# set-soft/ComfyUI-FLOAT_Optimized

Measured on AMD Instinct MI355X. Metric: 512x512 frames/sec end-to-end audio->video @50 ODE steps, higher is better.
Workload: dtype fp16; 1 GPU; configs[1]: 10 s audio + 512x512 portrait in HBM -> 250 frames in pinned host memory; appearance encoder + wav2vec2 audio encoder + FMT sampling (50 Euler evaluations/window, CFG a=2.0 e=1.0) + decode + D2H, through InferenceAgent.infer_device (the product call); nfe=51, frames_per_clip=250, fmt_dtype=fp16, dec_dtype=fp16, decode_batch=32, hip_graph=True, parallelism=replicas x1 (one clip per GPU), stage_overlap=off

## Files before the change

comfyui-float_optimized_amd/csrc/fmt_api.hip:

```cpp
#include <math.h>
#include <stdlib.h>

#include "fmt_gemm.hpp"
#include "fmt_kernels.hpp"
#include "fmt_rb_kernels.hpp"
#include "fmt_big_kernels.hpp"

namespace {

typedef FmtLin Lin;

struct Blk {
  Lin qkv, proj, fc1, fc2;
};

constexpr int kMaxTok = 80;
constexpr int kMaxSteps = 1024;

}

struct float_fmt {
  float_fmt_cfg_t cfg;
  DevicePool pool;
  int D, ntok, Mpad, Kc, Ntot, Kx;
// ... 388 lines not shown
  }
}

struct Tiling {
  int mtw, nt, nw;
};
int pick_nw(int K, int forced) {
  const int KB = K / 32;
  if (forced && KB % forced == 0) return forced;
  if (KB >= 128 && KB % 16 == 0) return 16;
  if (KB >= 32 && KB % 8 == 0) return 8;
  return 4;
}
Tiling pick_tiling(const FmtTune& tn, int M, int N, int K, bool need_full_rows) {
  const int mt = (M + 15) / 16;
  if (need_full_rows) {
    if (mt <= 4) return {4, 1, pick_nw(K, 0)};
    return {mt <= 12 ? 12 : 15, 1, (tn.full_nw == 8 && (K / 32) % 8 == 0) ? 8 : 4};
  }
  int split = mt <= 4 ? 4 : (mt <= 12 ? 3 : 5);
  if (mt <= 2) split = mt;
  const int blocks = (mt + split - 1) / split;
  const bool wide = N >= 16384;
  if (mt >= 12) {
    const int* o = tn.plan + (wide ? 3 : 0);
    if (o[0]) {
      int nw = o[0] >= 12 ? 4 : pick_nw(K, o[2]);
      while (nw > 4 && nw * o[0] * 16 * o[1] * 16 * 4 > 160 * 1024) nw >>= 1;
      return {o[0], o[1], nw};
    }
  }
  if (wide) return {mt <= 4 ? 4 : 6, 2, std::min(8, pick_nw(K, 0))};
  if (mt > 15 && N % 64 == 0) return {3, 4, 4};
  int nt = 1;
  if (mt >= 5) {
    if ((N / 64) * blocks >= 192 && N % 64 == 0) nt = 4;
    else if ((N / 32) * blocks >= 192 && N % 32 == 0) nt = 2;
  } else if ((N / 16) * blocks > 512) {
    nt = 2;
  }
  return {split, nt, pick_nw(K, 0)};
}

GemmArgs base_args(const u16* A, const Lin& L, int M) {
  GemmArgs g;
  memset(&g, 0, sizeof(g));
  g.A = A;
  g.W = L.W;
  g.bias = L.b;
  g.K = L.K;
  g.N = L.N;
  g.M = M;
  return g;
}

Tiling pick_tiling32(int M) {
  const int mt = (M + 15) / 16;
  return {mt <= 5 ? mt : (mt <= 12 ? 3 : 5), 1, 4};
}

template <class T, int EPI>
int run_gemm(const FmtTune& tn, const GemmArgs& g, hipStream_t s, bool need_full_rows = false, const LayerPlan* plan = nullptr) {
  if constexpr (T::is32) {
    FH_REQUIRE(!need_full_rows, "the fp32 mode has no all-rows CFG epilogue tiling (token-blocked head only)");
    const Tiling t = pick_tiling32(g.M);
    GemmArgs g2 = g;
    g2.touch.W = nullptr;
    return launch_gemm<T, EPI>(g2, t.mtw, t.nt, t.nw, false, s);
  }
  if (plan && plan->on() && (g.M + 15) / 16 <= 15) {
    GemmArgs g2 = g;
    g2.touch.W = nullptr;
    return launch_gemm<T, EPI>(g2, plan->v[0], plan->v[1], plan->v[2], false, s);
  }
  const Tiling t = pick_tiling(tn, g.M, g.N, g.K, need_full_rows);
  return launch_gemm<T, EPI>(g, t.mtw, t.nt, t.nw, false, s);
}

struct PendingRed {
  int ks = 0;
  LnRed red{};
};

template <class T>
int run_gemm_partial(float_fmt* h, GemmArgs g, int ksplit, hipStream_t s, const LayerPlan* plan = nullptr) {
  g.ksplit = ksplit;
  g.out_f32 = h->slab;
  g.ldo = g.N;
  g.slab_stride = (size_t)h->Mpad * g.N;
  if (plan && plan->on() && !T::is32 && (g.M + 15) / 16 <= 15) {
    g.touch.W = nullptr;
    return launch_gemm<T, EPI_PARTIAL>(g, plan->v[0], plan->v[1], plan->v[2], false, s);
  }
  Tiling t = T::is32 ? pick_tiling32(g.M) : pick_tiling(h->tune, g.M, g.N * ksplit, g.K / ksplit, false);
  while (t.nt > 1 && g.N % (t.nt * 16)) t.nt >>= 1;
  if (T::is32) g.touch.W = nullptr;
  return launch_gemm<T, EPI_PARTIAL>(g, t.mtw, t.nt, t.nw, false, s);
}

TouchSpec make_touch(const FmtTune& tn, const Lin& L, int M, int ksplit, unsigned lanes, unsigned per_lane, int force_nt = 0) {
  TouchSpec t{};
  Tiling tl = ksplit ? pick_tiling(tn, M, L.N * ksplit, L.K / ksplit, false) : pick_tiling(tn, M, L.N, L.K, false);
  if (force_nt) tl.nt = force_nt;
  if (ksplit)
    while (tl.nt > 1 && L.N % (tl.nt * 16)) tl.nt >>= 1;
  const int ks = ksplit ? ksplit : 1;
  if (L.N % (tl.nt * 16) || L.K % (32 * ks) || 8 % ks) return t;
  const int nbn = L.N / (tl.nt * 16);
  if ((nbn * ks) % 8) return t;
  auto lg = [](unsigned v) {
    int n = 0;
    while ((1u << n) < v) ++n;
    return (1u << n) == v ? n : -1;
  };
  const unsigned P = 8 / ks, run_lines = (unsigned)(L.K / 32 / ks) * 8u;
  if (lg(run_lines) < 0 || lg((unsigned)tl.nt) < 0) return t;
  t.run_shift = (unsigned)lg(run_lines);
  t.nt_shift = (unsigned)lg((unsigned)tl.nt);
  t.p_shift = (unsigned)lg(P);
  t.tile_bytes = (unsigned)(L.K / 32) * 1024u;
  t.total = ((unsigned)nbn / P) * (unsigned)tl.nt * run_lines;
  if ((size_t)t.total > (size_t)lanes * per_lane) return t;
  t.W = reinterpret_cast<const char*>(L.W);
  return t;
}

TouchSpec make_touch_rb(const Lin& L, int shape, int kb, unsigned lanes, unsigned per_lane) {
  TouchSpec t{};
  const int ct = shape == 0 ? 4 : 8;
  if (kb <= 0 || (kb & (kb - 1)) || L.N % (ct * 16) || (L.N / (ct * 16)) % 8 || L.K / 32 < kb) return t;
  const unsigned run_lines = (unsigned)kb * 8u;
  auto lg = [](unsigned v) {
    int n = 0;
    while ((1u << n) < v) ++n;
    return n;
  };
  t.run_shift = (unsigned)lg(run_lines);
  t.nt_shift = (unsigned)lg((unsigned)ct);
  t.p_shift = 3;
  t.tile_bytes = (unsigned)(L.K / 32) * 1024u;
  t.total = (unsigned)(L.N / (ct * 16) / 8) * (unsigned)ct * run_lines;
  if ((size_t)t.total > (size_t)lanes * per_lane) return t;
  t.W = reinterpret_cast<const char*>(L.W);
  return t;
}

unsigned gemm_lanes_per_xcd(const FmtTune& tn, int M, int N, int K) {
  const Tiling t = pick_tiling(tn, M, N, K, false);
  const int mblk = ((M + 15) / 16 + t.mtw - 1) / t.mtw;
  return (unsigned)((N / (t.nt * 16)) * mblk / 8) * (unsigned)(t.nw * 64);
}

template <class T>
int launch_lnmod(float_fmt* h, int M, const float* shift, const float* scale, hipStream_t s, PendingRed* pend = nullptr,
                 const Lin* next = nullptr, u16* out = nullptr, int perm = 0, int touch_bit = 1, int rb_shape = -1) {
  const int nv = h->D / 256;
  const int rpw = h->tune.ln_rows;
  dim3 grid(rpw == 1 ? ((M + 63) / 64) * 64 : (M + rpw - 1) / rpw), block(64 * rpw);
  const int ks = pend ? pend->ks : 0;
  const bool wt = M <= kWtRows;
  LnRed red{};
  if (ks) red = pend->red;
  TouchSpec pf{};
  if (next && (h->tune.touch & (1 | touch_bit)) && rpw == 1 && !T::is32)
    pf = rb_shape >= 0 ? make_touch_rb(*next, rb_shape, h->tune.rb_touch, (grid.x / 8) * 64, 6)
                       : make_touch(h->tune, *next, M, 0, (grid.x / 8) * 64, 6);
#define LN_LAUNCH(NV, KS)                                                                                                          \
  do {                                                                                                                             \
    if (pf.W && wt) hipLaunchKernelGGL((fmt_lnmod_kernel<T, NV, KS, true, true>), grid, block, 0, s, h->xres, M, shift, scale, h->Ntot, out ? out : h->h16, red, pf, h->ntok, perm, h->sat); \
    else if (pf.W) hipLaunchKernelGGL((fmt_lnmod_kernel<T, NV, KS, true, false>), grid, block, 0, s, h->xres, M, shift, scale, h->Ntot, out ? out : h->h16, red, pf, h->ntok, perm, h->sat); \
    else if (wt) hipLaunchKernelGGL((fmt_lnmod_kernel<T, NV, KS, false, true>), grid, block, 0, s, h->xres, M, shift, scale, h->Ntot, out ? out : h->h16, red, pf, h->ntok, perm, h->sat); \
    else hipLaunchKernelGGL((fmt_lnmod_kernel<T, NV, KS, false, false>), grid, block, 0, s, h->xres, M, shift, scale, h->Ntot, out ? out : h->h16, red, pf, h->ntok, perm, h->sat);   \
  } while (0)
#define LN_CASE(NV)                     \
  case NV:                              \
    if (ks == 0) LN_LAUNCH(NV, 0);      \
    else if (ks == 1) LN_LAUNCH(NV, 1); \
    else if (ks == 2) LN_LAUNCH(NV, 2); \
    else if (ks == 4) LN_LAUNCH(NV, 4); \
    else LN_LAUNCH(NV, 8);              \
    break;
  switch (nv) {
    LN_CASE(1) LN_CASE(2) LN_CASE(4) LN_CASE(8)
    default:
      fh_set_error("dim_h %d unsupported (must be 256*{1,2,4,8})", h->D);
      return FLOAT_E_INVALID;
  }
#undef LN_CASE
#undef LN_LAUNCH
  if (pend) pend->ks = 0;
  FH_CHECK_HIP(hipGetLastError());
  return FLOAT_OK;
}

template <class T>
void launch_attn(float_fmt* h, int M, const Lin* pull, hipStream_t s) {
  const float_fmt_cfg_t& c = h->cfg;
  const int D = h->D, ntok = h->ntok;
  const int qpw = h->tune.attn_qpw, lpq = h->tune.attn_lpq;
  dim3 grid(c.heads, (M + qpw - 1) / qpw), block(qpw * lpq);
  TouchSpec pf{};
  if (pull && !T::is32) pf = make_touch(h->tune, *pull, M, 0, (grid.x * grid.y / 8) * block.x, 2);
#define ATTN_LAUNCH(LPQ, TCH)                                                                                                  \
  do {                                                                                                                         \
    if (M <= kWtRows) hipLaunchKernelGGL((fmt_attn_kernel<T, LPQ, TCH, true>), grid, block, 0, s, h->qkv16, 3 * D, h->att16, ntok, M, D, c.attn_window, pf, h->sat); \
    else hipLaunchKernelGGL((fmt_attn_kernel<T, LPQ, TCH, false>), grid, block, 0, s, h->qkv16, 3 * D, h->att16, ntok, M, D, c.attn_window, pf, h->sat);             \
  } while (0)
  if (lpq == 16) {
    if (pf.W) ATTN_LAUNCH(16, true);
    else ATTN_LAUNCH(16, false);
  } else {
    if (pf.W) ATTN_LAUNCH(8, true);
    else ATTN_LAUNCH(8, false);
  }
#undef ATTN_LAUNCH
}

int attnproj_hpw(const float_fmt* h) {
  const int hd = h->cfg.heads, hpw = h->tune.attnproj;
  if (hpw <= 0 || h->D != hd * 128 || hd % hpw) return 0;
  const int ks = hd / hpw;
  return (ks == 1 || ks == 2 || ks == 4 || ks == 8) && (hpw == 1 || hpw == 2) ? hpw : 0;
}
template <class T>
int launch_attnproj(float_fmt* h, int M, const Lin& proj, hipStream_t s) {
  const float_fmt_cfg_t& c = h->cfg;
  const int hpw = attnproj_hpw(h);
  GemmArgs g = base_args(nullptr, proj, M);
  g.sat = h->sat;
  g.out_f32 = h->slab;
  g.ldo = g.N;
  g.slab_stride = (size_t)h->Mpad * g.N;
  g.ksplit = c.heads / hpw;
  g.mblk = ((M + 15) / 16 + 2) / 3;
  const dim3 grid((unsigned)(g.ksplit * (g.N / (128 / hpw)) * g.mblk));
  fh_launch_prof(0, hpw == 2 ? fmt_attnproj_kernel<T, 3, 2> : fmt_attnproj_kernel<T, 3, 1>, grid, dim3(512), 0, s, h->qkv16, 3 * h->D, g,
                 h->ntok, h->D, c.attn_window);
  FH_CHECK_HIP(hipGetLastError());
  return FLOAT_OK;
}

constexpr int kScSteps = 64;

static int stream_priority(hipStream_t s) {
  int prio = 0;
  if (hipStreamGetPriority(s, &prio) != hipSuccess) {
    (void)hipGetLastError();
    prio = 0;
  }
  return prio;
}

template <class T>
int run_mod_all(float_fmt* h, int M, int e0, int n, hipStream_t s) {
  const int D = h->D;
  const FmtTune& tn = h->tune;
  FH_REQUIRE(n >= 1 && n <= kScSteps, "modulation batch of %d evaluations (max %d)", n, kScSteps);
  const int prio = (s == h->cap_stream && s) ? h->cap_prio : stream_priority(s);
  const bool big = !T::is32 && tn.wide && prio == 0 && big_shape_ok(tn, n * M, h->adaln_all.N, h->adaln_all.K, h->n_cu);
  hipLaunchKernelGGL((fmt_silu_c_kernel<T>), dim3((M * D / 8 + 255) / 256, n), dim3(256), 0, s, h->sc16, h->temb + (size_t)e0 * D,
                     h->ccond, M, D, (size_t)h->Mpad * D, big ? M : 0, h->sat);
  h->mod_zs = big ? (size_t)M * h->Ntot : (size_t)h->Mmod * h->Ntot;
  if constexpr (!T::is32) {
    if (big) return launch_big4<T>(h->sc16, h->adaln_all, h->modall, n * M, h->Ntot, h->n_cu, false, s);
  }
  GemmArgs g = base_args(h->sc16, h->adaln_all, M);
  g.sat = h->sat;
  g.out_f32 = h->modall;
  g.ldo = h->Ntot;
  g.zcount = n;
  const bool dma = (tn.wide_variant == 6 || tn.wide_variant == 7) && (M + 15) / 16 > 4 && dma_shape_ok(g, 320);
  g.zgroup = tn.zgroup > 0 ? tn.zgroup : (dma ? 2 : 4);
  g.a_zstride = (size_t)h->Mpad * D;
  g.o_zstride = (size_t)h->Mmod * h->Ntot;
  if constexpr (!T::is32) {
    if (tn.wide && g.N % 128 == 0 && g.K % 128 == 0) return launch_wide<T>(g, tn.wide_variant, false, s);
  }
  for (int z = 0; z < n; ++z) {
    GemmArgs gz = g;
    gz.A = g.A + (size_t)z * g.a_zstride * (sizeof(typename T::elem) / sizeof(u16));
    gz.out_f32 = g.out_f32 + (size_t)z * g.o_zstride;
    gz.zcount = 0;
    int rc = run_gemm<T, EPI_F32>(tn, gz, s);
    if (rc) return rc;
  }
  return FLOAT_OK;
}

constexpr int kMegaWgs = 256, kMegaSmem = 8 * 48 * 64 * 4;
MegaSync mega_sync_of(const float_fmt* h) {
  unsigned* m = h->mega_sync;
  return MegaSync{m, m + 8 * 32, m + 9 * 32, m + 17 * 32, m + 18 * 32, h->mega_err_host, reinterpret_cast<unsigned long long*>(m + 20 * 32), (unsigned)h->tune.mega_stamp_wg};
}
int mega_poll(float_fmt* h) {
  if (!h->mega_err_host || *reinterpret_cast<volatile unsigned*>(h->mega_err_host) == 0u) return FLOAT_OK;
  FH_CHECK_HIP(hipDeviceSynchronize());
  for (auto& gr : h->graphs) (void)hipGraphExecDestroy(gr.exec);
  h->graphs.clear();
  if (h->mega_sync) FH_CHECK_HIP(hipMemset(h->mega_sync, 0, (size_t)(32 * 20) * sizeof(unsigned)));
  *reinterpret_cast<volatile unsigned*>(h->mega_err_host) = 0u;
  h->tune.mega = 0;
  h->job.active = false;
  fh_set_error("fmt_mega_kernel: a grid barrier timed out in an earlier call (not all %d workgroups were resident) - the results of "
               "that call are invalid; the handle falls back to the launch chain (FLOAT_FMT_MEGA=0 selects it from the start)", 256);
  return FLOAT_E_HIP;
}
template <class T>
bool mega_shape_ok(const float_fmt* h, int nclip, int bc) {
  const FmtTune& tn = h->tune;
  if (T::is32 || !tn.mega || nclip != 1 || bc != 3 || h->D != 1024 || h->cfg.heads != 8 || h->n_cu < kMegaWgs) return false;
  if (attnproj_hpw(h) || tn.fc2_split != 4 || tn.proj_split != 0) return false;
  const int M = bc * h->ntok;
  auto is = [](Tiling t, int a, int b, int c) { return t.mtw == a && t.nt == b && t.nw == c; };
  const Blk& B = h->blk[0];
  return (M + 15) / 16 == 12 && (h->ntok + 15) / 16 == 4 && h->x_embed.K % 256 == 0 && h->final_lin.K % 256 == 0 &&
         is(pick_tiling(tn, M, B.qkv.N, B.qkv.K, false), 3, 4, 8) && is(pick_tiling(tn, M, B.proj.N, B.proj.K, false), 3, 1, 8) &&
         is(pick_tiling(tn, M, B.fc1.N, B.fc1.K, false), 3, 4, 8) && is(pick_tiling(tn, M, B.fc2.N * 4, B.fc2.K / 4, false), 3, 4, 8) &&
         B.fc2.K % 512 == 0;
}

template <class T>
int build_mega(float_fmt* h, int bc) {
  float_fmt::MegaPlan& P = h->mega[bc];
  P.tried = 1;
  {
    int per_cu = 0;
    if (hipOccupancyMaxActiveBlocksPerMultiprocessor(&per_cu, reinterpret_cast<const void*>(fmt_mega_kernel<T>), 512, kMegaSmem) != hipSuccess) {
      (void)hipGetLastError();
      per_cu = 0;
    }
    if (per_cu * h->n_cu < kMegaWgs) {
      h->tune.mega = 0;
      return FLOAT_OK;
    }
  }
  const float_fmt_cfg_t& c = h->cfg;
  const FmtTune& tn = h->tune;
  const int D = h->D, ntok = h->ntok, M = bc * ntok;
  std::vector<MegaStage> st;
  const size_t esz = sizeof(typename T::elem) / sizeof(u16);
  const size_t n_h = (size_t)h->Mpad * D * esz, n_hid = (size_t)h->Mpad * c.mlp_hidden * esz;
  if (!h->mega_ws) {
    int rc0 = h->pool.alloc(&h->mega_ws, (size_t)c.depth * (3 * n_h + n_hid), true);
    if (rc0) return rc0;
  }
  auto ws_h1 = [&](int b) { return h->mega_ws + (size_t)b * (3 * n_h + n_hid); };
  auto ws_h2 = [&](int b) { return ws_h1(b) + n_h; };
  auto ws_att = [&](int b) { return ws_h1(b) + 2 * n_h; };
  auto ws_hid = [&](int b) { return ws_h1(b) + 3 * n_h; };
  auto gemm_stage = [&](int kind, GemmArgs g, int mtw, int nt) {
    MegaStage m;
    memset(&m, 0, sizeof(m));
    m.kind = kind;
    g.sat = h->sat;
    g.mblk = ((g.M + 15) / 16 + mtw - 1) / mtw;
    if (g.ksplit < 1) g.ksplit = 1;
    m.g = g;
    m.nblk = (unsigned)((g.N / (nt * 16)) * g.mblk * g.ksplit);
    return m;
  };
  auto ln_stage = [&](int b_mod, int which, int ks, const float* bias, int gate_col, const Lin* next, int touch_bit, u16* out, int perm) {
    MegaStage m;
    memset(&m, 0, sizeof(m));
    m.kind = MS_LN;
    m.nblk = (unsigned)(((M + 63) / 64) * 64);
    m.shift_off = (long long)b_mod * 6 * D + (long long)which * D;
    m.scale_off = m.shift_off + D;
    m.ks = ks;
    m.red_bias = bias;
    m.red_gate_off = (long long)b_mod * 6 * D + (long long)gate_col * D;
    m.ln_out = out ? out : h->h16;
    m.perm = perm;
    if (next && (tn.touch & (1 | touch_bit))) m.pf = make_touch(tn, *next, M, 0, (m.nblk / 8) * 64, 6);
    return m;
  };
  {
    GemmArgs g = base_args(h->xin16, h->x_embed, ntok);
    g.out_f32 = h->xres;
    g.ldo = D;
    g.pos = h->pos;
    g.bc = bc;
    g.ntok = ntok;
    st.push_back(gemm_stage(MS_XEMBED, g, 4, 1));
  }
  for (int b = 0; b < c.depth; ++b) {
    const Blk& B = h->blk[b];
    if (b == 0) st.push_back(ln_stage(b, 0, 0, nullptr, 0, &B.qkv, 128, ws_h1(b), 0));
    else {
      MegaStage m = ln_stage(b, 0, 4, h->blk[b - 1].fc2.b, 0, &B.qkv, 128, ws_h1(b), 0);
      m.red_gate_off = (long long)(b - 1) * 6 * D + 5LL * D;
      st.push_back(m);
    }
    {
      GemmArgs g = base_args(ws_h1(b), B.qkv, M);
      g.out16 = h->qkv16;
      g.ldo16 = 3 * D;
      if (tn.touch & 8) g.touch = make_touch(tn, B.proj, M, 0, gemm_lanes_per_xcd(tn, M, g.N, g.K), 2);
      st.push_back(gemm_stage(MS_QKV, g, 3, 4));
    }
    {
      MegaStage m;
      memset(&m, 0, sizeof(m));
      m.kind = MS_ATTN;
      m.nblk = (unsigned)(c.heads * ((M + 7) / 8));
      if (tn.touch & 2) m.pf = make_touch(tn, B.proj, M, 0, (m.nblk / 8) * 128, 2);
      m.att_out = ws_att(b);
      st.push_back(m);
    }
    {
      GemmArgs g = base_args(ws_att(b), B.proj, M);
      g.out_f32 = h->xres;
      g.ldo = D;
      g.ldg = h->Ntot;
      if (tn.touch & 16) g.touch = make_touch(tn, B.fc1, M, 0, gemm_lanes_per_xcd(tn, M, g.N, g.K), 2);
      MegaStage m = gemm_stage(MS_PROJ, g, 3, 1);
      m.gate_off = (long long)b * 6 * D + 2LL * D;
      st.push_back(m);
    }
    st.push_back(ln_stage(b, 3, 0, nullptr, 0, &B.fc1, 64, ws_h2(b), 0));
    {
      GemmArgs g = base_args(ws_h2(b), B.fc1, M);
      g.out16 = ws_hid(b);
      g.ldo16 = B.fc2.K / 32;
      if (tn.touch & 4) g.touch = make_touch(tn, B.fc2, M, 4, gemm_lanes_per_xcd(tn, M, g.N, g.K), 2);
      st.push_back(gemm_stage(MS_FC1, g, 3, 4));
    }
    {
      GemmArgs g = base_args(ws_hid(b), B.fc2, M);
      g.ksplit = 4;
      g.out_f32 = h->slab;
      g.ldo = g.N;
      g.slab_stride = (size_t)h->Mpad * g.N;
      if (tn.touch & 32) {
        const unsigned lanes = gemm_lanes_per_xcd(tn, M, g.N * 4, g.K / 4);
        if (b + 1 < c.depth) g.touch = make_touch(tn, h->blk[b + 1].qkv, M, 0, lanes, 2);
        else g.touch = make_touch(tn, h->final_lin, M, 0, lanes, 2, 1);
      }
      st.push_back(gemm_stage(MS_FC2, g, 3, 4));
    }
  }
  {
    const int nblk = (ntok + 15) / 16, seqs = bc;
    MegaStage m = ln_stage(c.depth, 0, 4, h->blk[c.depth - 1].fc2.b, 0, nullptr, 0, h->hfin16, seqs * 16);
    m.red_gate_off = (long long)(c.depth - 1) * 6 * D + 5LL * D;
    st.push_back(m);
    GemmArgs g = base_args(h->hfin16, h->final_lin, nblk * seqs * 16);
    g.tokblk = 1;
    g.nclip = 1;
    g.bc = bc;
    g.ntok = ntok;
    g.n_prev = c.n_prev;
    g.xcur = h->xcur;
    g.xin16 = h->xin16;
    g.ldx = h->Kx / 32;
    st.push_back(gemm_stage(MS_HEAD, g, bc, 1));
  }
  for (const MegaStage& m : st) FH_REQUIRE(m.nblk <= (unsigned)kMegaWgs, "persistent kernel: a stage needs %u workgroups", m.nblk);
  int rc;
  if (!h->mega_sync && (rc = h->pool.alloc(&h->mega_sync, 32 * 20 + 2 * 3 * 64, true))) return rc;
  if (!h->mega_err_host) {
    FH_CHECK_HIP(hipHostMalloc(reinterpret_cast<void**>(&h->mega_err_host), 64, hipHostMallocMapped));
    memset(h->mega_err_host, 0, 64);
  }
  if ((rc = h->pool.alloc(&P.dev, st.size(), false))) return rc;
  FH_CHECK_HIP(hipMemcpy(P.dev, st.data(), st.size() * sizeof(MegaStage), hipMemcpyHostToDevice));
  P.nstage = (int)st.size();
  P.bc = bc;
  P.ctx = MegaCtx{h->xres, h->qkv16, h->slab, (size_t)h->Mpad * D, M, D, ntok, h->Ntot, c.attn_window, c.heads, h->sat};
  return FLOAT_OK;
}

template <class T>
int run_mega(float_fmt* h, int bc, const float* modbuf, bool euler, float dt, float a, float r, float e, hipStream_t s, float* vout_to) {
  float_fmt::MegaPlan& P = h->mega[bc];
  MegaDyn d{modbuf, dt, a, r, e, euler ? 1 : 0, vout_to ? vout_to : h->vout};
  fh_launch_prof(0, (fmt_mega_kernel<T>), dim3(kMegaWgs), dim3(512), kMegaSmem, s, P.dev, P.nstage, d, P.ctx, mega_sync_of(h));
  FH_CHECK_HIP(hipGetLastError());
  return FLOAT_OK;
}

template <class T>
int run_blocks(float_fmt* h, int nclip, int bc, const float* modbuf, bool euler, float dt, float a, float r, float e, hipStream_t s,
               float* vout_to = nullptr) {
  const float_fmt_cfg_t& c = h->cfg;
  const FmtTune& tn = h->tune;
  const int D = h->D, ntok = h->ntok, M = nclip * bc * ntok;
  int rc;
  if constexpr (!T::is32) {
    if (bc <= 4 && mega_shape_ok<T>(h, nclip, bc)) {
      if (h->mega[bc].dev) return run_mega<T>(h, bc, modbuf, euler, dt, a, r, e, s, vout_to);
    }
  }
  {
    GemmArgs g = base_args(h->xin16, h->x_embed, nclip * ntok);
    g.sat = h->sat;
    g.out_f32 = h->xres;
    g.ldo = D;
    g.pos = h->pos;
    g.bc = bc;
    g.ntok = ntok;
    if ((rc = run_gemm<T, EPI_XEMBED>(tn, g, s))) return rc;
  }
  PendingRed pend;
  RbPlan rb_qkv, rb_proj, rb_fc1, rb_fc2;
  if constexpr (!T::is32) {
    rb_qkv = pick_rb(tn, RB_QKV, M), rb_proj = pick_rb(tn, RB_PROJ, M), rb_fc1 = pick_rb(tn, RB_FC1, M), rb_fc2 = pick_rb(tn, RB_FC2, M);
  }
  auto split_ok = [&](int ks, const Lin& L) { return (ks == 1 || ks == 2 || ks == 4) && L.K % (128 * ks) == 0; };
  for (int b = 0; b < c.depth; ++b) {
    const float* mod = modbuf + (size_t)b * 6 * D;
    const Blk& B = h->blk[b];
    if ((rc = launch_lnmod<T>(h, M, mod, mod + D, s, &pend, &B.qkv, nullptr, 0, 128, rb_qkv.shape))) return rc;
    {
      GemmArgs g = base_args(h->h16, B.qkv, M);
      g.sat = h->sat;
      g.out16 = h->qkv16;
      g.ldo16 = 3 * D;
      if ((tn.touch & 8) && attnproj_hpw(h)) g.touch = make_touch(tn, B.proj, M, c.heads / attnproj_hpw(h), gemm_lanes_per_xcd(tn, M, g.N, g.K), 2, 8 / attnproj_hpw(h));
      else if ((tn.touch & 8) && !split_ok(tn.proj_split, B.proj)) g.touch = make_touch(tn, B.proj, M, 0, gemm_lanes_per_xcd(tn, M, g.N, g.K), 2);
      if (rb_qkv.shape >= 0) rc = launch_rbs<T, EPI_T16>(g, rb_qkv.shape, false, s);
      else rc = run_gemm<T, EPI_T16>(tn, g, s, false, &tn.plan_layer[RB_QKV]);
      if (rc) return rc;
    }
    if (rb_proj.shape >= 0) {
      launch_attn<T>(h, M, nullptr, s);
      GemmArgs gp = base_args(h->att16, B.proj, M);
      gp.ksplit = rb_proj.ksplit;
      gp.out_f32 = h->slab;
      gp.ldo = gp.N;
      gp.slab_stride = (size_t)h->Mpad * gp.N;
      if ((rc = launch_rbs<T, EPI_PARTIAL>(gp, rb_proj.shape, false, s))) return rc;
      pend.ks = rb_proj.ksplit;
      pend.red = LnRed{h->slab, (size_t)h->Mpad * D, B.proj.b, mod + 2 * D};
    } else if (attnproj_hpw(h)) {
      if ((rc = launch_attnproj<T>(h, M, B.proj, s))) return rc;
      pend.ks = c.heads / attnproj_hpw(h);
      pend.red = LnRed{h->slab, (size_t)h->Mpad * D, B.proj.b, mod + 2 * D};
    } else if (split_ok(tn.proj_split, B.proj)) {
      launch_attn<T>(h, M, nullptr, s);
      GemmArgs gp = base_args(h->att16, B.proj, M);
      if ((rc = run_gemm_partial<T>(h, gp, tn.proj_split, s))) return rc;
      pend.ks = tn.proj_split;
      pend.red = LnRed{h->slab, (size_t)h->Mpad * D, B.proj.b, mod + 2 * D};
    } else {
      launch_attn<T>(h, M, (tn.touch & 2) ? &B.proj : nullptr, s);
      GemmArgs g = base_args(h->att16, B.proj, M);
      g.sat = h->sat;
      g.out_f32 = h->xres;
      g.ldo = D;
      g.gate = mod + 2 * D;
      g.ldg = h->Ntot;
      if (tn.touch & 16) g.touch = make_touch(tn, B.fc1, M, 0, gemm_lanes_per_xcd(tn, M, g.N, g.K), 2);
      if ((rc = run_gemm<T, EPI_GATE_RES>(tn, g, s, false, &tn.plan_layer[RB_PROJ]))) return rc;
    }
    if ((rc = launch_lnmod<T>(h, M, mod + 3 * D, mod + 4 * D, s, &pend, &B.fc1, nullptr, 0, 64, rb_fc1.shape))) return rc;
    {
      GemmArgs g = base_args(h->h16, B.fc1, M);
      g.sat = h->sat;
      g.out16 = h->hid16;
      g.ldo16 = B.fc2.K / 32;
      if ((tn.touch & 4) && rb_fc2.shape < 0)
        g.touch = make_touch(tn, B.fc2, M, split_ok(tn.fc2_split, B.fc2) ? tn.fc2_split : 0, gemm_lanes_per_xcd(tn, M, g.N, g.K), 2);
      if (rb_fc1.shape >= 0) rc = launch_rbs<T, EPI_GELU_P16>(g, rb_fc1.shape, false, s);
      else rc = run_gemm<T, EPI_GELU_P16>(tn, g, s, false, &tn.plan_layer[RB_FC1]);
      if (rc) return rc;
    }
    if (rb_fc2.shape >= 0) {
      GemmArgs g = base_args(h->hid16, B.fc2, M);
      g.ksplit = rb_fc2.ksplit;
      g.out_f32 = h->slab;
      g.ldo = g.N;
      g.slab_stride = (size_t)h->Mpad * g.N;
      if ((rc = launch_rbs<T, EPI_PARTIAL>(g, rb_fc2.shape, false, s))) return rc;
      pend.ks = rb_fc2.ksplit;
      pend.red = LnRed{h->slab, (size_t)h->Mpad * D, B.fc2.b, mod + 5 * D};
    } else if (split_ok(tn.fc2_split, B.fc2)) {
      GemmArgs g = base_args(h->hid16, B.fc2, M);
      g.sat = h->sat;
      if (tn.touch & 32) {
        const unsigned lanes = gemm_lanes_per_xcd(tn, M, g.N * tn.fc2_split, g.K / tn.fc2_split);
        if (b + 1 < c.depth) g.touch = make_touch(tn, h->blk[b + 1].qkv, M, 0, lanes, 2);
        else g.touch = make_touch(tn, h->final_lin, M, 0, lanes, 2, 1);
      }
      if ((rc = run_gemm_partial<T>(h, g, tn.fc2_split, s, &tn.plan_layer[RB_FC2]))) return rc;
      pend.ks = tn.fc2_split;
      pend.red = LnRed{h->slab, (size_t)h->Mpad * D, B.fc2.b, mod + 5 * D};
    } else {
      GemmArgs g = base_args(h->hid16, B.fc2, M);
      g.sat = h->sat;
      g.out_f32 = h->xres;
      g.ldo = D;
      g.gate = mod + 5 * D;
      g.ldg = h->Ntot;
      if ((rc = run_gemm<T, EPI_GATE_RES>(tn, g, s))) return rc;
    }
  }
  {
    const float* mod = modbuf + (size_t)c.depth * 6 * D;
    const bool tokblk = (!tn.no_tokblk || nclip > 1) && (bc == 1 || bc == 3 || bc == 4) && h->final_lin.K % 256 == 0;
    FH_REQUIRE(tokblk || nclip == 1, "batched sampling needs the token-blocked head GEMM");
    const int nblk = (ntok + 15) / 16, seqs = nclip * bc;
    if ((rc = launch_lnmod<T>(h, M, mod, mod + D, s, &pend, nullptr, tokblk ? h->hfin16 : nullptr, tokblk ? seqs * 16 : 0))) return rc;
    GemmArgs g = base_args(tokblk ? h->hfin16 : h->h16, h->final_lin, tokblk ? nblk * seqs * 16 : M);
    g.sat = h->sat;
    g.tokblk = tokblk ? 1 : 0;
    g.nclip = nclip;
    g.bc = bc;
    g.ntok = ntok;
    g.n_prev = c.n_prev;
    g.a_cfg = a;
    g.r_cfg = r;
    g.e_cfg = e;
    g.dt = dt;
    if (euler) {
      g.xcur = h->xcur;
      g.xin16 = h->xin16;
      g.ldx = h->Kx / 32;
    } else {
      g.vout = vout_to ? vout_to : h->vout;
    }
    if (tokblk) rc = launch_gemm<T, EPI_CFG>(g, bc, 1, 8, false, s);
    else rc = run_gemm<T, EPI_CFG>(tn, g, s, true);
    if (rc) return rc;
  }
  FH_CHECK_HIP(hipGetLastError());
  return FLOAT_OK;
}

void linspace01(int n, std::vector<float>* ts) {
  ts->resize(n);
  if (n == 1) {
    (*ts)[0] = 0.f;
    return;
  }
  const float step = 1.0f / (float)(n - 1);
  const int half = n / 2;
  for (int i = 0; i < n; ++i) (*ts)[i] = (i < half) ? (0.f + step * (float)i) : (1.0f - step * (float)(n - 1 - i));
}

struct TimeSpec {
  float t;
  int nfe, stages;
  float c[4];
};
template <class T>
int prepare_time(float_fmt* h, const TimeSpec& ts, int n, hipStream_t s) {
  int rc;
  hipLaunchKernelGGL((fmt_tsin_kernel<T>), dim3(n), dim3(256), 0, s, h->tsin16, h->freqs, n, ts.t, ts.nfe, ts.stages, ts.c[0],
                     ts.c[1], ts.c[2], ts.c[3]);
  GemmArgs g = base_args(h->tsin16, h->t0, n);
  g.sat = h->sat;
  g.out16 = h->th16;
  g.ldo16 = h->t2.K / 32;
  if ((rc = launch_gemm<T, EPI_SILU_P16>(g, 4, 1, T::is32 ? 4 : pick_nw(g.K, 0), false, s))) return rc;
  GemmArgs g2 = base_args(h->th16, h->t2, n);
  g2.sat = h->sat;
  g2.out_f32 = h->temb;
  g2.ldo = h->D;
  if ((rc = launch_gemm<T, EPI_F32>(g2, 4, 1, T::is32 ? 4 : pick_nw(g2.K, 0), false, s))) return rc;
  return FLOAT_OK;
}

struct CfgMode {
  int bc;
  unsigned wr_mask, wa_mask, we_mask;
  int nclip = 1;
};

CfgMode cfg_mode(float a, float r, float e, int include_r) {
  if (a == 1.0f && r == 1.0f && e == 1.0f) return {1, 1u, 1u, 1u, 1};
  if (!include_r) return {3, 0b111u, 0b110u, 0b010u, 1};
  return {4, 0b1110u, 0b1100u, 0b0100u, 1};
}

template <class T>
int stage_window(float_fmt* h, const CfgMode& m, const float* x0, const float* wa, const float* wr, const float* we,
                 int we_len, const float* prev_x, const float* prev_wa, const float* prev_we, hipStream_t s) {
  const float_fmt_cfg_t& c = h->cfg;
  const int M = m.nclip * m.bc * h->ntok;
  hipLaunchKernelGGL((fmt_build_cond_kernel<T>), dim3(M), dim3(256), 0, s, h->cond16, h->Kc, m.bc, h->ntok, c.n_prev,
                     c.dim_w, c.dim_a, c.dim_e, wr, wa, prev_wa, we, we_len, prev_we, m.wr_mask, m.wa_mask, m.we_mask, h->sat);
  GemmArgs g = base_args(h->cond16, h->c_embed, M);
  g.sat = h->sat;
  g.out_f32 = h->ccond;
  g.ldo = h->D;
  int rc;
  if ((rc = run_gemm<T, EPI_F32>(h->tune, g, s))) return rc;
  const int n = m.nclip * h->ntok * c.dim_w;
  hipLaunchKernelGGL((fmt_init_x_kernel<T>), dim3((n + 255) / 256), dim3(256), 0, s, h->xcur, h->xin16, h->Kx / 32, x0, prev_x,
                     c.n_prev, c.n_cur, c.dim_w, m.nclip, h->sat);
  FH_CHECK_HIP(hipGetLastError());
  return FLOAT_OK;
}

int check_common(float_fmt* h, const void* we, int we_len, const void* prev_we) {
  FH_REQUIRE(h != nullptr, "null FMT handle");
  FH_REQUIRE(we_len == 1 || we_len == h->cfg.n_cur,
             "Dynamic emotion latent `we` time dimension (%d) does not match audio latent `wa` time dimension (%d).",
             we_len, h->cfg.n_cur);
  FH_REQUIRE(!(we_len > 1 && prev_we == nullptr),
             "`we` is dynamic (T>1), but prev_we was not provided with prev_x/prev_wa.");
  (void)we;
  return FLOAT_OK;
}

struct Tableau {
  int s;
  float c[4], a[4][3], b[4];
};
const Tableau& tableau(int method) {
  static const Tableau T[5] = {
      {1, {0.f}, {{0.f}}, {1.f}},
      {2, {0.f, 0.5f}, {{0.f}, {0.5f}}, {0.f, 1.f}},
      {4, {0.f, 1.f / 3, 2.f / 3, 1.f}, {{0.f}, {1.f / 3}, {-1.f / 3, 1.f}, {1.f, -1.f, 1.f}}, {0.125f, 0.375f, 0.375f, 0.125f}},
      {2, {0.f, 1.f}, {{0.f}, {1.f}}, {0.5f, 0.5f}},
      {3, {0.f, 1.f / 3, 2.f / 3}, {{0.f}, {1.f / 3}, {0.f, 2.f / 3}}, {0.25f, 0.f, 0.75f}},
  };
  return T[method];
}

TimeSpec time_spec(int method, int nfe) {
  const Tableau& tb = tableau(method);
  TimeSpec ts{};
  ts.nfe = nfe;
  ts.stages = tb.s;
  for (int j = 0; j < 4; ++j) ts.c[j] = tb.c[j];
  return ts;
}
int n_evals(int method, int nfe) { return (nfe - 1) * tableau(method).s; }

template <class T>
int run_window_steps(float_fmt* h, const CfgMode& m, int nfe, const std::vector<float>& ts, float a, float r, float e,
                     hipStream_t s) {
  const Tableau& tb = tableau(h->method);
  const float_fmt_cfg_t& c = h->cfg;
  const size_t kstride = (size_t)h->Bmax * kMaxTok * c.dim_w;
  const int n = m.nclip * c.n_cur * c.dim_w, rows = m.nclip * m.bc * h->ntok;
  const int nev = n_evals(h->method, nfe), batch = h->tune.hoist ? kScSteps : 1;
  const bool euler = h->method == FLOAT_ODE_EULER;
  int rc;
  for (int ev = 0; ev < nev; ++ev) {
    const int i = ev / tb.s, j = ev - i * tb.s, z = ev % batch;
    const float dt = ts[i + 1] - ts[i];
    if (z == 0 && (rc = run_mod_all<T>(h, rows, ev, std::min(batch, nev - ev), s))) return rc;
    const float* mod = h->modall + (size_t)z * h->mod_zs;
    if (euler) {
      if ((rc = run_blocks<T>(h, m.nclip, m.bc, mod, true, dt, a, r, e, s))) return rc;
      continue;
    }
    if (j > 0) {
      hipLaunchKernelGGL((fmt_rk_combine_kernel<T>), dim3((n + 255) / 256), dim3(256), 0, s, h->xcur, h->kbuf, kstride, j,
                         dt * tb.a[j][0], dt * tb.a[j][1], dt * tb.a[j][2], 0.f, 0, h->xin16, h->Kx / 32, c.n_prev, c.n_cur,
                         c.dim_w, m.nclip, h->sat);
    }
    if ((rc = run_blocks<T>(h, m.nclip, m.bc, mod, false, 0.f, a, r, e, s, h->kbuf + (size_t)j * kstride))) return rc;
    if (j == tb.s - 1) {
      hipLaunchKernelGGL((fmt_rk_combine_kernel<T>), dim3((n + 255) / 256), dim3(256), 0, s, h->xcur, h->kbuf, kstride, tb.s,
                         dt * tb.b[0], dt * tb.b[1], dt * tb.b[2], dt * tb.b[3], 1, h->xin16, h->Kx / 32, c.n_prev, c.n_cur,
                         c.dim_w, m.nclip, h->sat);
    }
  }
  FH_CHECK_HIP(hipGetLastError());
  return FLOAT_OK;
}

constexpr size_t kMaxGraphs = 8;
template <class T>
int run_window_steps_graph(float_fmt* h, const CfgMode& m, int we_len, int nfe, const std::vector<float>& ts, float a,
                           float r, float e, hipStream_t s) {
  float_fmt::GraphKey key;
  memset(&key, 0, sizeof(key));
  key.nfe = nfe;
  key.method = h->method;
  key.bc = m.bc;
  key.nclip = m.nclip;
  key.we_len = we_len;
  key.a = a;
  key.r = r;
  key.e = e;
  key.prio = stream_priority(s);
  float_fmt::GraphEntry* hit = nullptr;
  for (auto& g : h->graphs)
    if (g.key == key) hit = &g;
  if (!hit) {
    if (!h->cap_stream) FH_CHECK_HIP(hipStreamCreateWithFlags(&h->cap_stream, hipStreamNonBlocking));
    hipGraph_t graph = nullptr;
    h->cap_prio = key.prio;
    FH_CHECK_HIP(hipStreamBeginCapture(h->cap_stream, hipStreamCaptureModeThreadLocal));
    int rc = run_window_steps<T>(h, m, nfe, ts, a, r, e, h->cap_stream);
    hipError_t ce = hipStreamEndCapture(h->cap_stream, &graph);
    if (rc) {
      if (graph) (void)hipGraphDestroy(graph);
      return rc;
    }
    FH_CHECK_HIP(ce);
    hipGraphExec_t exec = nullptr;
    FH_CHECK_HIP(hipGraphInstantiate(&exec, graph, nullptr, nullptr, 0));
    (void)hipGraphDestroy(graph);
    if (h->graphs.size() >= kMaxGraphs) {
      size_t lru = 0;
      for (size_t i = 1; i < h->graphs.size(); ++i)
        if (h->graphs[i].used < h->graphs[lru].used) lru = i;
      FH_CHECK_HIP(hipDeviceSynchronize());
      (void)hipGraphExecDestroy(h->graphs[lru].exec);
      h->graphs.erase(h->graphs.begin() + lru);
    }
    h->graphs.push_back({key, exec, 0});
    hit = &h->graphs.back();
  }
  hit->used = ++h->graph_clock;
  FH_CHECK_HIP(hipGraphLaunch(hit->exec, s));
  return FLOAT_OK;
}

template <class T>
int window_impl(float_fmt* h, const float* x0, const float* wa, const float* wr, const float* we, int we_len,
                const float* prev_x, const float* prev_wa, const float* prev_we, int nfe, const std::vector<float>& ts,
                float a, float r, float e, int include_r, hipStream_t s, int nclip = 1) {
  CfgMode m = cfg_mode(a, r, e, include_r);
  m.nclip = nclip;
  FH_REQUIRE(!h->tune.no_tokblk || m.bc * h->ntok <= 240,
             "%d-way CFG of %d tokens is %d rows; the all-rows CFG epilogue GEMM holds at most 240 (15 row tiles)", m.bc, h->ntok,
             m.bc * h->ntok);
  int rc = stage_window<T>(h, m, x0, wa, wr, we, we_len, prev_x, prev_wa, prev_we, s);
  if (rc) return rc;
  if (nfe <= 1) return FLOAT_OK;
  hipStreamCaptureStatus cs = hipStreamCaptureStatusNone;
  if (hipStreamIsCapturing(s, &cs) != hipSuccess) {
    (void)hipGetLastError();
    cs = hipStreamCaptureStatusNone;
  }
  if (h->cfg.use_graph && !g_fh_profiling && cs == hipStreamCaptureStatusNone)
    return run_window_steps_graph<T>(h, m, we_len, nfe, ts, a, r, e, s);
  return run_window_steps<T>(h, m, nfe, ts, a, r, e, s);
}

template <class T>
int eval_impl(float_fmt* h, float t, const float* x, const float* wa, const float* wr, const float* we, int we_len,
              const float* prev_x, const float* prev_wa, const float* prev_we, float a, float r, float e, int include_r,
              float* out, hipStream_t s) {
  TimeSpec tsp{};
  tsp.t = t;
  int rc = prepare_time<T>(h, tsp, 1, s);
  if (rc) return rc;
  const CfgMode m = cfg_mode(a, r, e, include_r);
  FH_REQUIRE(!h->tune.no_tokblk || m.bc * h->ntok <= 240,
             "%d-way CFG of %d tokens is %d rows; the all-rows CFG epilogue GEMM holds at most 240 (15 row tiles)", m.bc, h->ntok,
             m.bc * h->ntok);
  if ((rc = stage_window<T>(h, m, x, wa, wr, we, we_len, prev_x, prev_wa, prev_we, s))) return rc;
  if ((rc = run_mod_all<T>(h, m.bc * h->ntok, 0, 1, s))) return rc;
  if ((rc = run_blocks<T>(h, 1, m.bc, h->modall, false, 0.f, a, r, e, s))) return rc;
  return dev_copy(out, h->vout, (size_t)h->ntok * h->cfg.dim_w, s);
}

template <class T>
int sample_window(float_fmt* h, int k, hipStream_t s) {
  const float_fmt_cfg_t& c = h->cfg;
  auto& J = h->job;
  const int L = c.n_cur, P = c.n_prev, Tn = J.T, B = J.B;
  const bool dynamic = J.we_len > 1;
  int rc;
  auto blocks = [](int n) { return dim3((n + 255) / 256); };
  if (k == J.first) {
    if ((rc = prepare_time<T>(h, time_spec(h->method, J.nfe), std::max(1, n_evals(h->method, J.nfe)), s))) return rc;
    if (J.hist_x) rc = dev_copy(h->prev_x, J.hist_x, (size_t)B * P * c.dim_w, s);
    else rc = dev_zero(h->prev_x, (size_t)B * P * c.dim_w, s);
    if (rc) return rc;
    if (J.hist_wa) rc = dev_copy(h->prev_wa, J.hist_wa, (size_t)B * P * c.dim_a, s);
    else rc = dev_zero(h->prev_wa, (size_t)B * P * c.dim_a, s);
    if (rc) return rc;
    if (J.hist_we) rc = dev_copy(h->prev_we, J.hist_we, (size_t)B * P * c.dim_e, s);
    else rc = dev_zero(h->prev_we, (size_t)B * P * c.dim_e, s);
    if (rc) return rc;
  } else if (P > 0) {
    hipLaunchKernelGGL(fmt_tail_kernel, blocks(B * P * c.dim_w), dim3(256), 0, s, h->prev_x, h->xcur, P, L, c.dim_w, B);
    hipLaunchKernelGGL(fmt_tail_kernel, blocks(B * P * c.dim_a), dim3(256), 0, s, h->prev_wa, h->wa_c, P, L, c.dim_a, B);
    if (dynamic) hipLaunchKernelGGL(fmt_tail_kernel, blocks(B * P * c.dim_e), dim3(256), 0, s, h->prev_we, h->we_c, P, L, c.dim_e, B);
  }
  hipLaunchKernelGGL(fmt_slice_pad_kernel, blocks(B * L * c.dim_a), dim3(256), 0, s, h->wa_c, J.wa, k * L, Tn, L, c.dim_a, B);
  if (dynamic) hipLaunchKernelGGL(fmt_slice_pad_kernel, blocks(B * L * c.dim_e), dim3(256), 0, s, h->we_c, J.we, k * L, Tn, L, c.dim_e, B);
  if ((rc = dev_copy(h->x0_c, J.noise + (size_t)k * B * L * c.dim_w, (size_t)B * L * c.dim_w, s))) return rc;
  rc = window_impl<T>(h, h->x0_c, h->wa_c, J.wr, dynamic ? h->we_c : J.we, dynamic ? L : 1, h->prev_x, h->prev_wa,
                      dynamic ? h->prev_we : nullptr, J.nfe, J.ts, J.a, J.r, J.e, J.include_r, s, B);
  if (rc) return rc;
  const int rows = (k == J.total - 1) ? (Tn - k * L) : L;
  return dev_copy2d(J.r_d + (size_t)k * L * c.dim_w, (size_t)Tn * c.dim_w, h->xcur, (size_t)L * c.dim_w, rows * c.dim_w, B, s);
}

template <class T>
int create_impl(float_fmt* h, const TensorTable& tt) {
  const float_fmt_cfg_t& c = h->cfg;
  const int D = c.dim_h;
  int rc;
  prime_kernels<T>();
  if ((rc = pack_linear<T>(h, tt, {"x_embedder.proj"}, D, c.dim_w, &h->x_embed))) return rc;
  if ((rc = pack_linear<T>(h, tt, {"t_embedder.mlp.0"}, D, 256, &h->t0))) return rc;
  if ((rc = pack_linear<T>(h, tt, {"t_embedder.mlp.2"}, D, D, &h->t2))) return rc;
  if ((rc = pack_linear<T>(h, tt, {"c_embedder"}, D, c.dim_w + c.dim_a + c.dim_e, &h->c_embed))) return rc;
  h->blk.resize(c.depth);
  std::vector<std::string> ada;
  for (int b = 0; b < c.depth; ++b) {
    const std::string p = "blocks." + std::to_string(b) + ".";
    if ((rc = pack_linear<T>(h, tt, {p + "attn.qkv"}, 3 * D, D, &h->blk[b].qkv))) return rc;
    if ((rc = pack_linear<T>(h, tt, {p + "attn.proj"}, D, D, &h->blk[b].proj))) return rc;
    if ((rc = pack_linear<T>(h, tt, {p + "mlp.fc1"}, c.mlp_hidden, D, &h->blk[b].fc1))) return rc;
    if ((rc = pack_linear<T>(h, tt, {p + "mlp.fc2"}, D, c.mlp_hidden, &h->blk[b].fc2))) return rc;
    ada.push_back(p + "adaLN_modulation.1");
  }
  if ((rc = pack_linear<T>(h, tt, ada, 6 * D, D, &h->adaln_all))) return rc;
  {
    Lin tail;
    if ((rc = pack_linear<T>(h, tt, {"decoder.adaLN_modulation.1"}, 2 * D, D, &tail))) return rc;
    Lin fused;
    fused.N = h->adaln_all.N + tail.N;
    fused.K = h->adaln_all.K;
    constexpr size_t esz = sizeof(typename T::elem) / sizeof(u16);
    if ((rc = h->pool.alloc(&fused.W, (size_t)fused.N * fused.K * esz, false))) return rc;
    if ((rc = h->pool.alloc(&fused.b, (size_t)fused.N, false))) return rc;
    FH_CHECK_HIP(hipMemcpy(fused.W, h->adaln_all.W, (size_t)h->adaln_all.N * fused.K * esz * sizeof(u16), hipMemcpyDeviceToDevice));
    FH_CHECK_HIP(hipMemcpy(fused.W + (size_t)h->adaln_all.N * fused.K * esz, tail.W, (size_t)tail.N * fused.K * esz * sizeof(u16),
                           hipMemcpyDeviceToDevice));
    FH_CHECK_HIP(hipMemcpy(fused.b, h->adaln_all.b, (size_t)h->adaln_all.N * sizeof(float), hipMemcpyDeviceToDevice));
    FH_CHECK_HIP(hipMemcpy(fused.b + h->adaln_all.N, tail.b, (size_t)tail.N * sizeof(float), hipMemcpyDeviceToDevice));
    h->adaln_all = fused;
  }
  if ((rc = pack_linear<T>(h, tt, {"decoder.linear"}, c.dim_w, D, &h->final_lin))) return rc;
  return FLOAT_OK;
}

}


int fmt_pack_linear(const FmtTune& tn, DevicePool* pool, int dtype, const TensorTable& tt, const std::vector<std::string>& names,
                    int N_each, int K, FmtLin* out) {
  FH_REQUIRE(dtype == FLOAT_DT_BF16 || dtype == FLOAT_DT_FP16 || dtype == FLOAT_DT_FP32, "the GEMM service: unknown dtype %d", dtype);
  if (dtype == FLOAT_DT_FP32) return pack_linear_pool<FP32>(tn, pool, tt, names, N_each, K, out);
  return dtype == FLOAT_DT_BF16 ? pack_linear_pool<BF16>(tn, pool, tt, names, N_each, K, out)
                                : pack_linear_pool<FP16>(tn, pool, tt, names, N_each, K, out);
}

int fmt_pack_linear_raw(const FmtTune& tn, DevicePool* pool, int dtype, const float* w, const float* b, int N, int K, FmtLin* out) {
  std::vector<float> zeros;
  if (!b) {
    zeros.assign(N, 0.f);
    b = zeros.data();
  }
  float_tensor_t t[2];
  memset(t, 0, sizeof(t));
  t[0].name = "raw.weight";
  t[0].data = w;
  t[0].ndim = 2;
  t[0].shape[0] = N;
  t[0].shape[1] = K;
  t[1].name = "raw.bias";
  t[1].data = b;
  t[1].ndim = 1;
  t[1].shape[0] = N;
  TensorTable tt(t, 2);
  return fmt_pack_linear(tn, pool, dtype, tt, {"raw"}, N, K, out);
}

GemmArgs fmt_gemm_args(const u16* A, const FmtLin& L, int M) { return base_args(A, L, M); }

void fmt_gemm_prime(int dtype) {
  if (dtype == FLOAT_DT_BF16) prime_kernels<BF16>();
  else if (dtype == FLOAT_DT_FP32) prime_kernels<FP32>();
  else prime_kernels<FP16>();
}

template <class T>
static int gemm_run_t(const FmtTune& tn, int epi, const GemmArgs& g, hipStream_t s) {
  switch (epi) {
    case EPI_F32: return run_gemm<T, EPI_F32>(tn, g, s);
    case EPI_T16: return run_gemm<T, EPI_T16>(tn, g, s);
    case EPI_SILU_P16: return run_gemm<T, EPI_SILU_P16>(tn, g, s);
    case EPI_GELU_P16: return run_gemm<T, EPI_GELU_P16>(tn, g, s);
    case EPI_GELUERF_P16: return run_gemm<T, EPI_GELUERF_P16>(tn, g, s);
    default: fh_set_error("fmt_gemm_run: epilogue %d is not exported", epi); return FLOAT_E_INVALID;
  }
}

int fmt_gemm_run(const FmtTune& tn, int dtype, int epi, GemmArgs g, hipStream_t s) {
  if (dtype == FLOAT_DT_FP32) return gemm_run_t<FP32>(tn, epi, g, s);
  return dtype == FLOAT_DT_BF16 ? gemm_run_t<BF16>(tn, epi, g, s) : gemm_run_t<FP16>(tn, epi, g, s);
}

template <class T>
static int debug_impl(float_fmt* h, int what, const float* in, float* out, hipStream_t s) {
  const int D = h->D, ntok = h->ntok;
  if (what == 0) {
    return dev_copy(out, h->pos, (size_t)ntok * D, s);
  }
  if (what == 2) {
    FH_REQUIRE(h->mega_sync && h->mega[3].nstage > 0 && h->mega[3].nstage <= 64, "no persistent-kernel plan");
    FH_CHECK_HIP(hipStreamSynchronize(s));
    const int n = h->mega[3].nstage * 3;
    std::vector<unsigned long long> st(n);
    FH_CHECK_HIP(hipMemcpy(st.data(), h->mega_sync + 20 * 32, n * 8, hipMemcpyDeviceToHost));
    std::vector<float> us(n);
    for (int i = 0; i < n; ++i) us[i] = st[i] ? (float)((double)(st[i] - st[0]) * 0.01) : -1.f;
    FH_CHECK_HIP(hipMemcpy(out, us.data(), n * 4, hipMemcpyHostToDevice));
    return FLOAT_OK;
  }
  FH_REQUIRE(what == 1 && in != nullptr, "float_fmt_debug: unknown request %d (or null input)", what);
// ... 19 lines not shown
  FH_REQUIRE(cfg->max_batch >= 0 && cfg->max_batch <= 16, "max_batch must be in [0, 16] (got %d)", cfg->max_batch);
  float_fmt* h = new float_fmt();
  h->tune = FmtTune::from_env();
  h->cfg = *cfg;
  h->D = cfg->dim_h;
  h->ntok = cfg->n_prev + cfg->n_cur;
  h->Bmax = cfg->max_batch > 0 ? cfg->max_batch : 1;
  h->Mpad = 16 * ((h->Bmax * 4 * h->ntok + 15) / 16 + 12);
  h->Kc = round_up(cfg->dim_w + cfg->dim_a + cfg->dim_e, 128);
  h->Kx = round_up(cfg->dim_w, 128);
  {
    int dev = 0, ncu = 0;
    if (hipGetDevice(&dev) == hipSuccess && hipDeviceGetAttribute(&ncu, hipDeviceAttributeMultiprocessorCount, dev) == hipSuccess) h->n_cu = ncu;
    else (void)hipGetLastError();
  }
  h->Ntot = cfg->depth * 6 * h->D + 2 * h->D;
  TensorTable tt(tensors, n_tensors);
  int rc = (cfg->dtype == FLOAT_DT_BF16) ? create_impl<BF16>(h, tt)
           : (cfg->dtype == FLOAT_DT_FP16) ? create_impl<FP16>(h, tt) : create_impl<FP32>(h, tt);
  const int D = h->D, Mp = h->Mpad;
  const size_t esz = cfg->dtype == FLOAT_DT_FP32 ? 2 : 1;
  auto A = [&](auto** p, size_t n) {
    if (!rc) rc = h->pool.alloc(p, std::is_same<std::remove_reference_t<decltype(**p)>, u16>::value ? n * esz : n, true);
  };
  A(&h->pos, (size_t)kMaxTok * D);
  A(&h->freqs, 128);
  A(&h->cond16, (size_t)Mp * h->Kc);
  A(&h->sc16, (size_t)kScSteps * Mp * D + (size_t)12 * 16 * D);
  A(&h->h16, (size_t)Mp * D);
  A(&h->hfin16, (size_t)h->Bmax * 64 * ((kMaxTok + 15) / 16) * D);
  A(&h->qkv16, (size_t)Mp * 3 * D);
  A(&h->att16, (size_t)Mp * D);
  A(&h->hid16, (size_t)Mp * cfg->mlp_hidden);
  A(&h->xin16, (size_t)(h->Bmax * kMaxTok + 6 * 16) * h->Kx);
  A(&h->tsin16, (size_t)kMaxSteps * 256);
  A(&h->th16, (size_t)kMaxSteps * D);
  A(&h->ccond, (size_t)Mp * D);
  h->Mmod = 16 * ((h->Bmax * 4 * h->ntok + 15) / 16);
  if (!rc) rc = h->pool.alloc(&h->modall, (size_t)kScSteps * h->Mmod * h->Ntot, false);
  A(&h->kbuf, (size_t)4 * h->Bmax * kMaxTok * cfg->dim_w);
  A(&h->xres, (size_t)Mp * D);
  A(&h->slab, (size_t)8 * Mp * D);
  A(&h->sat, 1);
  A(&h->xcur, (size_t)h->Bmax * cfg->n_cur * cfg->dim_w);
  A(&h->temb, (size_t)kMaxSteps * D);
  A(&h->vout, (size_t)h->Bmax * kMaxTok * cfg->dim_w);
  A(&h->wa_c, (size_t)h->Bmax * cfg->n_cur * cfg->dim_a);
  A(&h->we_c, (size_t)h->Bmax * cfg->n_cur * cfg->dim_e);
  A(&h->x0_c, (size_t)h->Bmax * cfg->n_cur * cfg->dim_w);
  A(&h->prev_x, (size_t)h->Bmax * cfg->n_cur * cfg->dim_w);
  A(&h->prev_wa, (size_t)h->Bmax * cfg->n_cur * cfg->dim_a);
  A(&h->prev_we, (size_t)h->Bmax * cfg->n_cur * cfg->dim_e);
  if (!rc) {
    std::vector<float> pos((size_t)h->ntok * D);
    const float_tensor_t* pe = tt.find("pos_embed");
    if (pe && TensorTable::numel(pe) == (int64_t)h->ntok * D) {
      memcpy(pos.data(), pe->data, pos.size() * sizeof(float));
    } else {
      for (int p = 0; p < h->ntok; ++p)
        for (int j = 0; j < D; ++j) {
          const float ang = (float)((double)p / pow(10000.0, 2.0 * (double)(j / 2) / (double)D));
          pos[(size_t)p * D + j] = (j & 1) ? cosf(ang) : sinf(ang);
        }
    }
    std::vector<float> fr(128);
    for (int k = 0; k < 128; ++k) fr[k] = expf(-logf(10000.0f) * (float)k / 128.0f);
    if (hipMemcpy(h->pos, pos.data(), pos.size() * sizeof(float), hipMemcpyHostToDevice) != hipSuccess ||
        hipMemcpy(h->freqs, fr.data(), fr.size() * sizeof(float), hipMemcpyHostToDevice) != hipSuccess) {
      fh_set_error("hipMemcpy of FMT tables failed");
      rc = FLOAT_E_HIP;
    }
  }
  if (!rc && cfg->dtype != FLOAT_DT_FP32) {
    const bool ok = cfg->dtype == FLOAT_DT_BF16 ? mega_shape_ok<BF16>(h, 1, 3) : mega_shape_ok<FP16>(h, 1, 3);
    if (ok) rc = cfg->dtype == FLOAT_DT_BF16 ? build_mega<BF16>(h, 3) : build_mega<FP16>(h, 3);
  }
  if (rc) {
    float_fmt_destroy(h);
    return rc;
  }
  *out = h;
  return FLOAT_OK;
}

void float_fmt_destroy(float_fmt_t* h) {
  if (!h) return;
  for (auto& g : h->graphs) (void)hipGraphExecDestroy(g.exec);
  if (h->cap_stream) (void)hipStreamDestroy(h->cap_stream);
  if (h->mega_err_host) (void)hipHostFree(h->mega_err_host);
  h->pool.release();
  delete h;
}

int float_fmt_eval(float_fmt_t* h, float t, const float* x, const float* wa, const float* wr, const float* we,
                   int32_t we_len, const float* prev_x, const float* prev_wa, const float* prev_we, float a_cfg,
                   float r_cfg, float e_cfg, int32_t include_r_cfg, float* out, void* stream) {
  int rc = check_common(h, we, we_len, prev_we);
  if (rc) return rc;
  if ((rc = mega_poll(h))) return rc;
  FH_REQUIRE(x && wa && wr && we && prev_x && prev_wa && out, "null tensor argument to float_fmt_eval");
  hipStream_t s = (hipStream_t)stream;
  return h->cfg.dtype == FLOAT_DT_BF16
             ? eval_impl<BF16>(h, t, x, wa, wr, we, we_len, prev_x, prev_wa, prev_we, a_cfg, r_cfg, e_cfg, include_r_cfg, out, s)
         : h->cfg.dtype == FLOAT_DT_FP16
             ? eval_impl<FP16>(h, t, x, wa, wr, we, we_len, prev_x, prev_wa, prev_we, a_cfg, r_cfg, e_cfg, include_r_cfg, out, s)
             : eval_impl<FP32>(h, t, x, wa, wr, we, we_len, prev_x, prev_wa, prev_we, a_cfg, r_cfg, e_cfg, include_r_cfg, out, s);
}

int float_fmt_sample_chunk(float_fmt_t* h, const float* x0, const float* wa, const float* wr, const float* we,
                           int32_t we_len, const float* prev_x, const float* prev_wa, const float* prev_we, int32_t nfe,
                           float a_cfg, float r_cfg, float e_cfg, int32_t include_r_cfg, float* out, void* stream) {
  int rc = check_common(h, we, we_len, prev_we);
  if (rc) return rc;
  if ((rc = mega_poll(h))) return rc;
  FH_REQUIRE(x0 && wa && wr && we && prev_x && prev_wa && out, "null tensor argument to float_fmt_sample_chunk");
  FH_REQUIRE(nfe >= 1 && n_evals(h->method, nfe) < kMaxSteps, "nfe=%d: too many evaluations (max %d)", nfe, kMaxSteps);
  hipStream_t s = (hipStream_t)stream;
  std::vector<float> ts;
  linspace01(nfe, &ts);
  const float_fmt_cfg_t& c = h->cfg;
  if ((rc = dev_copy(h->x0_c, x0, (size_t)c.n_cur * c.dim_w, s))) return rc;
  if ((rc = dev_copy(h->wa_c, wa, (size_t)c.n_cur * c.dim_a, s))) return rc;
  if ((rc = dev_copy(h->prev_x, prev_x, (size_t)c.n_prev * c.dim_w, s))) return rc;
  if ((rc = dev_copy(h->prev_wa, prev_wa, (size_t)c.n_prev * c.dim_a, s))) return rc;
  if (we_len > 1) {
    if ((rc = dev_copy(h->we_c, we, (size_t)c.n_cur * c.dim_e, s))) return rc;
    if ((rc = dev_copy(h->prev_we, prev_we, (size_t)c.n_prev * c.dim_e, s))) return rc;
  }
  const float* we_p = we_len > 1 ? h->we_c : we;
  const float* pwe_p = we_len > 1 ? h->prev_we : nullptr;
  const TimeSpec tsp = time_spec(h->method, nfe);
  const int nev = std::max(1, n_evals(h->method, nfe));
#define FMT_CHUNK(TT)                                                                                                          \
  do {                                                                                                                           \
    if ((rc = prepare_time<TT>(h, tsp, nev, s))) return rc;                                                                      \
    rc = window_impl<TT>(h, h->x0_c, h->wa_c, wr, we_p, we_len, h->prev_x, h->prev_wa, pwe_p, nfe, ts, a_cfg, r_cfg, e_cfg,      \
                         include_r_cfg, s);                                                                                      \
  } while (0)
  if (c.dtype == FLOAT_DT_BF16) FMT_CHUNK(BF16);
  else if (c.dtype == FLOAT_DT_FP16) FMT_CHUNK(FP16);
  else FMT_CHUNK(FP32);
#undef FMT_CHUNK
  if (rc) return rc;
  return dev_copy(out, h->xcur, (size_t)c.n_cur * c.dim_w, s);
}

int float_fmt_debug(float_fmt_t* h, int32_t what, const float* in, float* out, void* stream) {
  FH_REQUIRE(h != nullptr && out != nullptr, "null argument to float_fmt_debug");
  return h->cfg.dtype == FLOAT_DT_BF16   ? debug_impl<BF16>(h, what, in, out, (hipStream_t)stream)
         : h->cfg.dtype == FLOAT_DT_FP16 ? debug_impl<FP16>(h, what, in, out, (hipStream_t)stream)
                                         : debug_impl<FP32>(h, what, in, out, (hipStream_t)stream);
}

int float_fmt_saturation(float_fmt_t* h, uint64_t* total, int32_t reset, void* stream) {
  FH_REQUIRE(h && total, "null argument to float_fmt_saturation");
  FH_CHECK_HIP(hipStreamSynchronize((hipStream_t)stream));
  unsigned long long v = 0;
  FH_CHECK_HIP(hipMemcpy(&v, h->sat, sizeof(v), hipMemcpyDeviceToHost));
  *total = v;
  if (reset) {
    FH_CHECK_HIP(hipMemsetAsync(h->sat, 0, sizeof(v), (hipStream_t)stream));
    FH_CHECK_HIP(hipStreamSynchronize((hipStream_t)stream));
  }
  if (int rc = mega_poll(h)) return rc;
  return FLOAT_OK;
}

int float_fmt_set_method(float_fmt_t* h, int32_t method) {
  FH_REQUIRE(h != nullptr, "null FMT handle");
  FH_REQUIRE(method >= FLOAT_ODE_EULER && method <= FLOAT_ODE_HEUN3, "unknown ODE method %d", method);
  h->method = method;
  return FLOAT_OK;
}

int float_fmt_sample_begin(float_fmt_t* h, const float* wr, const float* wa, int32_t T, const float* we, int32_t we_len,
                           const float* noise, int32_t nfe, float a_cfg, float r_cfg, float e_cfg, int32_t include_r_cfg,
                           float* r_d) {
  FH_REQUIRE(h != nullptr, "null FMT handle");
  FH_REQUIRE(wr && wa && we && noise && r_d, "null tensor argument to float_fmt_sample");
  FH_REQUIRE(T >= 1, "T must be >= 1 (got %d)", T);
  FH_REQUIRE(we_len == 1 || we_len == T,
             "Dynamic emotion latent `we` time dimension (%d) does not match audio latent `wa` time dimension (%d).",
             we_len, T);
  FH_REQUIRE(nfe >= 1 && n_evals(h->method, nfe) < kMaxSteps, "nfe=%d: too many evaluations (max %d)", nfe, kMaxSteps);
  auto& J = h->job;
  J.wr = wr;
  J.wa = wa;
  J.we = we;
  J.noise = noise;
  J.r_d = r_d;
  J.T = T;
  J.we_len = we_len;
  J.nfe = nfe;
  J.include_r = include_r_cfg;
  J.a = a_cfg;
  J.r = r_cfg;
  J.e = e_cfg;
  J.B = 1;
  J.next = 0;
  J.n_chunks = (T + h->cfg.n_cur - 1) / h->cfg.n_cur;
  J.first = 0;
  J.total = J.n_chunks;
  J.hist_x = J.hist_wa = J.hist_we = nullptr;
  linspace01(nfe, &J.ts);
  J.active = true;
  return FLOAT_OK;
}

int float_fmt_sample_begin_range(float_fmt_t* h, const float* wr, const float* wa, int32_t T, const float* we, int32_t we_len,
                                 const float* noise, int32_t nfe, float a_cfg, float r_cfg, float e_cfg, int32_t include_r_cfg,
                                 float* r_d, int32_t first_window, int32_t end_window, const float* hist_x, const float* hist_wa,
                                 const float* hist_we) {
  int rc = float_fmt_sample_begin(h, wr, wa, T, we, we_len, noise, nfe, a_cfg, r_cfg, e_cfg, include_r_cfg, r_d);
  if (rc) return rc;
  auto& J = h->job;
  J.active = false;
  FH_REQUIRE(first_window >= 0 && first_window < end_window && end_window <= J.total,
             "window range [%d, %d) outside the clip's %d windows", first_window, end_window, J.total);
  FH_REQUIRE(we_len == 1 || hist_we != nullptr || hist_x == nullptr,
             "a dynamic-emotion job that starts from a history needs hist_we too");
  J.first = J.next = first_window;
  J.n_chunks = end_window;
  J.hist_x = hist_x;
  J.hist_wa = hist_wa;
  J.hist_we = we_len > 1 ? hist_we : nullptr;
  J.active = true;
  return FLOAT_OK;
}

int float_fmt_sample_next(float_fmt_t* h, void* stream, int32_t* window_done, int32_t* windows_left) {
  FH_REQUIRE(h != nullptr && h->job.active, "float_fmt_sample_next without float_fmt_sample_begin");
  if (int prc = mega_poll(h)) return prc;
  auto& J = h->job;
  hipStream_t s = (hipStream_t)stream;
  const int k = J.next;
  int rc = h->cfg.dtype == FLOAT_DT_BF16   ? sample_window<BF16>(h, k, s)
           : h->cfg.dtype == FLOAT_DT_FP16 ? sample_window<FP16>(h, k, s)
                                           : sample_window<FP32>(h, k, s);
  if (rc) {
    J.active = false;
    return rc;
  }
  J.next = k + 1;
  if (window_done) *window_done = k;
  if (windows_left) *windows_left = J.n_chunks - J.next;
  if (J.next >= J.n_chunks) J.active = false;
  return FLOAT_OK;
}

int float_fmt_sample_batch(float_fmt_t* h, int32_t n_clips, const float* wr, const float* wa, int32_t T, const float* we,
                           int32_t we_len, const float* noise, int32_t nfe, float a_cfg, float r_cfg, float e_cfg,
                           int32_t include_r_cfg, float* r_d, void* stream) {
  FH_REQUIRE(h != nullptr, "null FMT handle");
  FH_REQUIRE(n_clips >= 1 && n_clips <= h->Bmax, "batch of %d clips, the handle was created with max_batch = %d", n_clips, h->Bmax);
  int rc = float_fmt_sample_begin(h, wr, wa, T, we, we_len, noise, nfe, a_cfg, r_cfg, e_cfg, include_r_cfg, r_d);
  if (rc) return rc;
  h->job.B = n_clips;
  int32_t left = 1;
  while (left > 0)
    if ((rc = float_fmt_sample_next(h, stream, nullptr, &left))) return rc;
  return FLOAT_OK;
}

int float_fmt_sample(float_fmt_t* h, const float* wr, const float* wa, int32_t T, const float* we, int32_t we_len,
                     const float* noise, int32_t nfe, float a_cfg, float r_cfg, float e_cfg, int32_t include_r_cfg,
                     float* r_d, void* stream) {
  int rc = float_fmt_sample_begin(h, wr, wa, T, we, we_len, noise, nfe, a_cfg, r_cfg, e_cfg, include_r_cfg, r_d);
  if (rc) return rc;
  int32_t left = 1;
  while (left > 0)
    if ((rc = float_fmt_sample_next(h, stream, nullptr, &left))) return rc;
  return FLOAT_OK;
}

}
```

comfyui-float_optimized_amd/csrc/fmt_kernels.hpp:

```cpp
#pragma once
#include "common.hpp"
#include "fmt_pack.hpp"

template <class T, int MTW, int NT, int NW, int EPI, bool COH>
__device__ __forceinline__ void fmt_gemm_body(const GemmArgs& g, const unsigned bid, const unsigned nblk) {
  constexpr int BN = NT * 16;
  constexpr int ROWS = MTW * 16;
  constexpr bool WT = NW >= 8 || COH;
  auto ldA = [](const typename T::elem* p) -> typename T::pack8 { return T::load8(p); };
  constexpr int NTHR = NW * 64;
  constexpr int PF = T::is32 ? 1 : ((MTW + NT <= 7) ? 4 : ((MTW + NT <= 8) ? 3 : 2));
  typedef typename T::elem E;
  typedef typename T::pack8 P8;
  extern __shared__ __attribute__((aligned(16))) float red[];
  const int lane = threadIdx.x & 63;
  const int w = threadIdx.x >> 6;
  const int r16 = lane & 15, q = lane >> 4;
  int bx, by, ks = 0;
  {
    const int nbn = g.N / BN, id = (int)bid;
    const int nbx = (EPI == EPI_PARTIAL) ? nbn * g.ksplit : nbn;
    if ((nbx & 7) == 0) {
      const int slot = id >> 3;
      by = slot % g.mblk;
      bx = (slot / g.mblk) * 8 + (id & 7);
    } else {
      bx = id % nbx;
      by = id / nbx;
    }
    if constexpr (EPI == EPI_PARTIAL) {
      if ((nbx & 7) == 0 && (8 % g.ksplit) == 0) {
        const int P = 8 / g.ksplit, x = bx & 7;
        ks = x / P;
        bx = (bx >> 3) * P + (x % P);
      } else {
        ks = bx / nbn;
        bx = bx % nbn;
      }
    }
  }
  const int nb0 = bx * NT;
  const int mt0 = by * MTW;
  const int n0 = nb0 * 16, m0 = mt0 * 16;

  f32x4 acc[MTW][NT];
#pragma unroll
  for (int i = 0; i < MTW; ++i)
#pragma unroll
    for (int j = 0; j < NT; ++j) acc[i][j] = f32x4{0.f, 0.f, 0.f, 0.f};

  const int KB = g.K >> 5;
  const int KBs = (EPI == EPI_PARTIAL) ? KB / g.ksplit : KB;
  const int KBw = KBs / NW;
  const E* Ap = reinterpret_cast<const E*>(g.A) + ((size_t)mt0 * KB + ks * KBs + w * KBw) * 512 + lane * 8;
  const E* Wp = reinterpret_cast<const E*>(g.W) + ((size_t)nb0 * KB + ks * KBs + w * KBw) * 512 + lane * 8;
  const size_t tstride = (size_t)KB * 512;
  constexpr bool kEarlyRes = (EPI == EPI_GATE_RES) && (MTW * 16 * (NT * 2) <= NW * 64);
  float4 res_pf[2], gate_pf[2];
  if constexpr (kEarlyRes) {
    const int r = threadIdx.x / (NT * 2), cg = threadIdx.x % (NT * 2);
    const int row = m0 + r, nb = n0 + cg * 8;
    if (r < ROWS && row < g.M) {
      const float* o = g.out_f32 + (size_t)row * g.ldo + nb;
      const float* gt = g.gate + (size_t)row * g.ldg + nb;
      res_pf[0] = fh_load_f4<COH>(o);
      res_pf[1] = fh_load_f4<COH>(o + 4);
      gate_pf[0] = fh_load_f4_stream(gt);
      gate_pf[1] = fh_load_f4_stream(gt + 4);
    }
  }

  P8 a[PF][MTW], b[PF][NT];
#pragma unroll
  for (int p = 0; p < PF; ++p) {
    if (p < KBw) {
#pragma unroll
      for (int j = 0; j < NT; ++j) b[p][j] = T::load8_nt(Wp + j * tstride + (size_t)p * 512);
#pragma unroll
      for (int i = 0; i < MTW; ++i) a[p][i] = ldA(Ap + i * tstride + (size_t)p * 512);
    }
  }
  constexpr bool kTouch = (EPI == EPI_GELU_P16 || EPI == EPI_T16 || EPI == EPI_GATE_RES || EPI == EPI_PARTIAL);
  unsigned touched[2] = {0u, 0u};
  if constexpr (kTouch) {
    if (g.touch.W) fmt_touch(g.touch, bid & 7, (bid >> 3) * NTHR + threadIdx.x, (nblk >> 3) * NTHR, touched);
  }
  for (int kb0 = 0; kb0 < KBw; kb0 += PF) {
#pragma unroll
    for (int p = 0; p < PF; ++p) {
      const int kb = kb0 + p;
      if (kb < KBw) {
#pragma unroll
        for (int i = 0; i < MTW; ++i)
#pragma unroll
          for (int j = 0; j < NT; ++j) acc[i][j] = T::mfma(a[p][i], b[p][j], acc[i][j]);
        if (kb + PF < KBw) {
#pragma unroll
          for (int j = 0; j < NT; ++j)
            b[p][j] = T::load8_nt(Wp + j * tstride + (size_t)(kb + PF) * 512);
#pragma unroll
          for (int i = 0; i < MTW; ++i) a[p][i] = ldA(Ap + i * tstride + (size_t)(kb + PF) * 512);
        }
      }
    }
  }

  if constexpr (kTouch) {
    if (g.touch.W) fmt_touch_retire(touched);
  }
  float* my = red + w * (ROWS * BN);
#pragma unroll
  for (int i = 0; i < MTW; ++i)
#pragma unroll
    for (int j = 0; j < NT; ++j)
#pragma unroll
      for (int r = 0; r < 4; ++r) my[(i * 16 + q * 4 + r) * BN + j * 16 + r16] = acc[i][j][r];
  __syncthreads();

  constexpr int S = ROWS * BN;
  constexpr int CG = BN / 8;
  unsigned rm = 0u;
  auto slab_sum = [&](int o) {
    float a = red[o];
#pragma unroll
    for (int ww = 1; ww < NW; ++ww) a += red[ww * S + o];
    return a;
  };
  if constexpr (EPI == EPI_CFG) {
    const int nclip = g.nclip > 1 ? g.nclip : 1;
    const int tb = g.tokblk ? by / nclip : 0, q = g.tokblk ? by - tb * nclip : 0;
    const int ni = g.tokblk ? 16 : g.ntok, i0 = tb * 16, rstride = g.tokblk ? 16 : g.ntok;
    float* const vout_q = g.vout ? g.vout + (size_t)q * g.ntok * g.N : nullptr;
    float* const xcur_q = g.xcur ? g.xcur + (size_t)q * (g.ntok - g.n_prev) * g.N : nullptr;
    for (int idx = threadIdx.x; idx < ni * BN; idx += NTHR) {
      const int il = idx / BN, i = i0 + il, c = idx % BN, n = n0 + c;
      if (i >= g.ntok) break;
      const float bias = g.bias[n];
      float v[4];
#pragma unroll
      for (int b2 = 0; b2 < 4; ++b2) {
        if (b2 < g.bc) {
          const int o = (b2 * rstride + il) * BN + c;
          v[b2] = slab_sum(o) + bias;
        } else {
          v[b2] = 0.f;
        }
      }
      float out;
      if (g.bc == 1) {
        out = v[0];
      } else if (g.bc == 3) {
        out = v[0] + g.a_cfg * (v[2] - v[0]) + g.e_cfg * (v[1] - v[2]);
      } else {
        out = v[0] + g.r_cfg * (v[1] - v[0]) + g.a_cfg * (v[3] - v[1]) + g.e_cfg * (v[2] - v[3]);
      }
      if (vout_q) vout_q[(size_t)i * g.N + n] = out;
      if (xcur_q && i >= g.n_prev) {
        const size_t xo = (size_t)(i - g.n_prev) * g.N + n;
        const float xn = xcur_q[xo] + g.dt * out;
        xcur_q[xo] = xn;
        reinterpret_cast<E*>(g.xin16)[fmt_pack_off(q * g.ntok + i, n, g.ldx)] = fh_cvt<T>(xn, rm);
      }
    }
  } else {
    for (int idx = threadIdx.x; idx < ROWS * CG; idx += NTHR) {
      const int r = idx / CG, cg = idx % CG;
      const int row = m0 + r, nb = n0 + cg * 8;
      if (row >= g.M) continue;
      float v[8];
      {
        const float* p0 = red + r * BN + cg * 8;
#pragma unroll
        for (int e = 0; e < 8; e += 4) {
          float4 a4 = *reinterpret_cast<const float4*>(p0 + e);
#pragma unroll
          for (int ww = 1; ww < NW; ++ww) {
            const float4 t4 = *reinterpret_cast<const float4*>(p0 + ww * S + e);
            a4.x += t4.x;
            a4.y += t4.y;
            a4.z += t4.z;
            a4.w += t4.w;
          }
          float4 bb = float4{0.f, 0.f, 0.f, 0.f};
          if constexpr (EPI != EPI_PARTIAL) bb = *reinterpret_cast<const float4*>(g.bias + nb + e);
          v[e + 0] = a4.x + bb.x;
          v[e + 1] = a4.y + bb.y;
          v[e + 2] = a4.z + bb.z;
          v[e + 3] = a4.w + bb.w;
        }
      }
      if constexpr (EPI == EPI_F32 || EPI == EPI_PARTIAL) {
        float* o = g.out_f32 + (size_t)ks * g.slab_stride + (size_t)row * g.ldo + nb;
        fh_store_f4_wt<fh_site<COH>(4), WT>(o, float4{v[0], v[1], v[2], v[3]});
        fh_store_f4_wt<fh_site<COH>(4), WT>(o + 4, float4{v[4], v[5], v[6], v[7]});
      } else if constexpr (EPI == EPI_T16 || EPI == EPI_SILU_P16 || EPI == EPI_GELU_P16 || EPI == EPI_GELUERF_P16) {
        P8 u;
#pragma unroll
        for (int i = 0; i < 8; ++i) {
          float x = v[i];
          if constexpr (EPI == EPI_SILU_P16) x = fh_silu(x);
          if constexpr (EPI == EPI_GELU_P16) x = fh_gelu_tanh(x);
          if constexpr (EPI == EPI_GELUERF_P16) x = fh_gelu_erf(x);
          T::set(u, i, x);
        }
        fh_track_pack<T>(rm, u);
        E* const o16 = reinterpret_cast<E*>(g.out16);
        if constexpr (EPI == EPI_T16) T::template store8_wt<fh_site<COH>(8), WT>(o16 + (size_t)row * g.ldo16 + nb, u);
        else T::template store8_wt<fh_site<COH>(8), WT>(o16 + fmt_pack_off(row, nb, g.ldo16), u);
      } else if constexpr (EPI == EPI_GATE_RES) {
        float* o = g.out_f32 + (size_t)row * g.ldo + nb;
        const float* gt = g.gate + (size_t)row * g.ldg + nb;
#pragma unroll
        for (int e = 0; e < 8; e += 4) {
          float4 x, gg;
          if constexpr (kEarlyRes) {
            x = res_pf[e / 4];
            gg = gate_pf[e / 4];
          } else {
            x = fh_load_f4<COH>(o + e);
            gg = fh_load_f4_stream(gt + e);
          }
          x.x += gg.x * v[e + 0];
          x.y += gg.y * v[e + 1];
          x.z += gg.z * v[e + 2];
          x.w += gg.w * v[e + 3];
          fh_store_f4_wt<fh_site<COH>(16), WT>(o + e, x);
        }
      } else if constexpr (EPI == EPI_XEMBED) {
        const int q = row / g.ntok, tok = row - q * g.ntok;
        const float* ps = g.pos + (size_t)tok * g.N + nb;
#pragma unroll
        for (int i = 0; i < 8; ++i) v[i] += ps[i];
        for (int b2 = 0; b2 < g.bc; ++b2) {
          float* o = g.out_f32 + (size_t)((q * g.bc + b2) * g.ntok + tok) * g.ldo + nb;
          fh_store_f4_wt<fh_site<COH>(32), WT>(o, float4{v[0], v[1], v[2], v[3]});
          fh_store_f4_wt<fh_site<COH>(32), WT>(o + 4, float4{v[4], v[5], v[6], v[7]});
        }
      }
    }
  }
  if constexpr (EPI == EPI_CFG || EPI == EPI_T16 || EPI == EPI_SILU_P16 || EPI == EPI_GELU_P16 || EPI == EPI_GELUERF_P16) fh_range_flush<T>(g.sat, rm);
}

template <class T, int MTW, int NT, int NW, int EPI>
__global__ __launch_bounds__(NW * 64) void fmt_gemm_kernel(GemmArgs g) {
  fmt_gemm_body<T, MTW, NT, NW, EPI, false>(g, blockIdx.x, gridDim.x);
}

template <class T, int MTW, int KCH , int NWV = 4>
__global__ __launch_bounds__(NWV * 64) void fmt_gemm_wide_kernel(GemmArgs g) {
  constexpr int EPI = EPI_F32;
  constexpr int NF = MTW * KCH;
  constexpr int NFW = (NF + NWV - 1) / NWV;
  constexpr int WR = NWV / 4, MTR = MTW / WR;
  static_assert(MTW % WR == 0, "row tiles must split evenly over the wave rows");
  extern __shared__ __attribute__((aligned(16))) unsigned char sA[];
  const int lane = threadIdx.x & 63, w = threadIdx.x >> 6, wc = w & 3, wr = w >> 2;
  const int r16 = lane & 15, q = lane >> 4;
  const int nbn = g.N >> 7;
  const int nbx = (EPI == EPI_PARTIAL) ? nbn * g.ksplit : nbn;
  int bx, by, bz = 0, ks = 0;
  {
    const int id = blockIdx.x;
    const int nz = g.zcount > 1 ? g.zcount : 1;
    if (nz > 1 && (nbx & 7) == 0 && g.zgroup > 1) {
      const int slot = id >> 3, G = g.zgroup, ncx = nbx >> 3, rows = g.mblk * nz;
      const int full = ncx / G, per_grp = G * rows;
      int grp = slot / per_grp, rem = slot - grp * per_grp, gw = G;
      if (grp >= full) {
        grp = full;
        rem = slot - full * per_grp;
        gw = ncx - full * G;
      }
      const int zy = rem / gw;
      bz = zy / g.mblk;
      by = zy - bz * g.mblk;
      bx = (grp * G + (rem - zy * gw)) * 8 + (id & 7);
    } else if ((nbx & 7) == 0) {
      const int slot = id >> 3, zy = slot % (g.mblk * nz);
      bz = zy / g.mblk;
      by = zy - bz * g.mblk;
      bx = (slot / (g.mblk * nz)) * 8 + (id & 7);
    } else {
      bx = id % nbx;
      const int zy = id / nbx;
      bz = zy / g.mblk;
      by = zy - bz * g.mblk;
    }
    if constexpr (EPI == EPI_PARTIAL) {
      if ((nbx & 7) == 0 && (8 % g.ksplit) == 0) {
        const int P = 8 / g.ksplit, x = bx & 7;
        ks = x / P;
        bx = (bx >> 3) * P + (x % P);
      } else {
        ks = bx / nbn;
        bx = bx % nbn;
      }
    }
  }
  const int mt0 = by * MTW;
  const int nb0 = bx * 8 + wc * 2;
  const int KB = g.K >> 5;
  const int KBs = (EPI == EPI_PARTIAL) ? KB / g.ksplit : KB;
  const int nchunk = KBs / KCH;
  const size_t tstride = (size_t)KB * 512;
  const u16* Wp = g.W + (size_t)nb0 * tstride + (size_t)ks * KBs * 512 + lane * 8;
  const u16* Ag = g.A + (size_t)bz * g.a_zstride + (size_t)mt0 * tstride + (size_t)ks * KBs * 512 + lane * 8;
  float* const outz = g.out_f32 + (size_t)bz * g.o_zstride + (size_t)ks * g.slab_stride;

  f32x4 acc[MTR][2];
#pragma unroll
  for (int i = 0; i < MTR; ++i) acc[i][0] = acc[i][1] = f32x4{0.f, 0.f, 0.f, 0.f};

  u32x4 an[NFW], bn[KCH][2], bc[KCH][2];
  auto issue = [&](int c) {
    const int kc = c * KCH;
#pragma unroll
    for (int f = 0; f < NFW; ++f) {
      const int fi = f * NWV + w;
      if (fi < NF) {
        const int i = fi / KCH, kk = fi % KCH;
        an[f] = *reinterpret_cast<const u32x4*>(Ag + i * tstride + (size_t)(kc + kk) * 512);
      }
    }
#pragma unroll
    for (int kk = 0; kk < KCH; ++kk) {
      bn[kk][0] = __builtin_nontemporal_load(reinterpret_cast<const u32x4*>(Wp + (size_t)(kc + kk) * 512));
      bn[kk][1] = __builtin_nontemporal_load(reinterpret_cast<const u32x4*>(Wp + tstride + (size_t)(kc + kk) * 512));
    }
  };
  auto commit = [&](int buf) {
#pragma unroll
    for (int f = 0; f < NFW; ++f) {
      const int fi = f * NWV + w;
      if (fi < NF) *reinterpret_cast<u32x4*>(sA + (buf * NF + fi) * 1024 + lane * 16) = an[f];
    }
#pragma unroll
    for (int kk = 0; kk < KCH; ++kk) {
      bc[kk][0] = bn[kk][0];
      bc[kk][1] = bn[kk][1];
    }
  };
  issue(0);
  commit(0);
  __syncthreads();
  for (int c = 0; c < nchunk; ++c) {
    const int buf = c & 1;
    if (c + 1 < nchunk) issue(c + 1);
#pragma unroll
    for (int kk = 0; kk < KCH; ++kk) {
#pragma unroll
      for (int i = 0; i < MTR; ++i) {
        const u32x4 a = *reinterpret_cast<const u32x4*>(sA + (buf * NF + (wr * MTR + i) * KCH + kk) * 1024 + lane * 16);
        acc[i][0] = T::mfma(bc[kk][0], a, acc[i][0]);
        acc[i][1] = T::mfma(bc[kk][1], a, acc[i][1]);
      }
    }
    if (c + 1 < nchunk) {
      commit(buf ^ 1);
      __syncthreads();
    }
  }
#pragma unroll
  for (int i = 0; i < MTR; ++i) {
// ... 86 lines not shown
#define DMA_WAIT(K)                                   \
  do {                                                \
    if (NHI == 0 || w < NHI) fh_wait_vmcnt<(K)*IMAX>(); \
    else fh_wait_vmcnt<(K)*ILO>();                    \
  } while (0)
  const unsigned abase = (unsigned)(lane * 16 + wr * 6 * 1024), bbase = (unsigned)(lane * 16 + (RT + wc * 5) * 1024);

  f32x4 acc[6][5];
#pragma unroll
  for (int i = 0; i < 6; ++i)
#pragma unroll
    for (int j = 0; j < 5; ++j) acc[i][j] = f32x4{0.f, 0.f, 0.f, 0.f};
  u32x4 a0[6], b0[5], a1[6], b1[5];

#define DMA_READ(S, AR, BR)                                        \
  do {                                                             \
    const unsigned so = (unsigned)(((S) % NS) * STAGE);            \
    AR[0] = fh_ds_read128<0>(abase + so);                          \
    AR[1] = fh_ds_read128<1024>(abase + so);                       \
    AR[2] = fh_ds_read128<2048>(abase + so);                       \
    AR[3] = fh_ds_read128<3072>(abase + so);                       \
    AR[4] = fh_ds_read128<4096>(abase + so);                       \
    AR[5] = fh_ds_read128<5120>(abase + so);                       \
    BR[0] = fh_ds_read128<0>(bbase + so);                          \
    BR[1] = fh_ds_read128<1024>(bbase + so);                       \
    BR[2] = fh_ds_read128<2048>(bbase + so);                       \
    BR[3] = fh_ds_read128<3072>(bbase + so);                       \
    BR[4] = fh_ds_read128<4096>(bbase + so);                       \
  } while (0)
#define DMA_STEP(S, AC, BC, AN, BN)                                                            \
  do {                                                                                         \
    const int s_ = (S);                                                                        \
    if (s_ + 1 < KB) {                                                                         \
      const int rem = KB - 2 - s_;                               \
      if (NS == 4 && rem >= 2) DMA_WAIT(2);                                                    \
      else if (rem >= 1) DMA_WAIT(1);                                                          \
      else DMA_WAIT(0);                                                                        \
    }                                                                                          \
    __builtin_amdgcn_s_barrier();                                                              \
    if (s_ + NS < KB) issue(s_ + NS);                                                          \
    if (s_ + 1 < KB) DMA_READ(s_ + 1, AN, BN);                                                 \
    __builtin_amdgcn_sched_barrier(0);                                                         \
    _Pragma("unroll") for (int i = 0; i < 6; ++i)                                              \
      _Pragma("unroll") for (int j = 0; j < 5; ++j) acc[i][j] = T::mfma(BC[j], AC[i], acc[i][j]); \
    __builtin_amdgcn_sched_barrier(0);                                                         \
    asm volatile("s_waitcnt lgkmcnt(0)" ::: "memory");                                         \
    __builtin_amdgcn_sched_barrier(0);                                                         \
  } while (0)

#define DMA_WAIT_UPTO(K)                      \
  do {                                        \
    const int k_ = (K);                       \
    if (NS == 4 && k_ >= 2) DMA_WAIT(2);      \
    else if (k_ >= 1) DMA_WAIT(1);            \
    else DMA_WAIT(0);                         \
  } while (0)
#define DMA_STEP_STG(S, AC, BC, AN, BN)                                                        \
  do {                                                                                         \
    const int s_ = (S);                                                                        \
    if (!g1 && s_ + 1 < KB) DMA_WAIT_UPTO(KB - 2 - s_);                                        \
    __builtin_amdgcn_s_barrier();                                                              \
    if (s_ + NS < KB) issue(s_ + NS);                                                          \
    if (s_ + 1 < KB) DMA_READ(s_ + 1, AN, BN);                                                 \
    asm volatile("s_waitcnt lgkmcnt(0)" ::: "memory");                                         \
    __builtin_amdgcn_sched_barrier(0);                                                         \
    if (g1 && s_ + 2 < KB) {                                                                   \
      DMA_WAIT_UPTO(KB - 3 - s_);                                                              \
    }                                                                                          \
    __builtin_amdgcn_s_barrier();                                                              \
    __builtin_amdgcn_sched_barrier(0);                                                         \
    _Pragma("unroll") for (int i = 0; i < 6; ++i)                                              \
      _Pragma("unroll") for (int j = 0; j < 5; ++j) acc[i][j] = T::mfma(BC[j], AC[i], acc[i][j]); \
    __builtin_amdgcn_sched_barrier(0);                                                         \
  } while (0)

  const bool g1 = wr == 1;
#ifdef DMA_CLK
  const unsigned long long c0 = clock64(), w0 = wall_clock64();
#endif
#pragma unroll
  for (int s = 0; s < NS; ++s) issue(s);
  if constexpr (STG) DMA_WAIT(NS - 2);
  else DMA_WAIT(NS - 1);
  __builtin_amdgcn_s_barrier();
  DMA_READ(0, a0, b0);
  asm volatile("s_waitcnt lgkmcnt(0)" ::: "memory");
  __builtin_amdgcn_sched_barrier(0);
  if constexpr (STG) {
    if (g1) __builtin_amdgcn_s_barrier();
    for (int s = 0; s < KB; s += 2) {
      DMA_STEP_STG(s, a0, b0, a1, b1);
      DMA_STEP_STG(s + 1, a1, b1, a0, b0);
    }
    if (!g1) __builtin_amdgcn_s_barrier();
  } else {
    for (int s = 0; s < KB; s += 2) {
      DMA_STEP(s, a0, b0, a1, b1);
      DMA_STEP(s + 1, a1, b1, a0, b0);
    }
  }
#ifdef DMA_CLK
  if ((blockIdx.x == 3000 || blockIdx.x == 6001) && threadIdx.x == 0) {
    const unsigned long long c1 = clock64(), w1 = wall_clock64();
    printf("tile loop: %llu core clocks, %llu wall ticks\n", c1 - c0, w1 - w0);
  }
#endif
#undef DMA_STEP_STG
#undef DMA_WAIT_UPTO
#undef DMA_STEP
#undef DMA_READ
#undef DMA_WAIT
  float* const outz = g.out_f32 + (size_t)bz * g.o_zstride;
  constexpr int OW = CT * 16, OSTR = OW + 4, C4 = OW / 4, NTHR = NW * 64;
  static_assert(96 * OSTR * 4 <= NS * STAGE, "output staging does not fit the ring");
  float* const so = reinterpret_cast<float*>(ring);
  float4 bb[5];
#pragma unroll
  for (int j = 0; j < 5; ++j) bb[j] = *reinterpret_cast<const float4*>(g.bias + (bx * CT + wc * 5 + j) * 16 + q * 4);
#pragma unroll
  for (int p = 0; p < 2; ++p) {
    if (wr == p) {
#pragma unroll
      for (int i = 0; i < 6; ++i)
#pragma unroll
        for (int j = 0; j < 5; ++j)
          *reinterpret_cast<float4*>(so + (i * 16 + r16) * OSTR + (wc * 5 + j) * 16 + q * 4) =
              float4{acc[i][j][0] + bb[j].x, acc[i][j][1] + bb[j].y, acc[i][j][2] + bb[j].z, acc[i][j][3] + bb[j].w};
    }
    __syncthreads();
    {
#pragma unroll
      for (int k = 0; k < (96 * C4) / NTHR; ++k) {
        const int idx = k * NTHR + threadIdx.x, rl = idx / C4, c4 = idx - rl * C4;
        const int row = by * (RT * 16) + p * 96 + rl;
        if (row < g.M)
          *reinterpret_cast<float4*>(outz + (size_t)row * g.ldo + bx * OW + c4 * 4) = *reinterpret_cast<const float4*>(so + rl * OSTR + c4 * 4);
      }
    }
    if (p == 0) __syncthreads();
  }
}

struct LnRed {
  const float* slab;
  size_t slab_stride;
  const float* bias;
  const float* gate;
};

constexpr int kLnTouch = 6;

template <class T, int NV, int KS, bool TOUCH, bool WT_, bool COH>
__device__ __forceinline__ void fmt_lnmod_body(float* __restrict__ x, int M, const float* __restrict__ shift,
                                               const float* __restrict__ scale, int ldm, u16* __restrict__ out, const LnRed& red,
                                               const TouchSpec& pf, int ntok, int perm, unsigned long long* sat, const unsigned bid,
                                               const unsigned nblk, const int wpb) {
  constexpr int D = NV * 256;
  constexpr bool WT = WT_ || COH;
  const int lane = threadIdx.x & 63;
  int row = bid * wpb + (threadIdx.x >> 6);
  unsigned touched[kLnTouch] = {};
  const unsigned tfirst = (bid >> 3) * 64 + lane, tstride = (nblk >> 3) * 64;
  const bool touch = TOUCH && wpb == 1;
  if (wpb == 1) {
    const int x = bid & 7, j = bid >> 3;
    row = (((j >> 3) * 8 + x) << 3) + (j & 7);
  }
  if (row >= M) {
    if (touch) {
      fmt_touch(pf, bid & 7, tfirst, tstride, touched);
      fmt_touch_retire(touched);
    }
    return;
  }
  float* xr = x + (size_t)row * D;
#ifdef FMT_DIAG_HOTMOD
  const size_t mrow = 0;
#else
  const size_t mrow = (size_t)row;
#endif
  const float* sh = shift + mrow * ldm;
  const float* sc = scale + mrow * ldm;
  float4 v[NV], a[NV], b[NV];
  float s = 0.f;
#pragma unroll
  for (int i = 0; i < NV; ++i) {
    const int c = i * 256 + lane * 4;
    v[i] = fh_load_f4<COH>(xr + c);
    a[i] = fh_load_f4_stream(sh + c);
    b[i] = fh_load_f4_stream(sc + c);
  }
  if (KS == 0 && touch) fmt_touch(pf, bid & 7, tfirst, tstride, touched);
  if constexpr (KS > 0) {
    float4 p[KS][NV], gt[NV], bi[NV];
#pragma unroll
    for (int i = 0; i < NV; ++i) {
      const int c = i * 256 + lane * 4;
#pragma unroll
      for (int k = 0; k < KS; ++k) {
        const float* ps = red.slab + k * red.slab_stride + (size_t)row * D + c;
        if constexpr (COH) p[k][i] = fh_load_f4<true>(ps);
        else p[k][i] = fh_load_f4_stream(ps);
      }
      gt[i] = fh_load_f4_stream(red.gate + mrow * ldm + c);
      bi[i] = *reinterpret_cast<const float4*>(red.bias + c);
    }
    if (touch) fmt_touch(pf, bid & 7, tfirst, tstride, touched);
#pragma unroll
    for (int i = 0; i < NV; ++i) {
      float4 t = p[0][i];
#pragma unroll
      for (int k = 1; k < KS; ++k) {
        t.x += p[k][i].x;
        t.y += p[k][i].y;
        t.z += p[k][i].z;
        t.w += p[k][i].w;
      }
      v[i].x += gt[i].x * (t.x + bi[i].x);
      v[i].y += gt[i].y * (t.y + bi[i].y);
      v[i].z += gt[i].z * (t.z + bi[i].z);
      v[i].w += gt[i].w * (t.w + bi[i].w);
      fh_store_f4_wt<fh_site<COH>(1), WT>(xr + i * 256 + lane * 4, v[i]);
    }
  }
#pragma unroll
  for (int i = 0; i < NV; ++i) s += (v[i].x + v[i].y) + (v[i].z + v[i].w);
  const float mu = wave_sum(s) * (1.f / D);
  float s2 = 0.f;
#pragma unroll
  for (int i = 0; i < NV; ++i) {
    const float d0 = v[i].x - mu, d1 = v[i].y - mu, d2 = v[i].z - mu, d3 = v[i].w - mu;
    s2 += (d0 * d0 + d1 * d1) + (d2 * d2 + d3 * d3);
  }
  const float rstd = rsqrtf(wave_sum(s2) * (1.f / D) + 1e-6f);
  unsigned rm = 0u;
  int orow = row;
  if (perm) {
    const int b = row / ntok, i = row - b * ntok;
    orow = (i >> 4) * perm + b * 16 + (i & 15);
  }
#pragma unroll
  for (int i = 0; i < NV; ++i) {
    const int c = i * 256 + lane * 4;
    fh_store4_wt<T, fh_site<COH>(1), WT>(reinterpret_cast<typename T::elem*>(out) + fmt_pack_off(orow, c, D / 32),
              (v[i].x - mu) * rstd * (1.f + b[i].x) + a[i].x, (v[i].y - mu) * rstd * (1.f + b[i].y) + a[i].y,
              (v[i].z - mu) * rstd * (1.f + b[i].z) + a[i].z, (v[i].w - mu) * rstd * (1.f + b[i].w) + a[i].w, rm);
  }
  fh_range_flush<T>(sat, rm);
  if (touch) fmt_touch_retire(touched);
}

template <class T, int NV, int KS, bool TOUCH, bool WT>
__global__ __launch_bounds__(256) void fmt_lnmod_kernel(float* __restrict__ x, int M, const float* __restrict__ shift,
                                                        const float* __restrict__ scale, int ldm, u16* __restrict__ out,
                                                        LnRed red, TouchSpec pf, int ntok, int perm, unsigned long long* sat) {
  fmt_lnmod_body<T, NV, KS, TOUCH, WT, false>(x, M, shift, scale, ldm, out, red, pf, ntok, perm, sat, blockIdx.x, gridDim.x,
                                              (int)(blockDim.x >> 6));
}

template <class T, int LPQ, bool TOUCH, bool WT_, bool COH>
__device__ __forceinline__ void fmt_attn_body(const u16* __restrict__ qkv, int ld, u16* __restrict__ out, int ntok, int M, int D,
                                              int window, const TouchSpec& pf, unsigned long long* sat, const int h, const int run,
                                              const int nthr, const unsigned lin, const unsigned nwg) {
  constexpr int HD = 128, PD = HD / LPQ, NU = PD / 8;
  constexpr bool WT = WT_ || COH;
  auto ld8 = [](const typename T::elem* p) -> typename T::pack8 {
    if constexpr (COH && !T::is32) return fh_load16<true>(p);
    else return T::load8(p);
  };
  const int row_ = run * (nthr / LPQ) + threadIdx.x / LPQ, part = threadIdx.x % LPQ;
  unsigned touched[2] = {0u, 0u};
  auto touch = [&]() {
    if constexpr (TOUCH) {
      fmt_touch(pf, lin & 7, (lin >> 3) * nthr + threadIdx.x, (nwg >> 3) * nthr, touched);
    }
  };
  if (row_ >= M) {
    touch();
    if constexpr (TOUCH) fmt_touch_retire(touched);
    return;
  }
  const int b = row_ / ntok, qi = row_ - b * ntok;
  const int d0 = h * HD + part * PD;
  const float scale = rsqrtf((float)HD);
  typedef typename T::elem E;
  typedef typename T::pack8 P8;
  const E* base = reinterpret_cast<const E*>(qkv) + (size_t)(b * ntok) * ld + d0;
  float qf[PD], o[PD];
#pragma unroll
  for (int u = 0; u < NU; ++u) {
    const P8 uu = ld8(base + (size_t)qi * ld + u * 8);
#pragma unroll
    for (int j = 0; j < 8; ++j) qf[u * 8 + j] = T::get(uu, j) * scale;
  }
#pragma unroll
  for (int i = 0; i < PD; ++i) o[i] = 0.f;
  float m = -INFINITY, l = 0.f;
  auto fold = [&](const P8* k, const P8* v, bool valid) {
    float dot = 0.f;
#pragma unroll
    for (int u = 0; u < NU; ++u) {
#pragma unroll
      for (int j = 0; j < 8; ++j) dot += qf[u * 8 + j] * T::get(k[u], j);
    }
#pragma unroll
    for (int d = 1; d < LPQ; d <<= 1) dot += __shfl_xor(dot, d, 64);
    if (!valid) return;
    const float mn = fmaxf(m, dot);
    const float alpha = __expf(m - mn), p = __expf(dot - mn);
    l = l * alpha + p;
    m = mn;
#pragma unroll
    for (int u = 0; u < NU; ++u) {
#pragma unroll
      for (int j = 0; j < 8; ++j) o[u * 8 + j] = o[u * 8 + j] * alpha + p * T::get(v[u], j);
    }
  };
  if (window <= 2) {
    P8 kk[5][NU], vv[5][NU];
#pragma unroll
    for (int t = 0; t < 5; ++t) {
      const int kj = min(max(qi + t - 2, 0), ntok - 1);
      const E* kp = base + (size_t)kj * ld + D;
#pragma unroll
      for (int u = 0; u < NU; ++u) {
        kk[t][u] = ld8(kp + u * 8);
        vv[t][u] = ld8(kp + D + u * 8);
      }
    }
    touch();
#pragma unroll
    for (int t = 0; t < 5; ++t) {
      const int kj = qi + t - 2;
      const bool valid = kj >= 0 && kj < ntok && (t - 2 >= -window) && (t - 2 <= window);
      fold(kk[t], vv[t], valid);
    }
  } else {
    touch();
    for (int kj = qi - window; kj <= qi + window; ++kj) {
      const int kc = min(max(kj, 0), ntok - 1);
      const E* kp = base + (size_t)kc * ld + D;
      P8 k[NU], v[NU];
#pragma unroll
      for (int u = 0; u < NU; ++u) {
        k[u] = ld8(kp + u * 8);
        v[u] = ld8(kp + D + u * 8);
      }
      fold(k, v, kj >= 0 && kj < ntok);
    }
  }
  const float inv = 1.f / l;
  const int row = b * ntok + qi;
  unsigned rm = 0u;
#pragma unroll
  for (int u = 0; u < NU; ++u) {
    P8 uo;
#pragma unroll
    for (int j = 0; j < 8; ++j) T::set(uo, j, o[u * 8 + j] * inv);
    fh_track_pack<T>(rm, uo);
    T::template store8_wt<fh_site<COH>(2), WT>(reinterpret_cast<E*>(out) + fmt_pack_off(row, d0 + u * 8, D / 32), uo);
  }
  fh_range_flush<T>(sat, rm);
  if constexpr (TOUCH) fmt_touch_retire(touched);
}

template <class T, int LPQ, bool TOUCH, bool WT>
__global__ __launch_bounds__(512) void fmt_attn_kernel(const u16* __restrict__ qkv, int ld, u16* __restrict__ out, int ntok,
                                                       int M, int D, int window, TouchSpec pf, unsigned long long* sat) {
  fmt_attn_body<T, LPQ, TOUCH, WT, false>(qkv, ld, out, ntok, M, D, window, pf, sat, blockIdx.x, blockIdx.y, blockDim.x,
                                          blockIdx.x + gridDim.x * blockIdx.y, gridDim.x * gridDim.y);
}

__device__ __forceinline__ float fh_sum8_dpp(float v) {
  v += __builtin_bit_cast(float, __builtin_amdgcn_mov_dpp(__builtin_bit_cast(int, v), 0xB1, 0xF, 0xF, true));
  v += __builtin_bit_cast(float, __builtin_amdgcn_mov_dpp(__builtin_bit_cast(int, v), 0x4E, 0xF, 0xF, true));
  v += __builtin_bit_cast(float, __builtin_amdgcn_mov_dpp(__builtin_bit_cast(int, v), 0x141, 0xF, 0xF, true));
  return v;
}

template <class T, int MTW, int HPW >
__global__ __launch_bounds__(512) void fmt_attnproj_kernel(const u16* __restrict__ qkv, int ld, GemmArgs g, int ntok, int D, int window) {
  constexpr int HD = 128, LPQ = 8, NU = HD / (LPQ * 8), KBH = HD / 32, NWV = 8, ROWS = MTW * 16;
  constexpr int NCT = NWV / HPW;
  constexpr int NPAIR = ROWS * HPW, NPASS = (NPAIR * LPQ + NWV * 64 - 1) / (NWV * 64);
  typedef typename T::elem E;
  typedef typename T::pack8 P8;
  __shared__ __attribute__((aligned(16))) E sO[HPW * MTW * KBH * 512];
  __shared__ __attribute__((aligned(16))) float sR[(HPW > 1 ? (HPW - 1) : 1) * NCT * MTW * 256];
  const int lane = threadIdx.x & 63, w = threadIdx.x >> 6, r16 = lane & 15, q4 = lane >> 4;
  const int ct = w % NCT, hh = w / NCT;
  int ks, bx, by;
  {
    const int id = blockIdx.x, nbn = g.N / (NCT * 16), nbx = nbn * g.ksplit;
    if ((nbx & 7) == 0 && (8 % g.ksplit) == 0) {
      const int slot = id >> 3, P = 8 / g.ksplit, x = id & 7;
      by = slot % g.mblk;
      ks = x / P;
      bx = (slot / g.mblk) * P + (x % P);
    } else {
      const int bxl = id % nbx;
      by = id / nbx;
      ks = bxl / nbn;
      bx = bxl - ks * nbn;
    }
  }
  const int KB = g.K >> 5;
  const int h0 = ks * HPW;
  const int nt = bx * NCT + ct;
  const E* Wp = reinterpret_cast<const E*>(g.W) + ((size_t)nt * KB + (h0 + hh) * KBH) * 512 + lane * 8;
// ... 15 lines not shown
      if (row_ < g.M) {
        const int bq = row_ / ntok, qi = row_ - bq * ntok;
        const E* base = reinterpret_cast<const E*>(qkv) + (size_t)(bq * ntok) * ld + (h0 + ah) * HD + part * 8;
        float qf[NU * 8], o[NU * 8];
        P8 qq[NU];
#pragma unroll
        for (int u = 0; u < NU; ++u) qq[u] = T::load8(base + (size_t)qi * ld + u * 64);
#pragma unroll
        for (int i = 0; i < NU * 8; ++i) o[i] = 0.f;
        float l = 0.f;
        auto dotk = [&](const P8* k) {
          float dot = 0.f;
#pragma unroll
          for (int u = 0; u < NU; ++u) {
#pragma unroll
            for (int j = 0; j < 8; ++j) dot += qf[u * 8 + j] * T::get(k[u], j);
          }
          return fh_sum8_dpp(dot);
        };
        if (window <= 2) {
          P8 kk[5][NU], vv[5][NU];
#pragma unroll
          for (int t = 0; t < 5; ++t) {
            const int kj = min(max(qi + t - 2, 0), ntok - 1);
            const E* kp = base + (size_t)kj * ld + D;
#pragma unroll
            for (int u = 0; u < NU; ++u) {
              kk[t][u] = T::load8(kp + u * 64);
              vv[t][u] = T::load8(kp + D + u * 64);
            }
          }
#pragma unroll
          for (int u = 0; u < NU; ++u) {
#pragma unroll
            for (int j = 0; j < 8; ++j) qf[u * 8 + j] = T::get(qq[u], j) * scale;
          }
          float dot[5], m = -INFINITY;
#pragma unroll
          for (int t = 0; t < 5; ++t) {
            const int kj = qi + t - 2;
            const bool valid = kj >= 0 && kj < ntok && (t - 2 >= -window) && (t - 2 <= window);
            dot[t] = valid ? dotk(kk[t]) : -INFINITY;
            m = fmaxf(m, dot[t]);
          }
#pragma unroll
          for (int t = 0; t < 5; ++t) {
            const float p = __expf(dot[t] - m);
            l += p;
#pragma unroll
            for (int u = 0; u < NU; ++u) {
#pragma unroll
              for (int j = 0; j < 8; ++j) o[u * 8 + j] += p * T::get(vv[t][u], j);
            }
          }
        } else {
#pragma unroll
          for (int u = 0; u < NU; ++u) {
#pragma unroll
            for (int j = 0; j < 8; ++j) qf[u * 8 + j] = T::get(qq[u], j) * scale;
          }
          float m = -INFINITY;
          for (int kj = max(qi - window, 0); kj <= min(qi + window, ntok - 1); ++kj) {
            const E* kp = base + (size_t)kj * ld + D;
            P8 k[NU], v[NU];
#pragma unroll
            for (int u = 0; u < NU; ++u) {
              k[u] = T::load8(kp + u * 64);
              v[u] = T::load8(kp + D + u * 64);
            }
            const float dot = dotk(k);
            const float mn = fmaxf(m, dot);
            const float alpha = __expf(m - mn), p = __expf(dot - mn);
            l = l * alpha + p;
            m = mn;
#pragma unroll
            for (int u = 0; u < NU; ++u) {
#pragma unroll
              for (int j = 0; j < 8; ++j) o[u * 8 + j] = o[u * 8 + j] * alpha + p * T::get(v[u], j);
            }
          }
        }
        const float inv = 1.f / l;
#pragma unroll
        for (int u = 0; u < NU; ++u) {
#pragma unroll
          for (int j = 0; j < 8; ++j) T::set(uo[u], j, o[u * 8 + j] * inv);
          fh_track_pack<T>(rm, uo[u]);
        }
      }
#pragma unroll
      for (int u = 0; u < NU; ++u) T::store8(sO + ah * (MTW * KBH * 512) + fmt_pack_off(qslot, u * 64 + part * 8, KBH), uo[u]);
    }
  }
  fh_range_flush<T>(g.sat, rm);
  __syncthreads();

  f32x4 acc[MTW];
#pragma unroll
  for (int i = 0; i < MTW; ++i) acc[i] = f32x4{0.f, 0.f, 0.f, 0.f};
  const E* const sOh = sO + hh * (MTW * KBH * 512);
#pragma unroll
  for (int kk = 0; kk < KBH; ++kk) {
#pragma unroll
    for (int i = 0; i < MTW; ++i) acc[i] = T::mfma(b[kk], T::load8(sOh + (i * KBH + kk) * 512 + lane * 8), acc[i]);
  }
  if constexpr (HPW > 1) {
    if (hh > 0) {
#pragma unroll
      for (int i = 0; i < MTW; ++i) *reinterpret_cast<f32x4*>(sR + (((hh - 1) * NCT + ct) * MTW + i) * 256 + lane * 4) = acc[i];
    }
    __syncthreads();
    if (hh > 0) return;
#pragma unroll
    for (int o = 1; o < HPW; ++o) {
#pragma unroll
      for (int i = 0; i < MTW; ++i) {
        const f32x4 t = *reinterpret_cast<const f32x4*>(sR + (((o - 1) * NCT + ct) * MTW + i) * 256 + lane * 4);
        acc[i] += t;
      }
    }
  }
  float* const outp = g.out_f32 + (size_t)ks * g.slab_stride + nt * 16 + q4 * 4;
#pragma unroll
  for (int i = 0; i < MTW; ++i) {
    const int row = (by * MTW + i) * 16 + r16;
    if (row < g.M) __builtin_nontemporal_store(acc[i], reinterpret_cast<f32x4*>(outp + (size_t)row * g.ldo));
  }
}

enum { MS_XEMBED = 0, MS_LN, MS_QKV, MS_ATTN, MS_PROJ, MS_FC1, MS_FC2, MS_HEAD };
struct MegaStage {
  int kind;
  unsigned nblk;
  GemmArgs g;
  long long gate_off;
  long long shift_off, scale_off, red_gate_off;
  int ks;
  const float* red_bias;
  u16* ln_out;
  int perm;
  TouchSpec pf;
  u16* att_out;
};
struct MegaCtx {
  float* xres;
  const u16* qkv16;
  const float* slab;
  size_t slab_stride;
  int M, D, ntok, ldm, window, heads;
  unsigned long long* sat;
};
struct MegaDyn {
  const float* mod;
  float dt, a, r, e;
  int euler;
  float* vout;
};
struct MegaSync {
  unsigned* grp;
  unsigned* top;
  unsigned* rel;
  unsigned* seq;
  unsigned* err;
  unsigned* err_host;
  unsigned long long* stamps;
  unsigned stamp_wg;
};

__device__ __forceinline__ bool fmt_grid_barrier(const MegaSync& sy, unsigned gen, unsigned nwg) {
  typedef __attribute__((address_space(1))) unsigned int gu32;
  const unsigned g = blockIdx.x & 7u, per = nwg >> 3;
  const unsigned old = __hip_atomic_fetch_add((gu32*)(sy.grp + g * 32), 1u, __ATOMIC_RELAXED, __HIP_MEMORY_SCOPE_AGENT);
  if (old + 1u == gen * per) {
    const unsigned t = __hip_atomic_fetch_add((gu32*)sy.top, 1u, __ATOMIC_RELAXED, __HIP_MEMORY_SCOPE_AGENT);
    if (t + 1u == gen * 8u) {
#pragma unroll
      for (int i = 0; i < 8; ++i) __hip_atomic_store((gu32*)(sy.rel + i * 32), gen, __ATOMIC_RELAXED, __HIP_MEMORY_SCOPE_AGENT);
    }
  }
  unsigned spins = 0;
  while ((int)(__hip_atomic_load((gu32*)(sy.rel + g * 32), __ATOMIC_RELAXED, __HIP_MEMORY_SCOPE_AGENT) - gen) < 0) {
    if (++spins > (1u << 18) || ((spins & 63u) == 0u && __hip_atomic_load((gu32*)sy.err, __ATOMIC_RELAXED, __HIP_MEMORY_SCOPE_AGENT) != 0u)) {
      __hip_atomic_store((gu32*)sy.err, 1u, __ATOMIC_RELAXED, __HIP_MEMORY_SCOPE_AGENT);
      if (sy.err_host) __hip_atomic_store((gu32*)sy.err_host, 1u, __ATOMIC_RELAXED, __HIP_MEMORY_SCOPE_SYSTEM);
      return false;
    }
    __builtin_amdgcn_s_sleep(1);
  }
  return true;
}

template <class T>
__global__ __launch_bounds__(512) void fmt_mega_kernel(const MegaStage* __restrict__ tab, int nstage, MegaDyn d, MegaCtx c,
                                                       MegaSync sy) {
  typedef __attribute__((address_space(1))) unsigned int gu32;
  __shared__ unsigned s_flag[2];
  const unsigned bid = blockIdx.x, nwg = gridDim.x;
  if (threadIdx.x == 0) {
    s_flag[0] = __hip_atomic_load((gu32*)sy.seq, __ATOMIC_RELAXED, __HIP_MEMORY_SCOPE_AGENT);
    s_flag[1] = 1u;
  }
  __syncthreads();
  const unsigned seq0 = s_flag[0];
  const unsigned gen0 = seq0 * (unsigned)(nstage - 1);
#ifdef MEGA_STAMPS
#define MEGA_STAMP(k) do { if (sy.stamps && bid == sy.stamp_wg && threadIdx.x == 0) sy.stamps[s * 3 + (k)] = __builtin_amdgcn_s_memrealtime(); } while (0)
#else
#define MEGA_STAMP(k) do { } while (0)
#endif
  for (int s = 0; s < nstage; ++s) {
    const MegaStage& st = tab[s];
    MEGA_STAMP(0);
    if (bid < st.nblk) {
      switch (st.kind) {
        case MS_XEMBED:
          fmt_gemm_body<T, 4, 1, 8, EPI_XEMBED, true>(st.g, bid, st.nblk);
          break;
        case MS_LN:
          if (threadIdx.x < 64) {
            const LnRed red{c.slab, c.slab_stride, st.red_bias, d.mod + st.red_gate_off};
            if (st.ks == 0)
              fmt_lnmod_body<T, 4, 0, true, true, true>(c.xres, c.M, d.mod + st.shift_off, d.mod + st.scale_off, c.ldm, st.ln_out, red,
                                                        st.pf, c.ntok, st.perm, c.sat, bid, st.nblk, 1);
            else
              fmt_lnmod_body<T, 4, 4, true, true, true>(c.xres, c.M, d.mod + st.shift_off, d.mod + st.scale_off, c.ldm, st.ln_out, red,
                                                        st.pf, c.ntok, st.perm, c.sat, bid, st.nblk, 1);
          }
          break;
        case MS_QKV:
          fmt_gemm_body<T, 3, 4, 8, EPI_T16, true>(st.g, bid, st.nblk);
          break;
        case MS_ATTN:
          if (threadIdx.x < 128)
            fmt_attn_body<T, 16, true, true, true>(c.qkv16, 3 * c.D, st.att_out, c.ntok, c.M, c.D, c.window, st.pf, c.sat,
                                                   (int)(bid % (unsigned)c.heads), (int)(bid / (unsigned)c.heads), 128, bid, st.nblk);
          break;
        case MS_PROJ: {
          GemmArgs g = st.g;
          g.gate = d.mod + st.gate_off;
          fmt_gemm_body<T, 3, 1, 8, EPI_GATE_RES, true>(g, bid, st.nblk);
          break;
        }
        case MS_FC1:
          fmt_gemm_body<T, 3, 4, 8, EPI_GELU_P16, true>(st.g, bid, st.nblk);
          break;
        case MS_FC2:
          fmt_gemm_body<T, 3, 4, 8, EPI_PARTIAL, true>(st.g, bid, st.nblk);
          break;
        default: {
          GemmArgs g = st.g;
          g.a_cfg = d.a;
          g.r_cfg = d.r;
          g.e_cfg = d.e;
          g.dt = d.dt;
          if (!d.euler) {
            g.xcur = nullptr;
            g.xin16 = nullptr;
            g.vout = d.vout;
          }
          fmt_gemm_body<T, 3, 1, 8, EPI_CFG, true>(g, bid, st.nblk);
          break;
        }
      }
    }
    MEGA_STAMP(1);
    if (s + 1 < nstage) {
      asm volatile("s_waitcnt vmcnt(0)" ::: "memory");
      __syncthreads();
      MEGA_STAMP(2);
      if (threadIdx.x == 0) {
        int pre = 0;
#pragma unroll
        for (int i = 0; i < (int)(sizeof(MegaStage) + 63) / 64; ++i) pre ^= reinterpret_cast<const int*>(&tab[s + 1])[i * 16];
        asm volatile("" ::"s"(pre));
        if (!fmt_grid_barrier(sy, gen0 + (unsigned)s + 1u, nwg)) s_flag[1] = 0u;
      }
      __syncthreads();
      if (s_flag[1] == 0u) return;
    }
  }
  if (bid == 0 && threadIdx.x == 0) __hip_atomic_store((gu32*)sy.seq, seq0 + 1u, __ATOMIC_RELAXED, __HIP_MEMORY_SCOPE_AGENT);
}

template <class T>
__global__ void fmt_build_cond_kernel(u16* __restrict__ out, int ld, int bc, int ntok, int n_prev, int dim_w, int dim_a,
                                      int dim_e, const float* __restrict__ wr, const float* __restrict__ wa,
                                      const float* __restrict__ prev_wa, const float* __restrict__ we, int we_len,
                                      const float* __restrict__ prev_we, unsigned wr_mask, unsigned wa_mask,
                                      unsigned we_mask, unsigned long long* sat) {
  const int row = blockIdx.x;
  const int s = row / ntok, i = row % ntok, q = s / bc, b = s - q * bc, n_cur = ntok - n_prev;
  const bool on_r = (wr_mask >> b) & 1, on_a = (wa_mask >> b) & 1, on_e = (we_mask >> b) & 1;
  wr += (size_t)q * dim_w;
  wa += (size_t)q * n_cur * dim_a;
  prev_wa += (size_t)q * n_prev * dim_a;
  we += (size_t)q * we_len * dim_e;
  if (prev_we) prev_we += (size_t)q * n_prev * dim_e;
  unsigned rm = 0u;
  for (int c = threadIdx.x; c < ld; c += blockDim.x) {
    float v = 0.f;
    if (c < dim_w) {
      v = on_r ? wr[c] : 0.f;
    } else if (c < dim_w + dim_a) {
      const int k = c - dim_w;
      if (i < n_prev) v = prev_wa[i * dim_a + k];
      else if (on_a) v = wa[(i - n_prev) * dim_a + k];
    } else if (c < dim_w + dim_a + dim_e) {
      const int k = c - dim_w - dim_a;
      if (on_e) {
        if (we_len == 1) v = we[k];
        else v = (i < n_prev) ? prev_we[i * dim_e + k] : we[(i - n_prev) * dim_e + k];
      }
    }
    reinterpret_cast<typename T::elem*>(out)[fmt_pack_off(row, c, ld / 32)] = fh_cvt<T>(v, rm);
  }
  fh_range_flush<T>(sat, rm);
}

__device__ __forceinline__ float fmt_linspace01(int i, int n) {
  if (n <= 1) return 0.f;
  const float step = __fdiv_rn(1.0f, (float)(n - 1));
  return (i < n / 2) ? __fmul_rn(step, (float)i) : __fsub_rn(1.0f, __fmul_rn(step, (float)(n - 1 - i)));
}
template <class T>
__global__ void fmt_tsin_kernel(u16* __restrict__ out, const float* __restrict__ freqs, int n_steps, float t0, int nfe,
                                int stages, float c0, float c1, float c2, float c3) {
  const int s = blockIdx.x;
  if (s >= n_steps) return;
  float t = t0;
  if (nfe > 0) {
    const int i = s / stages, j = s - i * stages;
    const float gi = fmt_linspace01(i, nfe);
    t = gi;
    if (j > 0) {
      const float cj = j == 1 ? c1 : (j == 2 ? c2 : c3);
      t = __fadd_rn(gi, __fmul_rn(__fsub_rn(fmt_linspace01(i + 1, nfe), gi), cj));
    }
  }
  (void)c0;
  const int k = threadIdx.x;
  const float arg = t * freqs[k & 127];
  reinterpret_cast<typename T::elem*>(out)[fmt_pack_off(s, k, 8)] = T::from_float(k < 128 ? cosf(arg) : sinf(arg));
}

template <class T>
__global__ void fmt_silu_c_kernel(u16* __restrict__ out, const float* __restrict__ temb, const float* __restrict__ ccond,
                                  int M, int D, size_t step_stride, int dense_rows, unsigned long long* sat) {
  const int idx = (blockIdx.x * blockDim.x + threadIdx.x) * 8;
  if (idx >= M * D) return;
  const int c = idx % D, row = idx / D + (int)blockIdx.y * dense_rows;
  typename T::elem* const o = reinterpret_cast<typename T::elem*>(out) + (dense_rows ? (size_t)0 : (size_t)blockIdx.y * step_stride);
  temb += (size_t)blockIdx.y * D;
  typename T::pack8 u;
#pragma unroll
  for (int h = 0; h < 2; ++h) {
    const float4 a = *reinterpret_cast<const float4*>(ccond + idx + 4 * h);
    const float4 t = *reinterpret_cast<const float4*>(temb + c + 4 * h);
    T::set(u, 4 * h + 0, fh_silu(a.x + t.x));
    T::set(u, 4 * h + 1, fh_silu(a.y + t.y));
    T::set(u, 4 * h + 2, fh_silu(a.z + t.z));
    T::set(u, 4 * h + 3, fh_silu(a.w + t.w));
  }
  unsigned rm = 0u;
  fh_track_pack<T>(rm, u);
  fh_range_flush<T>(sat, rm);
  T::store8(o + fmt_pack_off(row, c, D / 32), u);
}

template <class T>
__global__ void fmt_init_x_kernel(float* __restrict__ xcur, u16* __restrict__ xin16, int ldx, const float* __restrict__ x0,
                                  const float* __restrict__ prev_x, int n_prev, int n_cur, int dim_w, int nclip,
                                  unsigned long long* sat) {
  const int idx = blockIdx.x * blockDim.x + threadIdx.x;
  const int ntok = n_prev + n_cur;
  if (idx >= nclip * ntok * dim_w) return;
  const int q = idx / (ntok * dim_w), r = idx - q * ntok * dim_w;
  const int i = r / dim_w, c = r % dim_w;
  float v;
  if (i < n_prev) {
    v = prev_x[((size_t)q * n_prev + i) * dim_w + c];
  } else {
    v = x0[((size_t)q * n_cur + (i - n_prev)) * dim_w + c];
    xcur[((size_t)q * n_cur + (i - n_prev)) * dim_w + c] = v;
  }
  unsigned rm = 0u;
  reinterpret_cast<typename T::elem*>(xin16)[fmt_pack_off(q * ntok + i, c, ldx)] = fh_cvt<T>(v, rm);
  fh_range_flush<T>(sat, rm);
}

template <class T>
__global__ void fmt_rk_combine_kernel(float* __restrict__ xcur, const float* __restrict__ kbuf, size_t kstride, int nk, float c0,
                                      float c1, float c2, float c3, int final, u16* __restrict__ xin16, int ldx, int n_prev,
                                      int n_cur, int W, int nclip, unsigned long long* sat) {
  const int idx = blockIdx.x * blockDim.x + threadIdx.x;
  if (idx >= nclip * n_cur * W) return;
  const int q = idx / (n_cur * W), r = idx - q * n_cur * W;
  const int i = r / W, c = r % W, ntok = n_prev + n_cur;
  const float cf[4] = {c0, c1, c2, c3};
  float y = xcur[idx];
  for (int m = 0; m < nk; ++m) y += cf[m] * kbuf[(size_t)m * kstride + ((size_t)q * ntok + n_prev + i) * W + c];
  if (final) xcur[idx] = y;
  unsigned rm = 0u;
  reinterpret_cast<typename T::elem*>(xin16)[fmt_pack_off(q * ntok + n_prev + i, c, ldx)] = fh_cvt<T>(y, rm);
  fh_range_flush<T>(sat, rm);
}

__global__ void fmt_slice_pad_kernel(float* __restrict__ dst, const float* __restrict__ src, int t0, int T, int n, int dim,
                                     int nclip) {
  const int idx = blockIdx.x * blockDim.x + threadIdx.x;
  if (idx >= nclip * n * dim) return;
  const int q = idx / (n * dim), r = idx - q * n * dim;
  const int i = r / dim, c = r % dim;
  const int t = min(t0 + i, T - 1);
  dst[idx] = src[((size_t)q * T + t) * dim + c];
}

__global__ void fmt_tail_kernel(float* __restrict__ dst, const float* __restrict__ src, int n_prev, int n_cur, int dim, int nclip) {
  const int idx = blockIdx.x * blockDim.x + threadIdx.x;
  if (idx >= nclip * n_prev * dim) return;
  const int q = idx / (n_prev * dim), r = idx - q * n_prev * dim;
  dst[idx] = src[((size_t)q * n_cur + (n_cur - n_prev)) * dim + r];
}

template <class T>
__global__ void fmt_dbg_to16_kernel(u16* __restrict__ dst, const float* __restrict__ src, int n) {
  const int i = blockIdx.x * blockDim.x + threadIdx.x;
  if (i < n) reinterpret_cast<typename T::elem*>(dst)[i] = T::from_float(src[i]);
}
template <class T>
__global__ void fmt_dbg_unpack_kernel(float* __restrict__ dst, const u16* __restrict__ src, int rows, int D) {
  const int i = blockIdx.x * blockDim.x + threadIdx.x;
  if (i >= rows * D) return;
  const int r = i / D, c = i - r * D;
  dst[i] = T::to_float(reinterpret_cast<const typename T::elem*>(src)[fmt_pack_off(r, c, D / 32)]);
}

__global__ void fmt_copy_kernel(float* __restrict__ dst, size_t dpitch, const float* __restrict__ src, size_t spitch, int width, int rows) {
  const int idx = blockIdx.x * blockDim.x + threadIdx.x;
  if (idx >= rows * width) return;
  const int r = idx / width, c = idx - r * width;
  dst[(size_t)r * dpitch + c] = src ? src[(size_t)r * spitch + c] : 0.f;
}
```

comfyui-float_optimized_amd/csrc/fmt_pack.hpp:

```cpp
#pragma once
#include "common.hpp"

enum {
  EPI_F32 = 0,
  EPI_T16 = 1,
  EPI_SILU_P16 = 2,
  EPI_GELU_P16 = 3,
  EPI_GATE_RES = 4,
  EPI_XEMBED = 5,
  EPI_CFG = 6,
  EPI_PARTIAL = 7,
  EPI_GELUERF_P16 = 8
};

__host__ __device__ __forceinline__ size_t fmt_pack_off(int row, int k, int KB) {
  return ((size_t)((row >> 4) * KB + (k >> 5)) * 64 + (row & 15) + 16 * ((k >> 3) & 3)) * 8 + (k & 7);
}

struct TouchSpec {
  const char* W;
  unsigned run_shift;
  unsigned nt_shift;
  unsigned p_shift;
  unsigned tile_bytes;
  unsigned total;
};

__device__ __forceinline__ unsigned fmt_touch_line(const TouchSpec& t, unsigned xcd, unsigned l) {
  if (l >= t.total) return 0u;
  const unsigned r = l >> t.run_shift, off = l & ((1u << t.run_shift) - 1u);
  const unsigned cb = r >> t.nt_shift, jn = r & ((1u << t.nt_shift) - 1u);
  const unsigned ks = xcd >> t.p_shift, bx = (cb << t.p_shift) + (xcd & ((1u << t.p_shift) - 1u));
  return *reinterpret_cast<const unsigned*>(t.W + (size_t)((bx << t.nt_shift) + jn) * t.tile_bytes +
                                            ((size_t)((ks << t.run_shift) + off) << 7));
}
template <int N>
__device__ __forceinline__ void fmt_touch(const TouchSpec& t, unsigned xcd, unsigned first, unsigned stride, unsigned (&v)[N]) {
#pragma unroll
  for (int i = 0; i < N; ++i) v[i] = fmt_touch_line(t, xcd, first + (unsigned)i * stride);
}
template <int N>
__device__ __forceinline__ void fmt_touch_retire(const unsigned (&v)[N]) {
  unsigned o = 0u;
#pragma unroll
  for (int i = 0; i < N; ++i) o |= v[i];
  asm volatile("" ::"v"(o));
}

struct GemmArgs {
  const u16* A;
  const u16* W;
  const float* bias;
  int K, M, N;
  int mblk;
  float* out_f32;
  int ldo;
  u16* out16;
  int ldo16;
  const float* gate;
  int ldg;
  const float* pos;
  int bc, ntok, n_prev;
  int nclip;
  float a_cfg, r_cfg, e_cfg, dt;
  float* vout;
  float* xcur;
  u16* xin16;
  int ldx;
  int ksplit;
  size_t slab_stride;
  TouchSpec touch;
  int zcount, zgroup;
  size_t a_zstride, o_zstride;
  int tokblk;
  unsigned long long* sat;
};
```

comfyui-float_optimized_amd/csrc/tuning.hpp:

```cpp
#pragma once
#include <stdio.h>
#include <stdlib.h>
#include <string.h>

#include <algorithm>
#include <string>

inline int env_int(const char* name, int dflt, int lo, int hi) {
  const char* v = getenv(name);
  if (!v || !*v) return dflt;
  char* end = nullptr;
  const long x = strtol(v, &end, 10);
  return (end && *end == 0 && x >= lo && x <= hi) ? (int)x : dflt;
}
inline int env_atoi(const char* name, int dflt) {
  const char* v = getenv(name);
  return v ? atoi(v) : dflt;
}
inline bool env_set(const char* name) { return getenv(name) != nullptr; }
inline int env_scan(const char* s, int* v) { int n = 0; return sscanf(s, "%d%n", v, &n) == 1 ? n : 0; }
inline int env_scan(const char* s, double* v) { int n = 0; return sscanf(s, "%lf%n", v, &n) == 1 ? n : 0; }
template <class V>
int env_list(const char* name, V* v, int n, char sep = ',') {
  const char* s = getenv(name);
  int got = 0;
  while (s && got < n) {
    const int used = env_scan(s, v + got);
    if (!used) break;
    ++got;
    s += used;
    if (sep == ',' && *s++ != ',') break;
  }
  return got;
}

struct LayerPlan {
  int v[3] = {0, 0, 0};
  bool on() const { return v[0] > 0; }
};

enum { RB_QKV = 0, RB_PROJ, RB_FC1, RB_FC2 };

struct FmtTune {
  bool wide = true;
  int wide_variant = 7;
  bool big = true;
  bool rb = true;
  int rb_touch = 16;
  struct Rb {
    int n = 0, shape = -1, ksplit = 1;
  } rb_layer[4];
  int full_nw = 8;
  int plan[6] = {0, 0, 0, 0, 0, 0};
  LayerPlan plan_layer[4];
  int fc2_split = 4;
  int proj_split = 0;
  int touch = 230;
  bool hoist = true;
  int zgroup = 0;
  int ln_rows = 1;
  int attn_qpw = 8, attn_lpq = 16;
  bool no_tokblk = false;
  int attnproj = 0;
  int mega = 0;
  int mega_stamp_wg = 0;
  bool pack_host = false;

  static FmtTune from_env() {
    FmtTune t;
    t.wide = env_atoi("FLOAT_FMT_WIDE", 1) != 0;
    t.wide_variant = env_atoi("FLOAT_FMT_WIDE_VARIANT", t.wide_variant);
    t.big = env_atoi("FLOAT_FMT_BIG", 1) != 0;
    t.rb = env_atoi("FLOAT_FMT_RB", 1) != 0;
    t.rb_touch = env_atoi("FLOAT_FMT_RB_TOUCH", t.rb_touch);
    static const char* const layers[4] = {"QKV", "PROJ", "FC1", "FC2"};
    for (int l = 0; l < 4; ++l) {
      const std::string s = layers[l];
      int rb[2] = {-1, 1};
      t.rb_layer[l].n = env_list(("FLOAT_FMT_RB_" + s).c_str(), rb, 2);
      t.rb_layer[l].shape = rb[0];
      t.rb_layer[l].ksplit = rb[1];
      env_list(("FLOAT_FMT_PLAN_" + s).c_str(), t.plan_layer[l].v, 3);
    }
    t.full_nw = env_atoi("FLOAT_FMT_FULL_NW", t.full_nw);
    env_list("FLOAT_FMT_PLAN", t.plan, 6);
    t.fc2_split = env_atoi("FLOAT_FMT_FC2_SPLIT", t.fc2_split);
    t.proj_split = env_atoi("FLOAT_FMT_PROJ_SPLIT", t.proj_split);
    t.touch = env_atoi("FLOAT_FMT_TOUCH", t.touch);
    t.hoist = env_atoi("FLOAT_FMT_HOIST", 1) != 0;
    t.zgroup = std::max(0, env_atoi("FLOAT_FMT_ZGROUP", 0));
    t.ln_rows = std::max(1, std::min(4, env_atoi("FLOAT_FMT_LN_ROWS", 1)));
    int attn[2] = {t.attn_qpw, t.attn_lpq};
    env_list("FLOAT_FMT_ATTN", attn, 2);
    t.attn_lpq = attn[1] == 16 ? 16 : 8;
    t.attn_qpw = std::max(1, std::min(512 / t.attn_lpq, attn[0]));
    t.no_tokblk = env_set("FLOAT_FMT_NO_TOKBLK");
    t.attnproj = env_atoi("FLOAT_FMT_ATTNPROJ", 0);
    t.mega = env_atoi("FLOAT_FMT_MEGA", 0);
    t.mega_stamp_wg = env_atoi("FLOAT_FMT_MEGA_STAMP_WG", 0);
    t.pack_host = env_atoi("FLOAT_PACK_HOST", 0) != 0;
    return t;
  }
};

struct DecTune {
  int lds_pad = 0;
  unsigned ride_wgs = 16;
  int ride_min_res = 64;
  unsigned ride_pace = 3;
  bool ride_equal = false;
  double ride_w[4][3] = {{170, 140, 50}, {170, 155, 100}, {220, 200, 180}, {300, 250, 120}};
  int ride_tail = 0;
#ifdef DEC_STAMPS
  int ride_test = 0;
#endif
  bool cb_order = true;
  int conv_bn = 64, conv_bn_lo = 32;
  int tpw = 0;
  int conv_db = 0;
  bool no_zfuse = false;
  int zblur_min = 64;
  int flow_pix = 0;
  int flow_wgs = 2048;
  bool flow_epi = true;
  bool write_pyr = false;
  bool copy_memcpy = false;
  bool short_first = true;
  bool style_norm = true;

  static DecTune from_env() {
    DecTune t;
    t.lds_pad = env_int("FLOAT_DEC_LDS_PAD", 0, 0, 160 * 1024);
    t.ride_wgs = (unsigned)env_int("FLOAT_DEC_RIDE_WGS", 16, 0, 64) / 8 * 8;
    t.ride_min_res = env_int("FLOAT_DEC_RIDE_MIN_RES", 64, 64, 512);
    t.ride_pace = (unsigned)env_int("FLOAT_DEC_RIDE_PACE", 3, 0, 64);
    t.ride_equal = env_set("FLOAT_DEC_RIDE_EQUAL");
    double w[12];
    if (env_list("FLOAT_DEC_RIDE_W", w, 12, ' ') == 12)
      for (int i = 0; i < 12; ++i)
        if (w[i] > 0.0 && w[i] < 1e6) t.ride_w[i / 3][i % 3] = w[i];
    t.ride_tail = env_atoi("FLOAT_DEC_RIDE_TAIL", 0);
#ifdef DEC_STAMPS
    t.ride_test = env_int("FLOAT_DEC_RIDE_TEST", 0, 0, 2);
#endif
    t.cb_order = env_atoi("FLOAT_DEC_CB_ORDER", 1) != 0;
    t.conv_bn = env_int("FLOAT_DEC_CONV_BN", 64, 32, 64);
    t.conv_bn_lo = env_int("FLOAT_DEC_CONV_BN_LO", 32, 32, 64);
    t.tpw = env_int("FLOAT_DEC_TPW", 0, 0, 4096);
    t.conv_db = env_int("FLOAT_DEC_CONV_DB", 0, 0, 3);
    t.no_zfuse = env_set("FLOAT_DEC_NO_ZFUSE");
    t.zblur_min = env_int("FLOAT_DEC_ZBLUR_MIN", 64, 16, 4096);
    t.flow_pix = env_int("FLOAT_DEC_FLOW_PIX", 0, 0, 4);
    t.flow_wgs = env_int("FLOAT_DEC_FLOW_WGS", 2048, 8, 1 << 20);
    t.flow_epi = env_int("FLOAT_DEC_FLOW_EPI", 1, 0, 1) != 0;
    t.write_pyr = env_set("FLOAT_DEC_WRITE_PYR");
    const char* copy = getenv("FLOAT_DEC_COPY");
    t.copy_memcpy = copy && !strcmp(copy, "memcpy");
    t.short_first = env_int("FLOAT_DEC_SHORT_FIRST", 1, 0, 1) != 0;
    t.style_norm = env_int("FLOAT_DEC_STYLE_NORM", 1, 0, 1) != 0;
    return t;
  }
};

struct EncTune {
  bool no_tiles = false;
  static EncTune from_env() { return EncTune{env_set("FLOAT_ENC_NO_TILES")}; }
};

struct AudTune {
  bool attn_mfma = true;
  static AudTune from_env() { return AudTune{env_atoi("FLOAT_AUD_ATTN_MFMA", 1) != 0}; }
};
```

comfyui-float_optimized_amd/fmt.py:

```python
import ctypes as C
import math

import torch

from . import native
from .config import FmtConfig


@native.rebuildable
class FlowMatchingTransformerHIP:

    def __init__(self, state_dict, cfg: FmtConfig = None, device="cuda:0", dtype="fp16", use_graph=2, max_batch=1):
        self.cfg = cfg or FmtConfig()
        self.device = torch.device(device)
        self.dtype = dtype = native.canon_dtype(dtype)
        self.max_batch = max(1, int(max_batch))
        L = native.lib()
        c = self.cfg
        ncfg = native.FmtCfg(c.dim_w, c.dim_a, c.dim_e, c.dim_h, c.fmt_depth, c.num_heads,
                             int(c.dim_h * c.mlp_ratio), c.num_prev_frames, c.num_frames_for_clip,
                             c.attention_window, native.DTYPES[dtype], int(use_graph), self.max_batch)
        sd = {k[4:] if k.startswith("fmt.") else k: v for k, v in state_dict.items()
              if k not in ("alignment_mask", "fmt.alignment_mask")}
        arr, keep = native.tensor_table(sd)
        h = C.c_void_p()
        with torch.cuda.device(self.device):
            native.check(L.float_fmt_create(C.byref(ncfg), arr, len(sd), C.byref(h)))
        self._h = h
        del keep

    def set_method(self, name):
        if name not in native.ODE_METHODS:
            raise ValueError("unknown fixed-step ODE method %r (known: %s)" % (name, ", ".join(native.ODE_METHODS)))
        native.check(native.lib().float_fmt_set_method(self._h, native.ODE_METHODS[name]))
        self.method = name

    @torch.no_grad()
    def pos_embed_in_use(self):
        out = torch.empty(self.cfg.n_tokens, self.cfg.dim_h, device=self.device, dtype=torch.float32)
        with torch.cuda.device(self.device):
            native.check(native.lib().float_fmt_debug(self._h, 0, None, native.dev_ptr(out), native.stream_ptr(self.device)))
        return out

    @torch.no_grad()
    def attention_probe(self, qkv):
        qkv = self._f(qkv)
        if qkv.shape != (self.cfg.n_tokens, 3 * self.cfg.dim_h):
            raise ValueError("qkv must be (%d,%d)" % (self.cfg.n_tokens, 3 * self.cfg.dim_h))
        out = torch.empty(self.cfg.n_tokens, self.cfg.dim_h, device=self.device, dtype=torch.float32)
        with torch.cuda.device(self.device):
            native.check(native.lib().float_fmt_debug(self._h, 1, native.dev_ptr(qkv), native.dev_ptr(out),
                                                      native.stream_ptr(self.device)))
        return out

    def saturation(self, reset=False):
        with torch.cuda.device(self.device):
            return native.saturation("float_fmt_saturation", self._h, self.device, reset)

    def close(self):
        if getattr(self, "_h", None) and native is not None:
            native.lib().float_fmt_destroy(self._h)
            self._h = None

    __del__ = close

    def _f(self, t):
        return None if t is None else t.to(self.device, torch.float32).contiguous()

    def _check_shapes(self, x, wa, wr, we, prev_x, prev_wa, prev_we):
        c = self.cfg
        B = x.shape[0]
        if x.shape != (B, c.num_frames_for_clip, c.dim_w):
            raise ValueError("x must be (B,%d,%d), got %s" % (c.num_frames_for_clip, c.dim_w, tuple(x.shape)))
        if wa.shape != (B, c.num_frames_for_clip, c.dim_a):
            raise ValueError("wa must be (B,%d,%d), got %s" % (c.num_frames_for_clip, c.dim_a, tuple(wa.shape)))
        if wr.shape != (B, c.dim_w):
            raise ValueError("wr must be (B,%d), got %s" % (c.dim_w, tuple(wr.shape)))
        if prev_x is None or prev_wa is None:
            raise ValueError("prev_x was provided, but prev_wa was not." if prev_x is not None
                             else "prev_x / prev_wa are required")
        if we.dim() != 3 or we.shape[2] != c.dim_e:
            raise ValueError("we must be (B,1|%d,%d)" % (c.num_frames_for_clip, c.dim_e))
        if we.shape[1] > 1 and prev_we is None:
            raise ValueError("`we` is dynamic (T>1), but prev_we was not provided with prev_x/prev_wa.")
        if we.shape[1] not in (1, c.num_frames_for_clip):
            raise ValueError("Dynamic emotion latent `we` time dimension (%d) does not match audio latent `wa` "
                             "time dimension (%d)." % (we.shape[1] + c.num_prev_frames,
                                                       c.num_frames_for_clip + c.num_prev_frames))

    @torch.no_grad()
    def forward_with_cfv(self, t, x, wa, wr, we, prev_x, prev_wa, prev_we=None, a_cfg_scale=1.0, r_cfg_scale=1.0,
                         e_cfg_scale=1.0, include_r_cfg=False, **kwargs):
        x, wa, wr, we, prev_x, prev_wa, prev_we = map(self._f, (x, wa, wr, we, prev_x, prev_wa, prev_we))
        self._check_shapes(x, wa, wr, we, prev_x, prev_wa, prev_we)
        c, L = self.cfg, native.lib()
        tval = float(torch.as_tensor(t).reshape(-1)[0])
        B = x.shape[0]
        out = torch.empty(B, c.n_tokens, c.dim_w, device=self.device, dtype=torch.float32)
        dynamic = we.shape[1] > 1
        with torch.cuda.device(self.device):
            s = native.stream_ptr(self.device)
            for b in range(B):
                native.check(L.float_fmt_eval(
                    self._h, tval, native.dev_ptr(x[b]), native.dev_ptr(wa[b]), native.dev_ptr(wr[b]),
                    native.dev_ptr(we[b]), we.shape[1], native.dev_ptr(prev_x[b]), native.dev_ptr(prev_wa[b]),
                    native.dev_ptr(prev_we[b]) if dynamic else None, a_cfg_scale, r_cfg_scale, e_cfg_scale,
                    1 if include_r_cfg else 0, native.dev_ptr(out[b]), s))
        return out

    @torch.no_grad()
    def sample_chunk(self, x0, wa, wr, we, prev_x, prev_wa, prev_we=None, nfe=10, a_cfg_scale=1.0, r_cfg_scale=1.0,
                     e_cfg_scale=1.0, include_r_cfg=False):
        x0, wa, wr, we, prev_x, prev_wa, prev_we = map(self._f, (x0, wa, wr, we, prev_x, prev_wa, prev_we))
        self._check_shapes(x0, wa, wr, we, prev_x, prev_wa, prev_we)
        c, L = self.cfg, native.lib()
        B = x0.shape[0]
        out = torch.empty(B, c.num_frames_for_clip, c.dim_w, device=self.device, dtype=torch.float32)
        dynamic = we.shape[1] > 1
        with torch.cuda.device(self.device):
            s = native.stream_ptr(self.device)
            for b in range(B):
                native.check(L.float_fmt_sample_chunk(
                    self._h, native.dev_ptr(x0[b]), native.dev_ptr(wa[b]), native.dev_ptr(wr[b]),
                    native.dev_ptr(we[b]), we.shape[1], native.dev_ptr(prev_x[b]), native.dev_ptr(prev_wa[b]),
                    native.dev_ptr(prev_we[b]) if dynamic else None, int(nfe), a_cfg_scale, r_cfg_scale, e_cfg_scale,
                    1 if include_r_cfg else 0, native.dev_ptr(out[b]), s))
        return out

    @torch.no_grad()
    def sample(self, r_s, wa, we, noise, nfe=10, a_cfg_scale=2.0, r_cfg_scale=1.0, e_cfg_scale=1.0,
               include_r_cfg=False):
        r_s, wa, we, noise = map(self._f, (r_s, wa, we, noise))
        c, L = self.cfg, native.lib()
        B, T = wa.shape[0], wa.shape[1]
        n_chunks = int(math.ceil(T / c.num_frames_for_clip))
        if noise.shape != (n_chunks, B, c.num_frames_for_clip, c.dim_w):
            raise ValueError("noise must be (%d,%d,%d,%d), got %s" % (n_chunks, B, c.num_frames_for_clip, c.dim_w,
                                                                      tuple(noise.shape)))
        if we.shape[1] not in (1, T):
            raise ValueError("Dynamic emotion latent `we` time dimension (%d) does not match audio latent `wa` "
                             "time dimension (%d)." % (we.shape[1], T))
        r_d = torch.empty(B, T, c.dim_w, device=self.device, dtype=torch.float32)
        with torch.cuda.device(self.device):
            s = native.stream_ptr(self.device)
            for b0 in range(0, B, self.max_batch):
                nb = min(self.max_batch, B - b0)
                nz = noise[:, b0:b0 + nb].contiguous()
                native.check(L.float_fmt_sample_batch(
                    self._h, nb, native.dev_ptr(r_s[b0:b0 + nb]), native.dev_ptr(wa[b0:b0 + nb]), T,
                    native.dev_ptr(we[b0:b0 + nb]), we.shape[1], native.dev_ptr(nz), int(nfe), a_cfg_scale, r_cfg_scale,
                    e_cfg_scale, 1 if include_r_cfg else 0, native.dev_ptr(r_d[b0:b0 + nb]), s))
        return r_d


class WindowSampler:

    def __init__(self, fmt, r_s, wa, we, noise, nfe, a_cfg_scale, r_cfg_scale, e_cfg_scale, include_r_cfg=False,
                 windows=None, hist=None, r_d=None):
        self.fmt = fmt
        c = fmt.cfg
        f = fmt._f
        self.r_s, self.wa, self.we = f(r_s).reshape(-1), f(wa).reshape(-1, c.dim_a), f(we).reshape(-1, c.dim_e)
        self.T = self.wa.shape[0]
        self.n_chunks = int(math.ceil(self.T / c.num_frames_for_clip))
        self.noise = f(noise).reshape(self.n_chunks, c.num_frames_for_clip, c.dim_w)
        self.r_d = torch.empty(1, self.T, c.dim_w, device=fmt.device, dtype=torch.float32) if r_d is None else r_d
        w0, w1 = windows if windows is not None else (0, self.n_chunks)
        self.left = w1 - w0
        args = (fmt._h, native.dev_ptr(self.r_s), native.dev_ptr(self.wa), self.T, native.dev_ptr(self.we),
                self.we.shape[0], native.dev_ptr(self.noise), int(nfe), a_cfg_scale, r_cfg_scale, e_cfg_scale,
                1 if include_r_cfg else 0, native.dev_ptr(self.r_d))
        with torch.cuda.device(fmt.device):
            if windows is None and hist is None:
                native.check(native.lib().float_fmt_sample_begin(*args))
            else:
                self._hist = [None if t is None else f(t).reshape(c.num_prev_frames, -1) for t in (hist or (None, None, None))]
                native.check(native.lib().float_fmt_sample_begin_range(
                    *args, int(w0), int(w1), *[native.dev_ptr(t) if t is not None else None for t in self._hist]))

    def next(self):
        k, left = C.c_int32(0), C.c_int32(0)
        with torch.cuda.device(self.fmt.device):
            native.check(native.lib().float_fmt_sample_next(self.fmt._h, native.stream_ptr(self.fmt.device),
                                                            C.byref(k), C.byref(left)))
        self.left = left.value
        L = self.fmt.cfg.num_frames_for_clip
        return k.value, (k.value * L, min(self.T, (k.value + 1) * L))


def draw_noise(n_chunks, batch, cfg, seed, device="cpu"):
    g = torch.Generator(device)
    g.manual_seed(int(seed))
    return torch.stack([torch.randn(batch, cfg.num_frames_for_clip, cfg.dim_w, generator=g, device=device)
                        for _ in range(n_chunks)])
```

comfyui-float_optimized_amd/native.py:

```python
import ctypes as C
import os

import torch

_HERE = os.path.dirname(os.path.abspath(__file__))
LIB_PATH = os.path.join(_HERE, "csrc", "libfloat_hip.so")

FLOAT_DT_BF16, FLOAT_DT_FP16, FLOAT_DT_FP32 = 0, 1, 2
ODE_METHODS = {"euler": 0, "midpoint": 1, "rk4": 2, "heun2": 3, "heun3": 4}
DTYPES = {"bf16": FLOAT_DT_BF16, "bfloat16": FLOAT_DT_BF16, "fp16": FLOAT_DT_FP16, "float16": FLOAT_DT_FP16,
          "fp32": FLOAT_DT_FP32, "float32": FLOAT_DT_FP32}
DTYPE_NAMES = {FLOAT_DT_BF16: "bf16", FLOAT_DT_FP16: "fp16", FLOAT_DT_FP32: "fp32"}
DEC_SAT_SITES = 40
ABI_VERSION = 6


def canon_dtype(dtype):
    try:
        return DTYPE_NAMES[DTYPES[str(dtype)]]
    except KeyError:
        raise ValueError("unknown dtype %r (one of %s)" % (dtype, ", ".join(sorted(DTYPES)))) from None


class NativeLibraryError(RuntimeError):
    pass


class FloatTensor(C.Structure):
    _fields_ = [("name", C.c_char_p), ("data", C.POINTER(C.c_float)), ("ndim", C.c_int32),
                ("shape", C.c_int64 * 6)]


class FmtCfg(C.Structure):
    _fields_ = [(n, C.c_int32) for n in ("dim_w", "dim_a", "dim_e", "dim_h", "depth", "heads", "mlp_hidden",
                                         "n_prev", "n_cur", "attn_window", "dtype", "use_graph", "max_batch")]


class DecCfg(C.Structure):
    _fields_ = [(n, C.c_int32) for n in ("size", "style_dim", "dtype", "max_frames")]


class DecUnit(C.Structure):
    _fields_ = [(n, C.c_int32) for n in ("dtype", "cin", "cout", "res", "upsample", "n_frames", "style_dim", "flags")]


class EncCfg(C.Structure):
    _fields_ = [(n, C.c_int32) for n in ("size", "dim", "dim_motion", "dtype")]


class AudCfg(C.Structure):
    _fields_ = [("n_conv", C.c_int32), ("conv_dim", C.c_int32 * 8), ("conv_kernel", C.c_int32 * 8), ("conv_stride", C.c_int32 * 8)] + \
               [(n, C.c_int32) for n in ("hidden", "layers", "heads", "intermediate", "pos_k", "pos_groups", "dim_w", "only_last",
                                         "dtype")] + [("ln_eps", C.c_float)] + \
               [(n, C.c_int32) for n in ("feat_norm_layer", "stable_ln", "conv_bias", "num_labels")]


_F = C.POINTER(C.c_float)
_SIGNATURES = {
    "float_hip_abi_version": (C.c_int, []),
    "float_last_error": (C.c_char_p, []),
    "float_set_profiling": (C.c_int, [C.c_int32]),
    "float_probe_peaks": (C.c_int, [C.POINTER(C.c_float)] * 4 + [C.POINTER(C.c_int32)]),
    "float_profile_ms": (C.c_double, [C.c_int32, C.POINTER(C.c_int64)]),
    "float_stream_create_cu_range": (C.c_int, [C.c_int32, C.c_int32, C.POINTER(C.c_void_p)]),
    "float_stream_destroy": (C.c_int, [C.c_void_p]),
    "float_fmt_create": (C.c_int, [C.POINTER(FmtCfg), C.POINTER(FloatTensor), C.c_int32, C.POINTER(C.c_void_p)]),
    "float_fmt_destroy": (None, [C.c_void_p]),
    "float_fmt_set_method": (C.c_int, [C.c_void_p, C.c_int32]),
    "float_fmt_debug": (C.c_int, [C.c_void_p, C.c_int32, C.c_void_p, C.c_void_p, C.c_void_p]),
    "float_fmt_eval": (C.c_int, [C.c_void_p, C.c_float] + [C.c_void_p] * 4 + [C.c_int32] + [C.c_void_p] * 3 +
                       [C.c_float] * 3 + [C.c_int32, C.c_void_p, C.c_void_p]),
    "float_fmt_sample_chunk": (C.c_int, [C.c_void_p] + [C.c_void_p] * 4 + [C.c_int32] + [C.c_void_p] * 3 +
                               [C.c_int32] + [C.c_float] * 3 + [C.c_int32, C.c_void_p, C.c_void_p]),
    "float_fmt_sample": (C.c_int, [C.c_void_p, C.c_void_p, C.c_void_p, C.c_int32, C.c_void_p, C.c_int32, C.c_void_p,
                                   C.c_int32] + [C.c_float] * 3 + [C.c_int32, C.c_void_p, C.c_void_p]),
    "float_fmt_sample_batch": (C.c_int, [C.c_void_p, C.c_int32, C.c_void_p, C.c_void_p, C.c_int32, C.c_void_p, C.c_int32,
                                         C.c_void_p, C.c_int32] + [C.c_float] * 3 + [C.c_int32, C.c_void_p, C.c_void_p]),
    "float_fmt_sample_begin": (C.c_int, [C.c_void_p, C.c_void_p, C.c_void_p, C.c_int32, C.c_void_p, C.c_int32, C.c_void_p,
                                         C.c_int32] + [C.c_float] * 3 + [C.c_int32, C.c_void_p]),
    "float_fmt_sample_next": (C.c_int, [C.c_void_p, C.c_void_p, C.POINTER(C.c_int32), C.POINTER(C.c_int32)]),
    "float_fmt_sample_begin_range": (C.c_int, [C.c_void_p, C.c_void_p, C.c_void_p, C.c_int32, C.c_void_p, C.c_int32, C.c_void_p,
                                               C.c_int32] + [C.c_float] * 3 + [C.c_int32, C.c_void_p, C.c_int32, C.c_int32] +
                                     [C.c_void_p] * 3),
    "float_dec_create": (C.c_int, [C.POINTER(DecCfg), C.POINTER(FloatTensor), C.c_int32, C.POINTER(C.c_void_p)]),
    "float_dec_destroy": (None, [C.c_void_p]),
    "float_dec_set_feats": (C.c_int, [C.c_void_p, C.POINTER(C.c_void_p), C.c_int32, C.c_void_p]),
    "float_dec_frames": (C.c_int, [C.c_void_p, C.c_void_p, C.c_void_p, C.c_int32, C.c_void_p, C.c_void_p]),
    "float_dec_frames_host": (C.c_int, [C.c_void_p, C.c_void_p, C.c_void_p, C.c_int32, C.c_void_p, C.c_void_p, C.c_void_p,
                                        C.c_void_p]),
    "float_dec_frames_u8": (C.c_int, [C.c_void_p, C.c_void_p, C.c_void_p, C.c_int32, C.c_void_p, C.c_void_p]),
    "float_dec_frames_host_u8": (C.c_int, [C.c_void_p, C.c_void_p, C.c_void_p, C.c_int32, C.c_void_p, C.c_void_p, C.c_void_p,
                                           C.c_void_p]),
    "float_dec_feat_shape": (C.c_int, [C.c_void_p, C.c_int32, C.POINTER(C.c_int32), C.POINTER(C.c_int32)]),
    "float_dec_frames_raw": (C.c_int, [C.c_void_p, C.c_void_p, C.c_void_p, C.c_int32, C.c_void_p, C.c_void_p]),
    "float_dec_direction": (C.c_int, [C.c_void_p, C.c_void_p, C.c_void_p, C.c_void_p]),
    "float_dec_saturation": (C.c_int, [C.c_void_p, C.POINTER(C.c_uint64), C.POINTER(C.c_uint64), C.c_int32, C.c_void_p]),
    "float_dec_debug_styled_conv": (C.c_int, [C.POINTER(DecUnit), C.POINTER(FloatTensor), C.c_int32, C.c_void_p, C.c_void_p,
                                              C.c_void_p, C.POINTER(C.c_uint64), C.c_void_p]),
    "float_dec_debug_flow_level": (C.c_int, [C.POINTER(DecUnit), C.POINTER(FloatTensor), C.c_int32] + [C.c_void_p] * 9),
    "float_dec_set_feats16": (C.c_int, [C.c_void_p, C.POINTER(C.c_void_p), C.c_int32, C.c_int32, C.c_void_p]),
    "float_enc_create": (C.c_int, [C.POINTER(EncCfg), C.POINTER(FloatTensor), C.c_int32, C.POINTER(C.c_void_p)]),
    "float_enc_destroy": (None, [C.c_void_p]),
    "float_enc_forward": (C.c_int, [C.c_void_p] * 5 + [C.POINTER(C.c_void_p), C.c_int32, C.c_void_p]),
    "float_aud_create": (C.c_int, [C.POINTER(AudCfg), C.POINTER(FloatTensor), C.c_int32, C.POINTER(C.c_void_p)]),
    "float_aud_destroy": (None, [C.c_void_p]),
    "float_aud_reserve": (C.c_int, [C.c_void_p, C.c_int32, C.c_int32, C.c_void_p]),
    "float_aud_classify": (C.c_int, [C.c_void_p, C.c_void_p, C.c_int32, C.c_void_p, C.c_void_p]),
    "float_aud_inference": (C.c_int, [C.c_void_p, C.c_void_p, C.c_int32, C.c_int32, C.c_void_p, C.c_void_p]),
    "float_enc_feats16": (C.c_int, [C.c_void_p, C.POINTER(C.c_void_p), C.POINTER(C.c_int32), C.c_int32, C.POINTER(C.c_int32)]),
    "float_enc_export_feats16": (C.c_int, [C.c_void_p, C.POINTER(C.c_void_p), C.c_int32, C.c_void_p]),
    "float_fmt_saturation": (C.c_int, [C.c_void_p, C.POINTER(C.c_uint64), C.c_int32, C.c_void_p]),
    "float_enc_saturation": (C.c_int, [C.c_void_p, C.POINTER(C.c_uint64), C.c_int32, C.c_void_p]),
    "float_aud_saturation": (C.c_int, [C.c_void_p, C.POINTER(C.c_uint64), C.c_int32, C.c_void_p]),
    "float_cmp_segments": (C.c_int, [C.c_void_p, C.c_void_p, C.c_int32, C.c_int64, C.c_float, C.c_void_p, C.c_void_p, C.c_size_t,
                                     C.c_void_p]),
    "float_cmp_work_bytes": (C.c_size_t, [C.c_int32, C.c_int64]),
}
EXPORTS = tuple(_SIGNATURES)

_lib = None


def lib():
    global _lib
    if _lib is not None:
        return _lib
    if not os.path.exists(LIB_PATH):
        raise NativeLibraryError(
            "libfloat_hip.so not built: run `python -c 'import __graft_entry__ as g; g.build()'` or "
            "`make -C comfyui-float_optimized_amd/csrc` (there is no CPU fallback)")
    try:
        L = C.CDLL(LIB_PATH)
    except OSError as e:
        raise NativeLibraryError("cannot load %s: %s" % (LIB_PATH, e)) from e
    for name, (res, args) in _SIGNATURES.items():
        try:
            fn = getattr(L, name)
        except AttributeError as e:
            raise NativeLibraryError("libfloat_hip.so does not export %s" % name) from e
        fn.restype = res
        fn.argtypes = args
    if L.float_hip_abi_version() != ABI_VERSION:
        raise NativeLibraryError("libfloat_hip.so ABI version mismatch")
    _lib = L
    return L


_ERR_TYPES = {1: ValueError, 2: KeyError, 3: RuntimeError, 4: MemoryError}


def check(rc):
    if rc != 0:
        msg = lib().float_last_error().decode("utf-8", "replace")
        raise _ERR_TYPES.get(rc, RuntimeError)(msg)


def tensor_table(state):
    keep = []
    arr = (FloatTensor * len(state))()
    for i, (k, v) in enumerate(state.items()):
        t = v.detach().to("cpu", torch.float32).contiguous()
        nm = k.encode()
        keep.append((t, nm))
        arr[i].name = nm
        arr[i].data = C.cast(t.data_ptr(), _F)
        arr[i].ndim = t.dim()
        for d in range(t.dim()):
            arr[i].shape[d] = t.shape[d]
    return arr, keep


def dev_ptr(t, name="tensor"):
    if t is None:
        return None
    if not t.is_cuda:
        raise ValueError("%s must live on the GPU" % name)
    if t.dtype != torch.float32 or not t.is_contiguous():
        raise TypeError("%s must be contiguous float32" % name)
    return C.c_void_p(t.data_ptr())


def stream_ptr(device=None):
    return C.c_void_p(torch.cuda.current_stream(device).cuda_stream)


def cu_range_stream(cu_begin, cu_end, device=None):
    p = C.c_void_p()
    check(lib().float_stream_create_cu_range(int(cu_begin), int(cu_end), C.byref(p)))
    return torch.cuda.ExternalStream(p.value, device=device)


def saturation(fn_name, handle, device=None, reset=False):
    tot = C.c_uint64(0)
    check(getattr(lib(), fn_name)(handle, C.byref(tot), 1 if reset else 0, stream_ptr(device)))
    return int(tot.value)


CMP_STATS = ("sum_sq_diff", "sum_sq_ref", "max_abs", "beyond_thr", "non_finite")
_cmp_work = {}


def cmp_segments(a, b, seg_len, thr=2.0 / 255):
    if not a.is_cuda or a.device != b.device or a.numel() != b.numel():
        raise ValueError("cmp_segments: a and b must hold the same number of elements on one GPU")
    seg_len = int(seg_len)
    if seg_len <= 0 or a.numel() == 0 or a.numel() % seg_len:
        raise ValueError("cmp_segments: %d elements are not whole segments of %d" % (a.numel(), seg_len))
    n_seg = a.numel() // seg_len
    L = lib()
    need = int(L.float_cmp_work_bytes(n_seg, seg_len))
    with torch.cuda.device(a.device):
        s = stream_ptr(a.device)
        key = (a.device.index, s.value)
        work = _cmp_work.get(key)
        if work is None or work.numel() * 8 < need:
            work = _cmp_work[key] = torch.empty((need + 7) // 8, dtype=torch.float64, device=a.device)
        stats = torch.empty(n_seg, len(CMP_STATS), dtype=torch.float64, device=a.device)
        check(L.float_cmp_segments(dev_ptr(a, "a"), dev_ptr(b, "b"), n_seg, seg_len, float(thr), C.c_void_p(stats.data_ptr()),
                                   C.c_void_p(work.data_ptr()), work.numel() * 8, s))
    return stats


def set_profiling(on):
    check(lib().float_set_profiling(1 if on else 0))


def profile_ms(which):
    n = C.c_int64(0)
    ms = lib().float_profile_ms(which, C.byref(n))
    return ms, n.value


def rebuildable(cls):
    init = cls.__init__

    def __init__(self, *a, **k):
        if "_ctor" not in self.__dict__:
            self._ctor = (a, k)
        init(self, *a, **k)

    def offload(self):
        self.close()

    def to_target(self):
        if not self.__dict__.get("_h"):
            a, k = self._ctor
            type(self).__init__(self, *a, **k)
        return self

    cls.__init__ = __init__
    cls.offload = offload
    cls.to_target = to_target
    cls.resident = property(lambda self: bool(self.__dict__.get("_h")))
    return cls


def probe_peaks(device=None):
    v = [C.c_float(0) for _ in range(4)]
    n = C.c_int32(0)
    with torch.cuda.device(device if device is not None else torch.cuda.current_device()):
        torch.cuda.synchronize()
        check(lib().float_probe_peaks(C.byref(v[0]), C.byref(v[1]), C.byref(v[2]), C.byref(v[3]), C.byref(n)))
    return {"hbm_read_GBps": round(v[0].value, 1), "hbm_copy_GBps": round(v[1].value, 1), "mfma_f16_16x16x32_TFLOPs": round(v[2].value, 1),
            "mfma_f16_32x32x16_TFLOPs": round(v[3].value, 1), "compute_units": n.value}
# ... 1 lines not shown
```

include/float_hip.h:

```cpp
#ifndef FLOAT_HIP_H
#define FLOAT_HIP_H

#include <stddef.h>
#include <stdint.h>

#ifdef __cplusplus
extern "C" {
#endif

#define FLOAT_HIP_ABI_VERSION 6

enum {
  FLOAT_OK = 0,
  FLOAT_E_INVALID = 1,
  FLOAT_E_MISSING = 2,
  FLOAT_E_HIP = 3,
  FLOAT_E_NOMEM = 4
};

enum { FLOAT_DT_BF16 = 0, FLOAT_DT_FP16 = 1, FLOAT_DT_FP32 = 2 };

typedef struct {
  const char* name;
  const float* data;
  int32_t ndim;
  int64_t shape[6];
} float_tensor_t;

typedef struct {
  int32_t dim_w, dim_a, dim_e, dim_h;
  int32_t depth, heads;
  int32_t mlp_hidden;
  int32_t n_prev, n_cur;
  int32_t attn_window;
  int32_t dtype;
  int32_t use_graph;
  int32_t max_batch;
} float_fmt_cfg_t;

typedef struct float_fmt float_fmt_t;

int float_fmt_create(const float_fmt_cfg_t* cfg, const float_tensor_t* tensors, int32_t n_tensors,
                     float_fmt_t** out);
void float_fmt_destroy(float_fmt_t* h);

enum { FLOAT_ODE_EULER = 0, FLOAT_ODE_MIDPOINT = 1, FLOAT_ODE_RK4 = 2, FLOAT_ODE_HEUN2 = 3, FLOAT_ODE_HEUN3 = 4 };
int float_fmt_set_method(float_fmt_t* h, int32_t method);

int float_fmt_saturation(float_fmt_t* h, uint64_t* total, int32_t reset, void* stream);

int float_fmt_eval(float_fmt_t* h, float t, const float* x, const float* wa, const float* wr,
                   const float* we, int32_t we_len, const float* prev_x, const float* prev_wa,
                   const float* prev_we, float a_cfg, float r_cfg, float e_cfg, int32_t include_r_cfg,
                   float* out, void* stream);

int float_fmt_sample_chunk(float_fmt_t* h, const float* x0, const float* wa, const float* wr,
                           const float* we, int32_t we_len, const float* prev_x, const float* prev_wa,
                           const float* prev_we, int32_t nfe, float a_cfg, float r_cfg, float e_cfg,
                           int32_t include_r_cfg, float* out, void* stream);

int float_fmt_sample(float_fmt_t* h, const float* wr, const float* wa, int32_t T, const float* we,
                     int32_t we_len, const float* noise, int32_t nfe, float a_cfg, float r_cfg,
                     float e_cfg, int32_t include_r_cfg, float* r_d, void* stream);

int float_fmt_sample_batch(float_fmt_t* h, int32_t n_clips, const float* wr, const float* wa, int32_t T,
                           const float* we, int32_t we_len, const float* noise, int32_t nfe, float a_cfg,
                           float r_cfg, float e_cfg, int32_t include_r_cfg, float* r_d, void* stream);

int float_fmt_sample_begin(float_fmt_t* h, const float* wr, const float* wa, int32_t T, const float* we,
                           int32_t we_len, const float* noise, int32_t nfe, float a_cfg, float r_cfg,
                           float e_cfg, int32_t include_r_cfg, float* r_d);
int float_fmt_sample_next(float_fmt_t* h, void* stream, int32_t* window_done, int32_t* windows_left);

int float_fmt_sample_begin_range(float_fmt_t* h, const float* wr, const float* wa, int32_t T, const float* we,
                                 int32_t we_len, const float* noise, int32_t nfe, float a_cfg, float r_cfg,
                                 float e_cfg, int32_t include_r_cfg, float* r_d, int32_t first_window,
                                 int32_t end_window, const float* hist_x, const float* hist_wa, const float* hist_we);

int float_fmt_debug(float_fmt_t* h, int32_t what, const float* in, float* out, void* stream);

typedef struct {
  int32_t size;
  int32_t style_dim;
  int32_t dtype;
  int32_t max_frames;
} float_dec_cfg_t;

typedef struct float_dec float_dec_t;

int float_dec_create(const float_dec_cfg_t* cfg, const float_tensor_t* tensors, int32_t n_tensors,
                     float_dec_t** out);
void float_dec_destroy(float_dec_t* h);

int float_dec_set_feats(float_dec_t* h, const float* const* feats, int32_t n_feats, void* stream);

int float_dec_frames(float_dec_t* h, const float* s_r, const float* r_d, int32_t n_frames,
                     float* out_hwc, void* stream);

int float_dec_frames_host(float_dec_t* h, const float* s_r, const float* r_d, int32_t n_frames,
                          float* out_hwc, float* host_hwc, void* stream, void* copy_stream);

int float_dec_frames_u8(float_dec_t* h, const float* s_r, const float* r_d, int32_t n_frames,
                        uint8_t* out_hwc, void* stream);
int float_dec_frames_host_u8(float_dec_t* h, const float* s_r, const float* r_d, int32_t n_frames,
                             uint8_t* out_hwc, uint8_t* host_hwc, void* stream, void* copy_stream);

int float_dec_feat_shape(float_dec_t* h, int32_t i, int32_t* channels, int32_t* resolution);

int float_dec_frames_raw(float_dec_t* h, const float* s_r, const float* r_d, int32_t n_frames,
                         float* out_chw, void* stream);

#define FLOAT_DEC_SAT_SITES 40
int float_dec_saturation(float_dec_t* h, uint64_t* total, uint64_t* per_site, int32_t reset, void* stream);

typedef struct {
  int32_t dtype;
  int32_t cin, cout;
  int32_t res;
  int32_t upsample;
  int32_t n_frames;
  int32_t style_dim;
  int32_t flags;
} float_dec_unit_t;
int float_dec_debug_styled_conv(const float_dec_unit_t* u, const float_tensor_t* tensors, int32_t n_tensors, const float* x,
                                const float* style, float* out, uint64_t* saturated, void* stream);
int float_dec_debug_flow_level(const float_dec_unit_t* u, const float_tensor_t* tensors, int32_t n_tensors, const float* x,
                               const float* feat, const float* style, const float* prev_flow, const float* prev_rgb,
                               float* out_flow, float* out_blend, float* out_rgb, void* stream);

int float_dec_direction(float_dec_t* h, const float* lam, float* r_s, void* stream);

int float_dec_set_feats16(float_dec_t* h, const void* const* feats16, int32_t n_feats, int32_t dtype,
                          void* stream);

typedef struct {
  int32_t size;
  int32_t dim;
  int32_t dim_motion;
  int32_t dtype;
} float_enc_cfg_t;

typedef struct float_enc float_enc_t;

int float_enc_create(const float_enc_cfg_t* cfg, const float_tensor_t* tensors, int32_t n_tensors,
                     float_enc_t** out);
void float_enc_destroy(float_enc_t* h);

int float_enc_forward(float_enc_t* h, const float* img, float* s_r, float* lam, float* r_s,
                      float* const* feats, int32_t n_feats, void* stream);

int float_enc_saturation(float_enc_t* h, uint64_t* total, int32_t reset, void* stream);
int float_enc_feats16(float_enc_t* h, const void** feats16, int32_t* channels, int32_t max_feats,
                      int32_t* n_out);
int float_enc_export_feats16(float_enc_t* h, void* const* dst, int32_t n_feats, void* stream);

typedef struct {
  int32_t n_conv;
  int32_t conv_dim[8], conv_kernel[8], conv_stride[8];
  int32_t hidden, layers, heads, intermediate;
  int32_t pos_k, pos_groups;
  int32_t dim_w;
  int32_t only_last;
  int32_t dtype;
  float ln_eps;
  int32_t feat_norm_layer;
  int32_t stable_ln;
  int32_t conv_bias;
  int32_t num_labels;
} float_aud_cfg_t;

typedef struct float_aud float_aud_t;

int float_aud_create(const float_aud_cfg_t* cfg, const float_tensor_t* tensors, int32_t n_tensors,
                     float_aud_t** out);
void float_aud_destroy(float_aud_t* h);

int float_aud_reserve(float_aud_t* h, int32_t n_samples, int32_t seq_len, void* stream);
int float_aud_saturation(float_aud_t* h, uint64_t* total, int32_t reset, void* stream);

int float_aud_inference(float_aud_t* h, const float* a, int32_t n_samples, int32_t seq_len, float* wa,
                        void* stream);

int float_aud_classify(float_aud_t* h, const float* a, int32_t n_samples, float* scores, void* stream);

int float_hip_abi_version(void);
const char* float_last_error(void);
int float_stream_create_cu_range(int32_t cu_begin, int32_t cu_end, void** stream_out);
int float_stream_destroy(void* stream);
int float_set_profiling(int32_t on);
double float_profile_ms(int32_t which, int64_t* n_launches);
int float_probe_peaks(float* hbm_read_gbps, float* hbm_copy_gbps, float* mfma16_tflops, float* mfma32_tflops, int32_t* n_cu);

int float_cmp_segments(const float* a, const float* b, int32_t n_seg, int64_t seg_len, float thr, double* stats, void* work,
                       size_t work_bytes, void* stream);
size_t float_cmp_work_bytes(int32_t n_seg, int64_t seg_len);

#ifdef __cplusplus
}
#endif
#endif
```

Measured before the change: 2361 frames/s.

## Deduplicate adaLN modulation rows across CFG branches and tokens

Builds a compact row map so CFG branches that share the same conditioning, and tokens whose conditioning does not vary, share one modulation row. The condition build, c_embed GEMM and the per-step modulation computation then run only over the unique rows. LayerNorm-mod and gated-residual epilogues index the modulation buffer through this map instead of using the raw row index. This cuts the per-step modulation GEMM work and memory traffic, at the cost of an integer division/remap in hot epilogues and a more complex indexing contract.

After: 2303 frames/s. 2.5% lower.

```diff
diff --git a/comfyui-float_optimized_amd/csrc/fmt_api.hip b/comfyui-float_optimized_amd/csrc/fmt_api.hip
--- a/comfyui-float_optimized_amd/csrc/fmt_api.hip
+++ b/comfyui-float_optimized_amd/csrc/fmt_api.hip
@@ -564,7 +564,7 @@
 }
 
 template <class T>
-int launch_lnmod(float_fmt* h, int M, const float* shift, const float* scale, hipStream_t s, PendingRed* pend = nullptr,
+int launch_lnmod(float_fmt* h, int M, const float* shift, const float* scale, const ModRows& mr, hipStream_t s, PendingRed* pend = nullptr,
                  const Lin* next = nullptr, u16* out = nullptr, int perm = 0, int touch_bit = 1, int rb_shape = -1) {
   const int nv = h->D / 256;
   const int rpw = h->tune.ln_rows;
@@ -579,10 +579,10 @@
                        : make_touch(h->tune, *next, M, 0, (grid.x / 8) * 64, 6);
 #define LN_LAUNCH(NV, KS)                                                                                                          \
   do {                                                                                                                             \
-    if (pf.W && wt) hipLaunchKernelGGL((fmt_lnmod_kernel<T, NV, KS, true, true>), grid, block, 0, s, h->xres, M, shift, scale, h->Ntot, out ? out : h->h16, red, pf, h->ntok, perm, h->sat); \
-    else if (pf.W) hipLaunchKernelGGL((fmt_lnmod_kernel<T, NV, KS, true, false>), grid, block, 0, s, h->xres, M, shift, scale, h->Ntot, out ? out : h->h16, red, pf, h->ntok, perm, h->sat); \
-    else if (wt) hipLaunchKernelGGL((fmt_lnmod_kernel<T, NV, KS, false, true>), grid, block, 0, s, h->xres, M, shift, scale, h->Ntot, out ? out : h->h16, red, pf, h->ntok, perm, h->sat); \
-    else hipLaunchKernelGGL((fmt_lnmod_kernel<T, NV, KS, false, false>), grid, block, 0, s, h->xres, M, shift, scale, h->Ntot, out ? out : h->h16, red, pf, h->ntok, perm, h->sat);   \
+    if (pf.W && wt) hipLaunchKernelGGL((fmt_lnmod_kernel<T, NV, KS, true, true>), grid, block, 0, s, h->xres, M, shift, scale, h->Ntot, out ? out : h->h16, red, pf, h->ntok, perm, h->sat, mr); \
+    else if (pf.W) hipLaunchKernelGGL((fmt_lnmod_kernel<T, NV, KS, true, false>), grid, block, 0, s, h->xres, M, shift, scale, h->Ntot, out ? out : h->h16, red, pf, h->ntok, perm, h->sat, mr); \
+    else if (wt) hipLaunchKernelGGL((fmt_lnmod_kernel<T, NV, KS, false, true>), grid, block, 0, s, h->xres, M, shift, scale, h->Ntot, out ? out : h->h16, red, pf, h->ntok, perm, h->sat, mr); \
+    else hipLaunchKernelGGL((fmt_lnmod_kernel<T, NV, KS, false, false>), grid, block, 0, s, h->xres, M, shift, scale, h->Ntot, out ? out : h->h16, red, pf, h->ntok, perm, h->sat, mr);   \
   } while (0)
 #define LN_CASE(NV)                     \
   case NV:                              \
@@ -883,16 +883,16 @@
 }
 
 template <class T>
-int run_mega(float_fmt* h, int bc, const float* modbuf, bool euler, float dt, float a, float r, float e, hipStream_t s, float* vout_to) {
+int run_mega(float_fmt* h, int bc, const float* modbuf, const ModRows& mr, bool euler, float dt, float a, float r, float e, hipStream_t s, float* vout_to) {
   float_fmt::MegaPlan& P = h->mega[bc];
-  MegaDyn d{modbuf, dt, a, r, e, euler ? 1 : 0, vout_to ? vout_to : h->vout};
+  MegaDyn d{modbuf, mr, dt, a, r, e, euler ? 1 : 0, vout_to ? vout_to : h->vout};
   fh_launch_prof(0, (fmt_mega_kernel<T>), dim3(kMegaWgs), dim3(512), kMegaSmem, s, P.dev, P.nstage, d, P.ctx, mega_sync_of(h));
   FH_CHECK_HIP(hipGetLastError());
   return FLOAT_OK;
 }
 
 template <class T>
-int run_blocks(float_fmt* h, int nclip, int bc, const float* modbuf, bool euler, float dt, float a, float r, float e, hipStream_t s,
+int run_blocks(float_fmt* h, int nclip, int bc, const float* modbuf, const ModRows& mr, bool euler, float dt, float a, float r, float e, hipStream_t s,
                float* vout_to = nullptr) {
   const float_fmt_cfg_t& c = h->cfg;
   const FmtTune& tn = h->tune;
@@ -900,7 +900,7 @@
   int rc;
   if constexpr (!T::is32) {
     if (bc <= 4 && mega_shape_ok<T>(h, nclip, bc)) {
-      if (h->mega[bc].dev) return run_mega<T>(h, bc, modbuf, euler, dt, a, r, e, s, vout_to);
+      if (h->mega[bc].dev) return run_mega<T>(h, bc, modbuf, mr, euler, dt, a, r, e, s, vout_to);
     }
   }
   {
@@ -922,7 +922,7 @@
   for (int b = 0; b < c.depth; ++b) {
     const float* mod = modbuf + (size_t)b * 6 * D;
     const Blk& B = h->blk[b];
-    if ((rc = launch_lnmod<T>(h, M, mod, mod + D, s, &pend, &B.qkv, nullptr, 0, 128, rb_qkv.shape))) return rc;
+    if ((rc = launch_lnmod<T>(h, M, mod, mod + D, mr, s, &pend, &B.qkv, nullptr, 0, 128, rb_qkv.shape))) return rc;
     {
       GemmArgs g = base_args(h->h16, B.qkv, M);
       g.sat = h->sat;
@@ -962,10 +962,11 @@
       g.ldo = D;
       g.gate = mod + 2 * D;
       g.ldg = h->Ntot;
+      g.mrows = mr;
       if (tn.touch & 16) g.touch = make_touch(tn, B.fc1, M, 0, gemm_lanes_per_xcd(tn, M, g.N, g.K), 2);
       if ((rc = run_gemm<T, EPI_GATE_RES>(tn, g, s, false, &tn.plan_layer[RB_PROJ]))) return rc;
     }
-    if ((rc = launch_lnmod<T>(h, M, mod + 3 * D, mod + 4 * D, s, &pend, &B.fc1, nullptr, 0, 64, rb_fc1.shape))) return rc;
+    if ((rc = launch_lnmod<T>(h, M, mod + 3 * D, mod + 4 * D, mr, s, &pend, &B.fc1, nullptr, 0, 64, rb_fc1.shape))) return rc;
     {
       GemmArgs g = base_args(h->h16, B.fc1, M);
       g.sat = h->sat;
@@ -1004,6 +1005,7 @@
       g.ldo = D;
       g.gate = mod + 5 * D;
       g.ldg = h->Ntot;
+      g.mrows = mr;
       if ((rc = run_gemm<T, EPI_GATE_RES>(tn, g, s))) return rc;
     }
   }
@@ -1012,7 +1014,7 @@
     const bool tokblk = (!tn.no_tokblk || nclip > 1) && (bc == 1 || bc == 3 || bc == 4) && h->final_lin.K % 256 == 0;
     FH_REQUIRE(tokblk || nclip == 1, "batched sampling needs the token-blocked head GEMM");
     const int nblk = (ntok + 15) / 16, seqs = nclip * bc;
-    if ((rc = launch_lnmod<T>(h, M, mod, mod + D, s, &pend, nullptr, tokblk ? h->hfin16 : nullptr, tokblk ? seqs * 16 : 0))) return rc;
+    if ((rc = launch_lnmod<T>(h, M, mod, mod + D, mr, s, &pend, nullptr, tokblk ? h->hfin16 : nullptr, tokblk ? seqs * 16 : 0))) return rc;
     GemmArgs g = base_args(tokblk ? h->hfin16 : h->h16, h->final_lin, tokblk ? nblk * seqs * 16 : M);
     g.sat = h->sat;
     g.tokblk = tokblk ? 1 : 0;
@@ -1085,19 +1087,73 @@
   return {4, 0b1110u, 0b1100u, 0b0100u, 1};
 }
 
-template <class T>
-int stage_window(float_fmt* h, const CfgMode& m, const float* x0, const float* wa, const float* wr, const float* we,
+int mod_rows(const CfgMode& m, int we_len, int n_prev, int n_cur, bool compact, ModRows* out) {
+  ModRows r;
+  memset(&r, 0, sizeof(r));
+  FH_REQUIRE(m.bc >= 1 && m.bc <= 4 && n_prev >= 0 && n_cur >= 1, "modulation row layout: %d CFG branches of %d + %d tokens", m.bc, n_prev, n_cur);
+  const int ntok = n_prev + n_cur;
+  auto inv = [](int d) { return d > 1 ? (unsigned)((0xffffffffull + (unsigned)d) / (unsigned)d) : 0u; };
+  r.ntok = ntok;
+  r.n_prev = n_prev;
+  r.bc = m.bc;
+  r.inv_ntok = inv(ntok);
+  r.inv_bc = inv(m.bc);
+  r.one_ntok = ntok == 1;
+  r.one_bc = m.bc == 1;
+  int next = 0, prev_of[4], cur_of[4];
+  unsigned prev_key[4], cur_key[4];
+  for (int b = 0; b < m.bc; ++b) {
+    const unsigned on_r = (m.wr_mask >> b) & 1u, on_a = (m.wa_mask >> b) & 1u, on_e = (m.we_mask >> b) & 1u;
+    prev_key[b] = on_r | on_e << 2;
+    cur_key[b] = on_r | on_a << 1 | on_e << 2;
+    prev_of[b] = cur_of[b] = b;
+    if (compact)
+      for (int o = b - 1; o >= 0; --o) {
+        if (prev_key[o] == prev_key[b]) prev_of[b] = o;
+        if (cur_key[o] == cur_key[b]) cur_of[b] = o;
+      }
+    const bool per_tok = !compact || on_a || (on_e && we_len > 1);
+    unsigned pb, cb;
+    if (prev_of[b] == b) {
+      pb = (unsigned)next;
+      next += n_prev;
+      r.own |= 1u << b;
+    } else {
+      pb = (unsigned)(r.prev_base >> (16 * prev_of[b])) & 0xffffu;
+    }
+    if (cur_of[b] == b) {
+      cb = (unsigned)next;
+      next += per_tok ? n_cur : 1;
+      r.own |= 1u << (4 + b);
+    } else {
+      cb = (unsigned)(r.cur_base >> (16 * cur_of[b])) & 0xffffu;
+    }
+    r.prev_base |= (unsigned long long)pb << (16 * b);
+    r.cur_base |= (unsigned long long)cb << (16 * b);
+    if (per_tok) r.cur_stride |= 1u << b;
+  }
+  r.per_clip = next;
+  *out = r;
+  return FLOAT_OK;
+}
+int mod_rows_total(const ModRows& r, int nclip) { return nclip * r.per_clip; }
+
+template <class T>
+int stage_window(float_fmt* h, const CfgMode& m, const ModRows& mr, const float* x0, const float* wa, const float* wr, const float* we,
                  int we_len, const float* prev_x, const float* prev_wa, const float* prev_we, hipStream_t s) {
   const float_fmt_cfg_t& c = h->cfg;
   const int M = m.nclip * m.bc * h->ntok;
   hipLaunchKernelGGL((fmt_build_cond_kernel<T>), dim3(M), dim3(256), 0, s, h->cond16, h->Kc, m.bc, h->ntok, c.n_prev,
-                     c.dim_w, c.dim_a, c.dim_e, wr, wa, prev_wa, we, we_len, prev_we, m.wr_mask, m.wa_mask, m.we_mask, h->sat);
-  GemmArgs g = base_args(h->cond16, h->c_embed, M);
+                     c.dim_w, c.dim_a, c.dim_e, wr, wa, prev_wa, we, we_len, prev_we, m.wr_mask, m.wa_mask, m.we_mask, mr, h->sat);
+  GemmArgs g = base_args(h->cond16, h->c_embed, mod_rows_total(mr, m.nclip));
   g.sat = h->sat;
   g.out_f32 = h->ccond;
   g.ldo = h->D;
   int rc;
-  if ((rc = run_gemm<T, EPI_F32>(h->tune, g, s))) return rc;
+  {
+    const Tiling t = T::is32 ? pick_tiling32(M) : pick_tiling(h->tune, M, g.N, g.K, false);
+    if ((rc = launch_gemm<T, EPI_F32>(g, t.mtw, t.nt, t.nw, false, s))) return rc;
+  }
   const int n = m.nclip * h->ntok * c.dim_w;
   hipLaunchKernelGGL((fmt_init_x_kernel<T>), dim3((n + 255) / 256), dim3(256), 0, s, h->xcur, h->xin16, h->Kx / 32, x0, prev_x,
                      c.n_prev, c.n_cur, c.dim_w, m.nclip, h->sat);
@@ -1142,12 +1198,12 @@
 int n_evals(int method, int nfe) { return (nfe - 1) * tableau(method).s; }
 
 template <class T>
-int run_window_steps(float_fmt* h, const CfgMode& m, int nfe, const std::vector<float>& ts, float a, float r, float e,
-                     hipStream_t s) {
+int run_window_steps(float_fmt* h, const CfgMode& m, const ModRows& mr, int nfe, const std::vector<float>& ts, float a, float r,
+                     float e, hipStream_t s) {
   const Tableau& tb = tableau(h->method);
   const float_fmt_cfg_t& c = h->cfg;
   const size_t kstride = (size_t)h->Bmax * kMaxTok * c.dim_w;
-  const int n = m.nclip * c.n_cur * c.dim_w, rows = m.nclip * m.bc * h->ntok;
+  const int n = m.nclip * c.n_cur * c.dim_w, rows = mod_rows_total(mr, m.nclip);
   const int nev = n_evals(h->method, nfe), batch = h->tune.hoist ? kScSteps : 1;
   const bool euler = h->method == FLOAT_ODE_EULER;
   int rc;
@@ -1157,7 +1213,7 @@
     if (z == 0 && (rc = run_mod_all<T>(h, rows, ev, std::min(batch, nev - ev), s))) return rc;
     const float* mod = h->modall + (size_t)z * h->mod_zs;
     if (euler) {
-      if ((rc = run_blocks<T>(h, m.nclip, m.bc, mod, true, dt, a, r, e, s))) return rc;
+      if ((rc = run_blocks<T>(h, m.nclip, m.bc, mod, mr, true, dt, a, r, e, s))) return rc;
       continue;
     }
     if (j > 0) {
@@ -1165,7 +1221,7 @@
                          dt * tb.a[j][0], dt * tb.a[j][1], dt * tb.a[j][2], 0.f, 0, h->xin16, h->Kx / 32, c.n_prev, c.n_cur,
                          c.dim_w, m.nclip, h->sat);
     }
-    if ((rc = run_blocks<T>(h, m.nclip, m.bc, mod, false, 0.f, a, r, e, s, h->kbuf + (size_t)j * kstride))) return rc;
+    if ((rc = run_blocks<T>(h, m.nclip, m.bc, mod, mr, false, 0.f, a, r, e, s, h->kbuf + (size_t)j * kstride))) return rc;
     if (j == tb.s - 1) {
       hipLaunchKernelGGL((fmt_rk_combine_kernel<T>), dim3((n + 255) / 256), dim3(256), 0, s, h->xcur, h->kbuf, kstride, tb.s,
                          dt * tb.b[0], dt * tb.b[1], dt * tb.b[2], dt * tb.b[3], 1, h->xin16, h->Kx / 32, c.n_prev, c.n_cur,
@@ -1178,7 +1234,7 @@
 
 constexpr size_t kMaxGraphs = 8;
 template <class T>
-int run_window_steps_graph(float_fmt* h, const CfgMode& m, int we_len, int nfe, const std::vector<float>& ts, float a,
+int run_window_steps_graph(float_fmt* h, const CfgMode& m, const ModRows& mr, int we_len, int nfe, const std::vector<float>& ts, float a,
                            float r, float e, hipStream_t s) {
   float_fmt::GraphKey key;
   memset(&key, 0, sizeof(key));
@@ -1199,7 +1255,7 @@
     hipGraph_t graph = nullptr;
     h->cap_prio = key.prio;
     FH_CHECK_HIP(hipStreamBeginCapture(h->cap_stream, hipStreamCaptureModeThreadLocal));
-    int rc = run_window_steps<T>(h, m, nfe, ts, a, r, e, h->cap_stream);
+    int rc = run_window_steps<T>(h, m, mr, nfe, ts, a, r, e, h->cap_stream);
     hipError_t ce = hipStreamEndCapture(h->cap_stream, &graph);
     if (rc) {
       if (graph) (void)hipGraphDestroy(graph);
@@ -1234,8 +1290,10 @@
   FH_REQUIRE(!h->tune.no_tokblk || m.bc * h->ntok <= 240,
              "%d-way CFG of %d tokens is %d rows; the all-rows CFG epilogue GEMM holds at most 240 (15 row tiles)", m.bc, h->ntok,
              m.bc * h->ntok);
-  int rc = stage_window<T>(h, m, x0, wa, wr, we, we_len, prev_x, prev_wa, prev_we, s);
+  ModRows mr;
+  int rc = mod_rows(m, we_len, h->cfg.n_prev, h->cfg.n_cur, h->tune.modrows, &mr);
   if (rc) return rc;
+  if ((rc = stage_window<T>(h, m, mr, x0, wa, wr, we, we_len, prev_x, prev_wa, prev_we, s))) return rc;
   if (nfe <= 1) return FLOAT_OK;
   hipStreamCaptureStatus cs = hipStreamCaptureStatusNone;
   if (hipStreamIsCapturing(s, &cs) != hipSuccess) {
@@ -1243,8 +1301,8 @@
     cs = hipStreamCaptureStatusNone;
   }
   if (h->cfg.use_graph && !g_fh_profiling && cs == hipStreamCaptureStatusNone)
-    return run_window_steps_graph<T>(h, m, we_len, nfe, ts, a, r, e, s);
-  return run_window_steps<T>(h, m, nfe, ts, a, r, e, s);
+    return run_window_steps_graph<T>(h, m, mr, we_len, nfe, ts, a, r, e, s);
+  return run_window_steps<T>(h, m, mr, nfe, ts, a, r, e, s);
 }
 
 template <class T>
@@ -1259,9 +1317,11 @@
   FH_REQUIRE(!h->tune.no_tokblk || m.bc * h->ntok <= 240,
              "%d-way CFG of %d tokens is %d rows; the all-rows CFG epilogue GEMM holds at most 240 (15 row tiles)", m.bc, h->ntok,
              m.bc * h->ntok);
-  if ((rc = stage_window<T>(h, m, x, wa, wr, we, we_len, prev_x, prev_wa, prev_we, s))) return rc;
-  if ((rc = run_mod_all<T>(h, m.bc * h->ntok, 0, 1, s))) return rc;
-  if ((rc = run_blocks<T>(h, 1, m.bc, h->modall, false, 0.f, a, r, e, s))) return rc;
+  ModRows mr;
+  if ((rc = mod_rows(m, we_len, h->cfg.n_prev, h->cfg.n_cur, h->tune.modrows, &mr))) return rc;
+  if ((rc = stage_window<T>(h, m, mr, x, wa, wr, we, we_len, prev_x, prev_wa, prev_we, s))) return rc;
+  if ((rc = run_mod_all<T>(h, mod_rows_total(mr, 1), 0, 1, s))) return rc;
+  if ((rc = run_blocks<T>(h, 1, m.bc, h->modall, mr, false, 0.f, a, r, e, s))) return rc;
   return dev_copy(out, h->vout, (size_t)h->ntok * h->cfg.dim_w, s);
 }
 
@@ -1587,6 +1647,27 @@
                                          : debug_impl<FP32>(h, what, in, out, (hipStream_t)stream);
 }
 
+int float_fmt_mod_rows(float_fmt_t* h, float a_cfg, float r_cfg, float e_cfg, int32_t include_r_cfg, int32_t we_len, int32_t n_clips,
+                       int32_t* total, int32_t* row_of, int32_t n_rows) {
+  FH_REQUIRE(h && total, "null argument to float_fmt_mod_rows");
+  FH_REQUIRE(n_clips >= 1, "float_fmt_mod_rows: %d clips", n_clips);
+  CfgMode m = cfg_mode(a_cfg, r_cfg, e_cfg, include_r_cfg);
+  m.nclip = n_clips;
+  ModRows mr;
+  if (int rc = mod_rows(m, we_len, h->cfg.n_prev, h->cfg.n_cur, h->tune.modrows, &mr)) return rc;
+  *total = mod_rows_total(mr, n_clips);
+  if (row_of) {
+    const int M = n_clips * m.bc * h->ntok;
+    FH_REQUIRE(n_rows == M, "float_fmt_mod_rows: row_of holds %d rows, the chain has %d", n_rows, M);
+    for (int row = 0; row < M; ++row) {
+      const int seq = row / mr.ntok, tok = row - seq * mr.ntok, clip = seq / mr.bc, b = seq - clip * mr.bc;
+      const int pb = (int)((mr.prev_base >> (16 * b)) & 0xffffu), cb = (int)((mr.cur_base >> (16 * b)) & 0xffffu);
+      row_of[row] = clip * mr.per_clip + (tok < mr.n_prev ? pb + tok : cb + (((mr.cur_stride >> b) & 1u) ? tok - mr.n_prev : 0));
+    }
+  }
+  return FLOAT_OK;
+}
+
 int float_fmt_saturation(float_fmt_t* h, uint64_t* total, int32_t reset, void* stream) {
   FH_REQUIRE(h && total, "null argument to float_fmt_saturation");
   FH_CHECK_HIP(hipStreamSynchronize((hipStream_t)stream));
diff --git a/comfyui-float_optimized_amd/csrc/fmt_kernels.hpp b/comfyui-float_optimized_amd/csrc/fmt_kernels.hpp
--- a/comfyui-float_optimized_amd/csrc/fmt_kernels.hpp
+++ b/comfyui-float_optimized_amd/csrc/fmt_kernels.hpp
@@ -62,7 +62,7 @@
     const int row = m0 + r, nb = n0 + cg * 8;
     if (r < ROWS && row < g.M) {
       const float* o = g.out_f32 + (size_t)row * g.ldo + nb;
-      const float* gt = g.gate + (size_t)row * g.ldg + nb;
+      const float* gt = g.gate + (size_t)fmt_mod_row(g.mrows, (unsigned)row) * g.ldg + nb;
       res_pf[0] = fh_load_f4<COH>(o);
       res_pf[1] = fh_load_f4<COH>(o + 4);
       gate_pf[0] = fh_load_f4_stream(gt);
@@ -209,7 +209,7 @@
         else T::template store8_wt<fh_site<COH>(8), WT>(o16 + fmt_pack_off(row, nb, g.ldo16), u);
       } else if constexpr (EPI == EPI_GATE_RES) {
         float* o = g.out_f32 + (size_t)row * g.ldo + nb;
-        const float* gt = g.gate + (size_t)row * g.ldg + nb;
+        const float* gt = g.gate + (size_t)fmt_mod_row(g.mrows, (unsigned)row) * g.ldg + nb;
 #pragma unroll
         for (int e = 0; e < 8; e += 4) {
           float4 x, gg;
@@ -602,8 +602,8 @@
 
 template <class T, int NV, int KS, bool TOUCH, bool WT_, bool COH>
 __device__ __forceinline__ void fmt_lnmod_body(float* __restrict__ x, int M, const float* __restrict__ shift,
-                                               const float* __restrict__ scale, int ldm, u16* __restrict__ out, const LnRed& red,
-                                               const TouchSpec& pf, int ntok, int perm, unsigned long long* sat, const unsigned bid,
+                                               const float* __restrict__ scale, int ldm, const ModRows& mr, u16* __restrict__ out,
+                                               const LnRed& red, const TouchSpec& pf, int ntok, int perm, unsigned long long* sat, const unsigned bid,
                                                const unsigned nblk, const int wpb) {
   constexpr int D = NV * 256;
   constexpr bool WT = WT_ || COH;
@@ -616,6 +616,11 @@
     const int x = bid & 7, j = bid >> 3;
     row = (((j >> 3) * 8 + x) << 3) + (j & 7);
   }
+#ifdef FMT_DIAG_HOTMOD
+  const size_t mrow = 0;
+#else
+  const size_t mrow = (size_t)fmt_mod_row(mr, (unsigned)__builtin_amdgcn_readfirstlane(row));
+#endif
   if (row >= M) {
     if (touch) {
       fmt_touch(pf, bid & 7, tfirst, tstride, touched);
@@ -624,11 +629,6 @@
     return;
   }
   float* xr = x + (size_t)row * D;
-#ifdef FMT_DIAG_HOTMOD
-  const size_t mrow = 0;
-#else
-  const size_t mrow = (size_t)row;
-#endif
   const float* sh = shift + mrow * ldm;
   const float* sc = scale + mrow * ldm;
   float4 v[NV], a[NV], b[NV];
@@ -703,8 +703,9 @@
 template <class T, int NV, int KS, bool TOUCH, bool WT>
 __global__ __launch_bounds__(256) void fmt_lnmod_kernel(float* __restrict__ x, int M, const float* __restrict__ shift,
                                                         const float* __restrict__ scale, int ldm, u16* __restrict__ out,
-                                                        LnRed red, TouchSpec pf, int ntok, int perm, unsigned long long* sat) {
-  fmt_lnmod_body<T, NV, KS, TOUCH, WT, false>(x, M, shift, scale, ldm, out, red, pf, ntok, perm, sat, blockIdx.x, gridDim.x,
+                                                        LnRed red, TouchSpec pf, int ntok, int perm, unsigned long long* sat,
+                                                        ModRows mr) {
+  fmt_lnmod_body<T, NV, KS, TOUCH, WT, false>(x, M, shift, scale, ldm, mr, out, red, pf, ntok, perm, sat, blockIdx.x, gridDim.x,
                                               (int)(blockDim.x >> 6));
 }
 
@@ -1026,6 +1027,7 @@
 };
 struct MegaDyn {
   const float* mod;
+  ModRows mrows;
   float dt, a, r, e;
   int euler;
   float* vout;
@@ -1094,10 +1096,10 @@
           if (threadIdx.x < 64) {
             const LnRed red{c.slab, c.slab_stride, st.red_bias, d.mod + st.red_gate_off};
             if (st.ks == 0)
-              fmt_lnmod_body<T, 4, 0, true, true, true>(c.xres, c.M, d.mod + st.shift_off, d.mod + st.scale_off, c.ldm, st.ln_out, red,
+              fmt_lnmod_body<T, 4, 0, true, true, true>(c.xres, c.M, d.mod + st.shift_off, d.mod + st.scale_off, c.ldm, d.mrows, st.ln_out, red,
                                                         st.pf, c.ntok, st.perm, c.sat, bid, st.nblk, 1);
             else
-              fmt_lnmod_body<T, 4, 4, true, true, true>(c.xres, c.M, d.mod + st.shift_off, d.mod + st.scale_off, c.ldm, st.ln_out, red,
+              fmt_lnmod_body<T, 4, 4, true, true, true>(c.xres, c.M, d.mod + st.shift_off, d.mod + st.scale_off, c.ldm, d.mrows, st.ln_out, red,
                                                         st.pf, c.ntok, st.perm, c.sat, bid, st.nblk, 1);
           }
           break;
@@ -1112,6 +1114,7 @@
         case MS_PROJ: {
           GemmArgs g = st.g;
           g.gate = d.mod + st.gate_off;
+          g.mrows = d.mrows;
           fmt_gemm_body<T, 3, 1, 8, EPI_GATE_RES, true>(g, bid, st.nblk);
           break;
         }
@@ -1161,9 +1164,11 @@
                                       int dim_e, const float* __restrict__ wr, const float* __restrict__ wa,
                                       const float* __restrict__ prev_wa, const float* __restrict__ we, int we_len,
                                       const float* __restrict__ prev_we, unsigned wr_mask, unsigned wa_mask,
-                                      unsigned we_mask, unsigned long long* sat) {
+                                      unsigned we_mask, ModRows mr, unsigned long long* sat) {
   const int row = blockIdx.x;
   const int s = row / ntok, i = row % ntok, q = s / bc, b = s - q * bc, n_cur = ntok - n_prev;
+  if (i < n_prev ? !((mr.own >> b) & 1u) : (!((mr.own >> (4 + b)) & 1u) || (!((mr.cur_stride >> b) & 1u) && i > n_prev))) return;
+  const int orow = (int)fmt_mod_row(mr, (unsigned)row);
   const bool on_r = (wr_mask >> b) & 1, on_a = (wa_mask >> b) & 1, on_e = (we_mask >> b) & 1;
   wr += (size_t)q * dim_w;
   wa += (size_t)q * n_cur * dim_a;
@@ -1186,7 +1191,7 @@
         else v = (i < n_prev) ? prev_we[i * dim_e + k] : we[(i - n_prev) * dim_e + k];
       }
     }
-    reinterpret_cast<typename T::elem*>(out)[fmt_pack_off(row, c, ld / 32)] = fh_cvt<T>(v, rm);
+    reinterpret_cast<typename T::elem*>(out)[fmt_pack_off(orow, c, ld / 32)] = fh_cvt<T>(v, rm);
   }
   fh_range_flush<T>(sat, rm);
 }
diff --git a/comfyui-float_optimized_amd/csrc/fmt_pack.hpp b/comfyui-float_optimized_amd/csrc/fmt_pack.hpp
--- a/comfyui-float_optimized_amd/csrc/fmt_pack.hpp
+++ b/comfyui-float_optimized_amd/csrc/fmt_pack.hpp
@@ -47,6 +47,30 @@
   asm volatile("" ::"v"(o));
 }
 
+struct ModRows {
+  unsigned long long prev_base, cur_base;
+  unsigned cur_stride;
+  unsigned own;
+  unsigned inv_ntok, inv_bc;
+  unsigned one_ntok, one_bc;
+  int ntok, n_prev, bc;
+  int per_clip;
+};
+__device__ __forceinline__ unsigned fmt_udiv(unsigned n, unsigned inv, unsigned one) { return __umulhi(n, inv) + n * one; }
+struct ModRowPos {
+  unsigned clip, b, tok;
+};
+__device__ __forceinline__ ModRowPos fmt_mod_pos(const ModRows& m, unsigned row) {
+  const unsigned seq = fmt_udiv(row, m.inv_ntok, m.one_ntok), clip = fmt_udiv(seq, m.inv_bc, m.one_bc);
+  return ModRowPos{clip, seq - clip * (unsigned)m.bc, row - seq * (unsigned)m.ntok};
+}
+__device__ __forceinline__ unsigned fmt_mod_row(const ModRows& m, unsigned row) {
+  const ModRowPos p = fmt_mod_pos(m, row);
+  const unsigned pb = (unsigned)(m.prev_base >> (p.b * 16u)) & 0xffffu, cb = (unsigned)(m.cur_base >> (p.b * 16u)) & 0xffffu;
+  const unsigned cur = cb + (((m.cur_stride >> p.b) & 1u) ? p.tok - (unsigned)m.n_prev : 0u);
+  return p.clip * (unsigned)m.per_clip + (p.tok < (unsigned)m.n_prev ? pb + p.tok : cur);
+}
+
 struct GemmArgs {
   const u16* A;
   const u16* W;
@@ -74,4 +98,5 @@
   size_t a_zstride, o_zstride;
   int tokblk;
   unsigned long long* sat;
+  ModRows mrows;
 };
diff --git a/comfyui-float_optimized_amd/csrc/tuning.hpp b/comfyui-float_optimized_amd/csrc/tuning.hpp
--- a/comfyui-float_optimized_amd/csrc/tuning.hpp
+++ b/comfyui-float_optimized_amd/csrc/tuning.hpp
@@ -57,6 +57,7 @@
   int proj_split = 0;
   int touch = 230;
   bool hoist = true;
+  bool modrows = true;
   int zgroup = 0;
   int ln_rows = 1;
   int attn_qpw = 8, attn_lpq = 16;
@@ -88,6 +89,7 @@
     t.proj_split = env_atoi("FLOAT_FMT_PROJ_SPLIT", t.proj_split);
     t.touch = env_atoi("FLOAT_FMT_TOUCH", t.touch);
     t.hoist = env_atoi("FLOAT_FMT_HOIST", 1) != 0;
+    t.modrows = env_atoi("FLOAT_FMT_MODROWS", 1) != 0;
     t.zgroup = std::max(0, env_atoi("FLOAT_FMT_ZGROUP", 0));
     t.ln_rows = std::max(1, std::min(4, env_atoi("FLOAT_FMT_LN_ROWS", 1)));
     int attn[2] = {t.attn_qpw, t.attn_lpq};
diff --git a/comfyui-float_optimized_amd/fmt.py b/comfyui-float_optimized_amd/fmt.py
--- a/comfyui-float_optimized_amd/fmt.py
+++ b/comfyui-float_optimized_amd/fmt.py
@@ -56,6 +56,16 @@
     def saturation(self, reset=False):
         with torch.cuda.device(self.device):
             return native.saturation("float_fmt_saturation", self._h, self.device, reset)
+
+    def mod_rows(self, a_cfg_scale=2.0, r_cfg_scale=1.0, e_cfg_scale=1.0, include_r_cfg=False, dynamic_we=False, n_clips=1):
+        c = self.cfg
+        a, r, e = float(a_cfg_scale), float(r_cfg_scale), float(e_cfg_scale)
+        bc = 1 if (a == 1.0 and r == 1.0 and e == 1.0) else (4 if include_r_cfg else 3)
+        n = int(n_clips) * bc * c.n_tokens
+        total, row_of = C.c_int32(0), (C.c_int32 * n)()
+        native.check(native.lib().float_fmt_mod_rows(self._h, a, r, e, 1 if include_r_cfg else 0,
+                                                     c.num_frames_for_clip if dynamic_we else 1, int(n_clips), C.byref(total), row_of, n))
+        return int(total.value), list(row_of)
 
     def close(self):
         if getattr(self, "_h", None) and native is not None:
diff --git a/comfyui-float_optimized_amd/native.py b/comfyui-float_optimized_amd/native.py
--- a/comfyui-float_optimized_amd/native.py
+++ b/comfyui-float_optimized_amd/native.py
@@ -110,6 +110,8 @@
     "float_enc_feats16": (C.c_int, [C.c_void_p, C.POINTER(C.c_void_p), C.POINTER(C.c_int32), C.c_int32, C.POINTER(C.c_int32)]),
     "float_enc_export_feats16": (C.c_int, [C.c_void_p, C.POINTER(C.c_void_p), C.c_int32, C.c_void_p]),
     "float_fmt_saturation": (C.c_int, [C.c_void_p, C.POINTER(C.c_uint64), C.c_int32, C.c_void_p]),
+    "float_fmt_mod_rows": (C.c_int, [C.c_void_p] + [C.c_float] * 3 + [C.c_int32] * 3 + [C.POINTER(C.c_int32), C.POINTER(C.c_int32),
+                                     C.c_int32]),
     "float_enc_saturation": (C.c_int, [C.c_void_p, C.POINTER(C.c_uint64), C.c_int32, C.c_void_p]),
     "float_aud_saturation": (C.c_int, [C.c_void_p, C.POINTER(C.c_uint64), C.c_int32, C.c_void_p]),
     "float_cmp_segments": (C.c_int, [C.c_void_p, C.c_void_p, C.c_int32, C.c_int64, C.c_float, C.c_void_p, C.c_void_p, C.c_size_t,
diff --git a/include/float_hip.h b/include/float_hip.h
--- a/include/float_hip.h
+++ b/include/float_hip.h
@@ -48,6 +48,9 @@
 int float_fmt_set_method(float_fmt_t* h, int32_t method);
 
 int float_fmt_saturation(float_fmt_t* h, uint64_t* total, int32_t reset, void* stream);
+
+int float_fmt_mod_rows(float_fmt_t* h, float a_cfg, float r_cfg, float e_cfg, int32_t include_r_cfg, int32_t we_len,
+                       int32_t n_clips, int32_t* total, int32_t* row_of, int32_t n_rows);
 
 int float_fmt_eval(float_fmt_t* h, float t, const float* x, const float* wa, const float* wr,
                    const float* we, int32_t we_len, const float* prev_x, const float* prev_wa,
```
